# BaratiLab/GAMD

Measured on AMD Instinct MI355X. Metric: atom-steps/sec (force eval + integrate), 10k-atom LJ box, higher is better.
Workload: dtype f32; 1 GPU; C2: 10 000-atom LJ box, rho*=0.5, L=92.29 A, cutoff 3.0 sigma=10.2 A, fp32, 4 conv layers x 128, random-init weights (seed 0), 1 box per GPU; n_atoms=10000, boxes=1, launch=single process

## Files before the change

gamd_amd/csrc/conv_edge.hip:

```cpp
#include "gamd_common.h"
#include "gamd_internal.h"

#include <cstdlib>

namespace {

constexpr int CONV_LDS_FLOATS = 2 * GAMD_WFRAG_FLOATS + 3 * 128;

template <bool F2, typename Post, typename Mid>
__device__ __forceinline__ void gemm128_post(const f32x4* W, int lane, const f32x16 (&X)[4], f32x16 (&acc)[4], Post post, Mid mid) {
#pragma unroll
    for (int tp = 0; tp < 4; ++tp) {
        if (tp == 1) mid();
#pragma unroll
        for (int t = 0; t < 4; ++t) {
#pragma unroll
            for (int q = 0; q < 4; ++q) {
                const f32x4 w = W[((tp * 4 + t) * 4 + q) * 64 + lane];
#pragma unroll
                for (int j = 0; j < 4; ++j) {
                    const float x = X[t][q * 4 + j];
                    acc[tp] = F2 ? mfma32(x, w[j], acc[tp]) : mfma32(w[j], x, acc[tp]);
                }
                if (tp > 0) post(tp - 1, t * 4 + q);
            }
        }
    }
#pragma unroll
    for (int g = 0; g < 16; ++g) post(3, g);
}

template <int N>
__device__ __forceinline__ void phase_barrier() {
    asm volatile("s_waitcnt vmcnt(%0) lgkmcnt(0)" ::"n"(N) : "memory");
    __builtin_amdgcn_s_barrier();
}

__device__ __forceinline__ void load_e_tile(const float* __restrict__ e_frag, int tile, int lane, f32x16 (&X)[4]) {
    const f32x4* ef = (const f32x4*)e_frag + (size_t)tile * 16 * 64;
#pragma unroll
    for (int t = 0; t < 4; ++t)
#pragma unroll
        for (int q = 0; q < 4; ++q) {
            const f32x4 v = gamd_load_stream(&ef[(t * 4 + q) * 64 + lane]);
#pragma unroll
            for (int j = 0; j < 4; ++j) X[t][q * 4 + j] = v[j];
        }
}

template <bool TIME>
__global__ void __launch_bounds__(512, 2) k_conv_edge(ConvEdgeArgs a) {
    if (a.devflags[DEVFLAG_FROZEN]) return;
    extern __shared__ __attribute__((aligned(16))) float lds[];
    float* buf0 = lds;
    float* buf1 = lds + GAMD_WFRAG_FLOATS;
    float* vb1 = buf1 + GAMD_WFRAG_FLOATS;
    float* vb3 = vb1 + 128;
    float* vb4 = vb3 + 128;

    const int tid = threadIdx.x, lane = tid & 63, slot = lane & 31, half = lane >> 5;
    const int wave = __builtin_amdgcn_readfirstlane(tid >> 6);
    const unsigned lane16 = (unsigned)lane * 16u;
    int E = a.counters[CNT_E];
    if ((long long)E > a.e_cap) E = (int)a.e_cap;
    const int n_tiles = (E + GAMD_TILE - 1) / GAMD_TILE;
    const int n_units = (n_tiles + 3) / 4;
    int first, end, step;
    gamd_xcd_range(n_units, blockIdx.x, gridDim.x, first, end, step);
    if (first >= end) return;
    const int n_iter = ((end - first + step - 1) / step + 1) / 2;
    const int wsub = wave & 3, whalf = wave >> 2;
    const bool early = whalf == 0;
    auto tile_of = [&](int it) {
        const int u = first + (2 * it + whalf) * step;
        return (it < n_iter && u < end) ? u * 4 + wsub : n_tiles;
    };
    auto stage = [&](const float* gw, float* buf) { gamd_stage_weight_raw_contig<8>(gw, buf, wave, lane16); };

    long long tacc[16];
#pragma unroll
    for (int i = 0; i < 16; ++i) tacc[i] = 0;
    long long tprev = 0;
#define TMARK(i) do { if (TIME) { const long long tn__ = (long long)__builtin_readcyclecounter(); tacc[i] += tn__ - tprev; tprev = tn__; } } while (0)

    if (tid < 128) { vb1[tid] = a.b1[tid]; vb3[tid] = a.b3[tid]; vb4[tid] = a.b4[tid]; }
    stage(a.w1p, buf0);

    f32x16 RA[4], RB[4], RC[4];
    auto init_b4 = [&]() {
#pragma unroll
        for (int tp = 0; tp < 4; ++tp) {
            const float b = vb4[32 * tp + slot];
#pragma unroll
            for (int r = 0; r < 16; ++r) RC[tp][r] = b;
        }
    };

    int tile = tile_of(0);
    bool active = tile < n_tiles;
    int src = 0, dst = 0;
    {
        const int x = tile * GAMD_TILE + gamd_pi(slot);
        if (active && x < E) { src = GAMD_CHK_RANGE(a.sticky, a.col[x], 0, a.zero_row, GAMD_CHK_CONV_SRC); dst = GAMD_CHK_RANGE(a.sticky, a.erow[x], 0, a.zero_row, GAMD_CHK_CONV_DST); }
        else { src = a.zero_row; dst = a.zero_row; }
        if (active) load_e_tile(a.e_frag, tile, lane, RA);
    }
    asm volatile("" ::"v"(src), "v"(dst));
    asm volatile("s_waitcnt vmcnt(0)" ::: "memory");
    __syncthreads();
    if (TIME) tprev = (long long)__builtin_readcyclecounter();
    unsigned pend_ends = 0;
    int pend_p = 0;

    auto gather_S = [&]() { load_row_chain(a.S + (size_t)src * GAMD_H, half, RA); };
    auto gather_hn = [&]() {
        const unsigned soff = (unsigned)src << 9;
        const unsigned idx0 = 16u * (unsigned)half;
        const unsigned slot16 = 16u * (unsigned)slot;
#pragma unroll
        for (int r4 = 0; r4 < 4; ++r4) {
            unsigned o0, o1, o2, o3;
            asm volatile("ds_bpermute_b32 %0, %4, %5 offset:%6\n\tds_bpermute_b32 %1, %4, %5 offset:%7\n\t"
                         "ds_bpermute_b32 %2, %4, %5 offset:%8\n\tds_bpermute_b32 %3, %4, %5 offset:%9\n\ts_waitcnt lgkmcnt(0)"
                         : "=&v"(o0), "=&v"(o1), "=&v"(o2), "=&v"(o3)
                         : "v"(idx0), "v"(soff), "n"(4 * (0 + 8 * r4)), "n"(4 * (1 + 8 * r4)), "n"(4 * (2 + 8 * r4)), "n"(4 * (3 + 8 * r4)));
            const unsigned o[4] = {o0, o1, o2, o3};
#pragma unroll
            for (int k = 0; k < 4; ++k) {
                const f32x4 hv = *(const f32x4*)((const char*)a.hn + (o[k] + slot16));
#pragma unroll
                for (int tp = 0; tp < 4; ++tp) RA[r4][k * 4 + tp] = hv[tp];
            }
        }
    };

    auto early_barrier = [&](bool gathered) { if (gathered) phase_barrier<16>(); else phase_barrier<0>(); };
    auto piece_stores = [&]() {
        while (__any(pend_ends != 0)) {
            if (pend_ends != 0) {
                const int r = __builtin_ctz(pend_ends);
                pend_ends &= pend_ends - 1;
                f32x4 pv;
#pragma unroll
                for (int tp = 0; tp < 4; ++tp) {
                    float v = RC[tp][0];
#pragma unroll
                    for (int k = 1; k < 16; ++k) v = (r == k) ? RC[tp][k] : v;
                    pv[tp] = v;
                }
                *(f32x4*)(a.partial + (size_t)pend_p * GAMD_H + 4 * slot) = pv;
                ++pend_p;
            }
        }
    };
#define FENCE() __builtin_amdgcn_sched_barrier(0)

    for (int it = 0; it < n_iter; ++it) {
        const int x0 = tile * GAMD_TILE + 16 * half;
        int nvalid = E - x0;
        nvalid = !active ? 0 : (nvalid >= 16 ? 16 : (nvalid <= 0 ? 0 : nvalid));
        const int tile_n = tile_of(it + 1);
        const bool active_n = tile_n < n_tiles;
        int src_n = a.zero_row, dst_n = src_n;

        if (active) {
            load_bias_chain(vb1, half, RB);
            TMARK(0);
            gemm128_post<false>((const f32x4*)buf0, lane, RA, RB,
                                [&](int tp, int g) { RB[tp][g] = gamd_silu_hw(RB[tp][g]); },
                                [&]() {
                                    FENCE();
                                    piece_stores();
                                    load_row_chain(a.D + (size_t)dst * GAMD_H, half, RC);
                                    stage(a.w2p, buf1);
                                    FENCE();
                                });
            TMARK(1);
        } else {
            piece_stores();
            stage(a.w2p, buf1);
        }
        if (!early) phase_barrier<0>();
        TMARK(2);
        if (active) gather_S();
        TMARK(3);
        if (early) early_barrier(active);
        if (active) {
            gemm128_post<false>((const f32x4*)buf1, lane, RB, RC,
                                [&](int tp, int g) { RC[tp][g] = gamd_silu_hw(RC[tp][g] + RA[tp][g]); },
                                [&]() { FENCE(); stage(a.w3p, buf0); FENCE(); });
            TMARK(4);
        } else {
            stage(a.w3p, buf0);
        }
        if (!early) phase_barrier<0>();
        TMARK(5);
        if (active) gather_hn();
        TMARK(6);
        if (early) early_barrier(active);
        unsigned mask = 0;
        int p0 = 0;
        if (active) {
            mask = a.chunk_mask[tile * 2 + half];
            p0 = GAMD_CHK_RANGE(a.sticky, a.chunk_piece[tile * 2 + half], 0, a.piece_cap - 17, GAMD_CHK_PIECE);
        }
        if (active_n) {
            const int xn = tile_n * GAMD_TILE + gamd_pi(slot);
            if (xn < E) { src_n = GAMD_CHK_RANGE(a.sticky, a.col[xn], 0, a.zero_row, GAMD_CHK_CONV_SRC); dst_n = GAMD_CHK_RANGE(a.sticky, a.erow[xn], 0, a.zero_row, GAMD_CHK_CONV_DST); }
        }
        if (active) {
            load_bias_chain(vb3, half, RB);
            TMARK(7);
            gemm128_post<false>((const f32x4*)buf0, lane, RC, RB,
                                [&](int tp, int g) { RB[tp][g] = gamd_silu_hw(RB[tp][g]); },
                                [&]() { FENCE(); stage(a.w4p, buf1); FENCE(); });
            TMARK(8);
        } else {
            stage(a.w4p, buf1);
        }
        phase_barrier<0>();
        asm volatile("" ::"v"(mask), "v"(p0), "v"(src_n), "v"(dst_n));
        TMARK(9);
        if (active) {
            init_b4();
            const unsigned keep_bits = ~(mask << 1);
            gemm128_post<true>((const f32x4*)buf1, lane, RB, RC, [&](int tp, int r) {
                RC[tp][r] = gamd_msg_acc(RA[r >> 2][(r & 3) * 4 + tp], RC[tp][r], (r > 0 && ((keep_bits >> r) & 1u)) ? RC[tp][r - 1] : 0.f);
            }, [&]() { FENCE(); if (it + 1 < n_iter) stage(a.w1p, buf0); FENCE(); });
            pend_ends = mask;
            if (nvalid > 0 && !((mask >> (nvalid - 1)) & 1u)) pend_ends |= 1u << (nvalid - 1);
            pend_p = p0;
            TMARK(10);
        } else {
            if (it + 1 < n_iter) stage(a.w1p, buf0);
        }
        if (!early) phase_barrier<0>();
        TMARK(11);
        if (active_n) load_e_tile(a.e_frag, tile_n, lane, RA);
        TMARK(12);
        if (early) early_barrier(active_n);
        TMARK(13);
        tile = tile_n; active = active_n; src = src_n; dst = dst_n;
    }
#undef FENCE
    piece_stores();
    if (TIME && a.tdbg && lane == 0) {
#pragma unroll
        for (int i = 0; i < 16; ++i) a.tdbg[((size_t)blockIdx.x * 8 + wave) * 16 + i] = tacc[i];
    }
#undef TMARK
}

template <bool TIME>
int launch(const ConvEdgeArgs& a, int n_blocks, hipStream_t st) {
    const size_t lds = sizeof(float) * CONV_LDS_FLOATS;
    static PerDeviceOnce once;
    if (int e = gamd_allow_dynamic_lds(once, (int)lds, k_conv_edge<TIME>)) return e;
    hipLaunchKernelGGL(k_conv_edge<TIME>, dim3(n_blocks), dim3(512), lds, st, a);
    GAMD_CHECK_LAUNCH();
    return 0;
}

}

int launch_conv_edge(const ConvEdgeArgs& a, int n_blocks, hipStream_t st) {
#ifdef GAMD_PROFILING
    static const bool timed = getenv("GAMD_CONV_TIME") != nullptr;
    if (timed) return launch<true>(a, n_blocks, st);
#endif
    return launch<false>(a, n_blocks, st);
}
```

gamd_amd/csrc/conv_edge_small.hip:

```cpp
#include "gamd_common.h"
#include "gamd_internal.h"

namespace {

constexpr int XLD = GAMD_XLD;

template <int EHT, int HT, bool WIDE>
__global__ void __launch_bounds__(256) k_conv_edge_small(ConvEdgeArgs a) {
    if (a.devflags[DEVFLAG_FROZEN]) return;
    constexpr int H = 128 * HT;
    __shared__ __attribute__((aligned(16))) float xbuf[32 * XLD];
    const int lane = threadIdx.x & 63, slot = lane & 31, half = lane >> 5;
    const int quarter = __builtin_amdgcn_readfirstlane(threadIdx.x >> 6);
    int E = a.counters[CNT_E];
    if ((long long)E > a.e_cap) E = (int)a.e_cap;
    const int n_tiles = (E + GAMD_TILE - 1) / GAMD_TILE;

    auto feat4 = [&](int ob) { return WIDE ? 128 * ob + 32 * quarter + slot : 4 * slot + quarter; };
    for (int tile = blockIdx.x; tile < n_tiles; tile += gridDim.x) {
        const int x = tile * GAMD_TILE + gamd_pi(slot);
        const bool valid = x < E;
        const int src = valid ? GAMD_CHK_RANGE(a.sticky, a.col[x], 0, a.zero_row, GAMD_CHK_CONV_SRC) : 0;
        const int dst = valid ? GAMD_CHK_RANGE(a.sticky, a.erow[x], 0, a.zero_row, GAMD_CHK_CONV_DST) : 0;
        f32x16 X[4], XE[EHT][4], acc;
        WQuarter wa, wb;
        const float* wblk = a.w1p;
        load_wquarter(wblk, quarter, lane, wa);
#pragma unroll
        for (int kb = 0; kb < EHT; ++kb) {
            const f32x4* ef = (const f32x4*)a.e_frag + ((size_t)tile * EHT + kb) * 16 * 64;
#pragma unroll
            for (int t = 0; t < 4; ++t)
#pragma unroll
                for (int q = 0; q < 4; ++q) {
                    const f32x4 v = ef[(t * 4 + q) * 64 + lane];
#pragma unroll
                    for (int j = 0; j < 4; ++j) XE[kb][t][q * 4 + j] = v[j];
                }
        }
        const f32x16 s_q = load_slice(a.S + (size_t)src * 128, quarter, half);
        const f32x16 d_q = load_slice(a.D + (size_t)dst * 128, quarter, half);
        f32x16 hn_q[HT];
#pragma unroll
        for (int r = 0; r < 16; ++r) {
            const int rho = (r & 3) + 8 * (r >> 2) + 4 * half;
            const int s = __shfl(src, rho, 64);
#pragma unroll
            for (int ob = 0; ob < HT; ++ob) hn_q[ob][r] = a.hn[(size_t)s * H + feat4(ob)];
        }
        const unsigned mask = a.chunk_mask[tile * 2 + half];
        const int p0 = GAMD_CHK_RANGE(a.sticky, a.chunk_piece[tile * 2 + half], 0, a.piece_cap - 17, GAMD_CHK_PIECE);
        const int x0 = tile * GAMD_TILE + 16 * half;
        int nvalid = E - x0;
        nvalid = nvalid >= 16 ? 16 : (nvalid <= 0 ? 0 : nvalid);

        acc = load_slice(a.b1, quarter, half);
#pragma unroll
        for (int kb = 0; kb < EHT; ++kb) {
            WQuarter& cur = (kb & 1) ? wb : wa;
            WQuarter& nxt = (kb & 1) ? wa : wb;
            load_wquarter(wblk + (size_t)(kb + 1) * GAMD_WFRAG_FLOATS, quarter, lane, nxt);
            gemm_quarter<false>(cur, XE[kb], acc);
        }
#pragma unroll
        for (int r = 0; r < 16; ++r) acc[r] = gamd_silu_hw(acc[r]);
        exchange(xbuf, quarter, slot, half, acc, X);
        constexpr int B2 = EHT;
        WQuarter& w2 = (B2 & 1) ? wb : wa;
        WQuarter& w3 = (B2 & 1) ? wa : wb;
        if (WIDE) acc = s_q + d_q; else acc = d_q;
        load_wquarter(wblk + (size_t)(B2 + 1) * GAMD_WFRAG_FLOATS, quarter, lane, w3);
        gemm_quarter<false>(w2, X, acc);
#pragma unroll
        for (int r = 0; r < 16; ++r) acc[r] = gamd_silu_hw(WIDE ? acc[r] : acc[r] + s_q[r]);
        exchange(xbuf, quarter, slot, half, acc, X);
        acc = load_slice(a.b3, quarter, half);
        load_wquarter(wblk + (size_t)(B2 + 2) * GAMD_WFRAG_FLOATS, quarter, lane, w2);
        gemm_quarter<false>(w3, X, acc);
#pragma unroll
        for (int r = 0; r < 16; ++r) acc[r] = gamd_silu_hw(acc[r]);
        exchange(xbuf, quarter, slot, half, acc, X);
        const unsigned keep_bits = ~(mask << 1);
        unsigned ends0 = mask;
        if (nvalid > 0 && !((mask >> (nvalid - 1)) & 1u)) ends0 |= 1u << (nvalid - 1);
#pragma unroll
        for (int ob = 0; ob < HT; ++ob) {
            WQuarter& cur = (ob & 1) ? w3 : w2;
            WQuarter& nxt = (ob & 1) ? w2 : w3;
            if (ob + 1 < HT) load_wquarter(wblk + (size_t)(B2 + 3 + ob) * GAMD_WFRAG_FLOATS, quarter, lane, nxt);
            const float b = a.b4[128 * ob + 32 * quarter + slot];
#pragma unroll
            for (int r = 0; r < 16; ++r) acc[r] = b;
            gemm_quarter<true>(cur, X, acc);
            if (WIDE && a.emb_out) {
#pragma unroll
                for (int r = 0; r < 16; ++r) a.emb_out[(size_t)(x0 + r) * H + feat4(ob)] = acc[r];
            }
#pragma unroll
            for (int r = 0; r < 16; ++r) {
                acc[r] = gamd_msg_acc((r < nvalid) ? hn_q[ob][r] : 0.f, acc[r], (r > 0 && ((keep_bits >> r) & 1u)) ? acc[r - 1] : 0.f);
            }
            unsigned ends = ends0;
            int p = p0;
            while (__any(ends != 0)) {
                if (ends != 0) {
                    const int r = __builtin_ctz(ends);
                    ends &= ends - 1;
                    float v = acc[0];
#pragma unroll
                    for (int k = 1; k < 16; ++k) v = (r == k) ? acc[k] : v;
                    a.partial[(size_t)p * H + feat4(ob)] = v;
                    ++p;
                }
            }
        }
    }
}

}

int launch_conv_edge_small(const ConvEdgeArgs& a, int n_blocks, hipStream_t st) {
    hipLaunchKernelGGL((k_conv_edge_small<1, 1, false>), dim3(n_blocks), dim3(256), 0, st, a);
    GAMD_CHECK_LAUNCH();
    return 0;
}

int launch_conv_edge_small_wide(const ConvEdgeArgs& a, int eht, int ht, int n_blocks, hipStream_t st) {
    if (eht == 1 && ht == 1) hipLaunchKernelGGL((k_conv_edge_small<1, 1, true>), dim3(n_blocks), dim3(256), 0, st, a);
    else if (eht == 1 && ht == 2) hipLaunchKernelGGL((k_conv_edge_small<1, 2, true>), dim3(n_blocks), dim3(256), 0, st, a);
    else if (eht == 2 && ht == 1) hipLaunchKernelGGL((k_conv_edge_small<2, 1, true>), dim3(n_blocks), dim3(256), 0, st, a);
    else if (eht == 2 && ht == 2) hipLaunchKernelGGL((k_conv_edge_small<2, 2, true>), dim3(n_blocks), dim3(256), 0, st, a);
    else return -22;
    GAMD_CHECK_LAUNCH();
    return 0;
}
```

gamd_amd/csrc/gamd_api.hip:

```cpp
#include "../../include/gamd_hip.h"
#include "gamd_common.h"
#include "gamd_internal.h"

#include <algorithm>
#include <cmath>
#include <cstdarg>
#include <cstddef>
#include <cstdio>
#include <cstdlib>
#include <cstring>
#include <deque>
#include <map>
#include <string>
#include <vector>

namespace {

thread_local char g_err[512] = "";

int fail(int code, const char* fmt, ...) {
    va_list ap;
    va_start(ap, fmt);
    vsnprintf(g_err, sizeof(g_err), fmt, ap);
    va_end(ap);
    return code;
}

#define HIP_TRY(expr)                                                                              \
    do {                                                                                           \
        hipError_t e__ = (expr);                                                                   \
        if (e__ != hipSuccess) return fail(-1000 - (int)e__, "%s: %s", #expr, hipGetErrorString(e__)); \
    } while (0)

struct HostTensor {
    std::vector<int64_t> shape;
    std::vector<float> data;
};

thread_local hipStream_t tl_init_stream = nullptr;
struct InitStream {
    hipStream_t prev;
    explicit InitStream(hipStream_t st) : prev(tl_init_stream) { tl_init_stream = st; }
    ~InitStream() { tl_init_stream = prev; }
    InitStream(const InitStream&) = delete;
    InitStream& operator=(const InitStream&) = delete;
};
hipError_t init_upload(void* dst, const void* src, size_t bytes) {
    hipError_t e = hipMemcpyAsync(dst, src, bytes, hipMemcpyHostToDevice, tl_init_stream);
    return e != hipSuccess ? e : hipStreamSynchronize(tl_init_stream);
}

struct DevBuf {
    void* p = nullptr;
    size_t bytes = 0;
    int ensure(size_t want, bool zero) {
        if (want <= bytes && p) return 0;
        if (p) { hipError_t e = hipFree(p); if (e != hipSuccess) return (int)e; p = nullptr; bytes = 0; }
        hipError_t e = hipMalloc(&p, want);
        if (e != hipSuccess) return (int)e;
        bytes = want;
        if (zero) {
            e = hipMemsetAsync(p, 0, want, tl_init_stream);
            if (e == hipSuccess) e = hipStreamSynchronize(tl_init_stream);
            if (e != hipSuccess) return (int)e;
        }
        return 0;
    }
    void release() { if (p) (void)hipFree(p); p = nullptr; bytes = 0; }
    template <typename T> T* as() const { return reinterpret_cast<T*>(p); }
};

struct LayerDev {
    const float *w1p, *w2p, *w3p, *w4p, *b1, *b3, *b4;
    const float *w16p = nullptr;
    const float *e_ln_g = nullptr, *e_ln_b = nullptr;
    NodeLayerW node;
};

struct DeviceGuard {
    int prev = -1;
    bool changed = false;
    explicit DeviceGuard(int dev) {
        if (hipGetDevice(&prev) == hipSuccess && prev != dev) changed = hipSetDevice(dev) == hipSuccess;
    }
    ~DeviceGuard() { if (changed) (void)hipSetDevice(prev); }
    DeviceGuard(const DeviceGuard&) = delete;
    DeviceGuard& operator=(const DeviceGuard&) = delete;
};

struct MdPending {
    bool active = false;
    int kind = 0;
    MdArgs m{};
    NhcArgs a{};
    unsigned long long first_step = 0;
    long long n_steps = 0;
    float* x = nullptr;
    float* f = nullptr;
    const uint8_t* species = nullptr;
    hipStream_t st = nullptr;
};

}

static_assert(sizeof(gamd_config) == 96 && offsetof(gamd_config, n_boxes) == 88 && offsetof(gamd_config, edge_capacity) == 40,
              "gamd_config layout is part of the C ABI (gamd_amd/_lib.py mirrors it)");

struct gamd_handle {
    gamd_config cfg{};
    int dev = 0;
    int n = 0, L = 0, n_feat = 44, n_cu = 256;
    int n_boxes = 1, n_per_box = 0;
    bool use_small = false;
    DevBuf boxes_dev, box_shift;
    std::vector<float> boxes_host;
    int H = 128, Eh = 128, HT = 1, EHT = 1;
    int H_true = 128, Eh_true = 128, D_true = 128;
    int Dp = 128, DT = 1;
    int norm_bn = 0;
    bool update_edge = false;
    bool node_f16 = false;
    bool wide_enc = false, wide_conv = false;
    long long small_tile_limit = 512;
    std::map<std::string, HostTensor> host_w;
    bool finalized = false;
    double scaler_mean = 0.0, scaler_var = 1.0;

    DevBuf wblob;
    std::vector<LayerDev> layers;
    const float *enc_w1p = nullptr, *enc_w2p = nullptr, *enc_w3p = nullptr, *enc_b1 = nullptr, *enc_b2 = nullptr,
                *enc_b3 = nullptr, *enc_lng = nullptr, *enc_lnb = nullptr, *centers = nullptr;
    const float *node_emb = nullptr, *nenc_w = nullptr, *nenc_b = nullptr;
    const float *dec_w1p = nullptr, *dec_b1 = nullptr, *dec_w2 = nullptr, *dec_b2 = nullptr;
    float length_mean = 0.f, length_std = 1.f;
    RbfGrid rbf{};

    DevBuf pos_w, pos_s, cell_of, perm, inv_perm, deg, row_ptr, na_excl, bond_nbr;
    DevBuf hbuf, hn, S, D, P, f_norm, f_den;
    DevBuf l0_h, l0_hn, l0_S, l0_D, l0_P;
    DevBuf cell_cnt, cell_fill, cell_start;
    int ncell_cap = 0;
    long long e_cap = 0;
    long long piece_cap = 0;
    DevBuf col, erow, chunk_piece, chunk_mask, e_frag, partial, feat_dbg, e_emb, e_frag2;
    DevBuf counters, tdbg, tmp_eid, ke_partial, com_partial;
    DevBuf cnt2;
    int cnt_parity = 0;
    long long skin_calls = 0;
    int* cur_counters = nullptr;
    int* counters_host = nullptr;
    float* host_in = nullptr;
    float* host_out = nullptr;
    DevBuf pos_in;
    int* sticky_host = nullptr;
    int* sticky_dev = nullptr;
    hipStream_t init_stream = nullptr;
    DevBuf devflags;
    const float* feat_dev = nullptr;
    const uint8_t* rigid_checked = nullptr;
    MdPending pending;
    bool has_bonds = false;

    float skin = 0.f;
    DevBuf ref_pos, cand_deg, cand_ptr, cand_col;
    long long cand_cap = 0;
    bool cand_valid = false;

    float box[3] = {0, 0, 0};
    int nc[3] = {1, 1, 1};
    int ncell = 1;

    bool timing = false;
    std::vector<hipEvent_t> tev;
    std::vector<int> tev_kind;
    size_t tev_used = 0;
    std::vector<hipEvent_t> sev;
    std::vector<uint8_t> sev_closes;
    size_t sev_used = 0;
    static constexpr size_t EVENT_POOL_CAP = 1u << 16;
};

namespace {

bool small_path(const gamd_handle* h) { return h->use_small; }

BoxRef box_ref(const gamd_handle* h) {
    BoxRef r{};
    r.n_boxes = h->n_boxes;
    r.n_per_box = h->n_per_box;
    r.inv_npb = 1.0f / (float)h->n_per_box;
    r.boxes = h->n_boxes > 1 ? h->boxes_dev.as<float4>() : nullptr;
    return r;
}

int fill_com(gamd_handle* h, int enabled, MdCom* c) {
    c->enabled = enabled ? 1 : 0;
    c->blocks = std::max(1, std::min(16, (h->n_per_box + 1023) / 1024));
    c->partial = nullptr;
    if (!c->enabled) return 0;
    if (h->com_partial.ensure(sizeof(double) * 4 * (size_t)c->blocks * (size_t)h->n_boxes, true)) return fail(-12, "allocation failed");
    c->partial = h->com_partial.as<double>();
    return 0;
}

int alloc_candidates(gamd_handle* h, long long cap) {
    cap = std::max<long long>(cap, h->n);
    if (h->cand_col.ensure(sizeof(int) * ((size_t)cap + 64), true)) return fail(-12, "candidate buffer allocation failed");
    h->cand_cap = cap;
    h->cand_valid = false;
    return 0;
}

int alloc_edges(gamd_handle* h, long long e_cap) {
    const size_t ec = (size_t)e_cap + 2 * GAMD_TILE;
    int r = 0;
    r |= h->col.ensure(sizeof(int) * ec, true);
    r |= h->erow.ensure(sizeof(int) * ec, true);
    r |= h->chunk_piece.ensure(sizeof(int) * (ec / GAMD_CHUNK + 2), true);
    r |= h->chunk_mask.ensure(sizeof(unsigned) * (ec / GAMD_CHUNK + 2), true);
    r |= h->e_frag.ensure(sizeof(float) * 4096 * (size_t)h->EHT * (ec / GAMD_TILE + 1), false);
    r |= h->partial.ensure(sizeof(float) * (size_t)h->H * (ec / GAMD_CHUNK + (size_t)h->n + 2), false);
    h->piece_cap = (long long)(ec / GAMD_CHUNK + (size_t)h->n + 2);
    if (h->update_edge) {
        r |= h->e_emb.ensure(sizeof(float) * (size_t)h->H * ec, false);
        r |= h->e_frag2.ensure(sizeof(float) * 4096 * (size_t)h->EHT * (ec / GAMD_TILE + 1), false);
    }
    if (h->cfg.keep_stages) r |= h->feat_dbg.ensure(sizeof(float) * 48 * ec, true);
    if (r) return fail(-12, "edge buffer allocation failed for capacity %lld", e_cap);
    h->e_cap = e_cap;
    if (h->skin > 0.f) {
        const double grow = std::pow(((double)h->cfg.cutoff + h->skin) / (double)h->cfg.cutoff, 3.0);
        const long long want = (long long)((double)e_cap * grow * 1.7) + 1024;
        if (want > h->cand_cap) return alloc_candidates(h, want);
    }
    return 0;
}

int set_box(gamd_handle* h, const float* box, hipStream_t st = nullptr) {
    const int nb = h->n_boxes;
    bool changed = h->boxes_host.size() != (size_t)nb * 3;
    for (int b = 0; b < nb; ++b)
        for (int d = 0; d < 3; ++d) {
            const float v = box[3 * b + d];
            if (!(v > 0.f)) return fail(-22, "box[%d][%d] = %g is not positive", b, d, (double)v);
            if (!changed && h->boxes_host[(size_t)3 * b + d] != v) changed = true;
        }
    if (!changed) return 0;
    h->cand_valid = false;
    std::vector<int> grid((size_t)nb * 4);
    long long ncell = 0;
    for (int b = 0; b < nb; ++b) {
        long long nc_b = 1;
        for (int d = 0; d < 3; ++d) {
            const int nc = std::max(1, (int)std::floor((double)box[3 * b + d] / (((double)h->cfg.cutoff + (double)h->skin) * 1.0001)));
            grid[(size_t)4 * b + d] = nc;
            nc_b *= nc;
        }
        if (ncell + nc_b > (1ll << 30)) return fail(-22, "cell grid too large");
        grid[(size_t)4 * b + 3] = (int)ncell;
        ncell += nc_b;
    }
    for (int d = 0; d < 3; ++d) { h->box[d] = box[d]; h->nc[d] = grid[d]; }
    h->ncell = (int)ncell;
    if ((int)ncell > h->ncell_cap) {
        int r = 0;
        r |= h->counters.ensure(sizeof(int) * (CNT_COUNT + 2 * (size_t)ncell), true);
        r |= h->cell_start.ensure(sizeof(int) * ((size_t)ncell + 1), true);
        if (r) return fail(-12, "cell buffer allocation failed");
        h->ncell_cap = (int)ncell;
    }
    h->boxes_host.assign(box, box + (size_t)nb * 3);
    if (nb > 1) {
        HIP_TRY(hipStreamSynchronize(st));
        std::vector<float> img((size_t)nb * 12, 0.f);
        for (int b = 0; b < nb; ++b) {
            for (int d = 0; d < 3; ++d) { img[(size_t)12 * b + d] = box[3 * b + d]; img[(size_t)12 * b + 4 + d] = 0.5f * box[3 * b + d]; }
            memcpy(&img[(size_t)12 * b + 8], &grid[(size_t)4 * b], 4 * sizeof(int));
        }
        HIP_TRY(init_upload(h->boxes_dev.p, img.data(), sizeof(float) * img.size()));
    }
    return 0;
}

NbrArgs nbr_args(gamd_handle* h, const float* pos_dev, const uint8_t* species_dev) {
    NbrArgs a{};
    a.n = h->n;
    a.flavour = h->cfg.nbr_flavour;
    for (int d = 0; d < 3; ++d) {
        a.box[d] = h->box[d];
        a.half[d] = 0.5f * h->box[d];
        a.nc[d] = h->nc[d];
    }
    a.rc = h->cfg.cutoff;
    a.rc2 = (float)((double)h->cfg.cutoff * (double)h->cfg.cutoff);
    a.ncell = h->ncell;
    a.bx = box_ref(h);
    a.box_shift = h->box_shift.as<int>();
    a.e_cap = h->e_cap;
    a.pos = pos_dev;
    a.species = species_dev;
    a.feat = h->feat_dev;
    a.self_loop = h->cfg.self_loop_mode == GAMD_SELF_LOOP_APPEND_ZERO_FEATURE ? 1 : 0;
    a.devflags = h->devflags.as<int>();
    a.pos_w = h->pos_w.as<float4>();
    a.pos_s = h->pos_s.as<float4>();
    a.cell_of = h->cell_of.as<int>();
    a.ncell_cap = h->ncell_cap;
    a.cell_cnt = h->counters.as<int>() + CNT_COUNT;
    a.cell_fill = h->counters.as<int>() + CNT_COUNT + h->ncell_cap;
    a.cell_start = h->cell_start.as<int>();
    a.perm = h->perm.as<int>();
    a.inv_perm = h->inv_perm.as<int>();
    a.deg = h->deg.as<int>();
    a.row_ptr = h->row_ptr.as<int>();
    a.na_excl = h->na_excl.as<int>();
    a.col = h->col.as<int>();
    a.erow = h->erow.as<int>();
    a.chunk_piece = h->chunk_piece.as<int>();
    a.chunk_mask = h->chunk_mask.as<unsigned>();
    a.counters = h->cur_counters ? h->cur_counters : h->counters.as<int>();
    a.sticky = h->sticky_dev;
    if (h->skin > 0.f) {
        a.skin_half2 = 0.25f * h->skin * h->skin;
        a.rc_build = h->cfg.cutoff + h->skin;
        a.rc2_build = (float)((double)a.rc_build * (double)a.rc_build);
        a.cand_deg = h->cand_deg.as<int>();
        a.cand_ptr = h->cand_ptr.as<int>();
        a.cand_col = h->cand_col.as<int>();
        a.cand_cap = h->cand_cap;
        a.use_small = small_path(h) ? 1 : 0;
        a.cand_stride = (int)std::max<long long>(1, std::min<long long>(h->cand_cap / h->n, 1 << 20));
    }
    return a;
}

void pack128(const float* W, float* out, int ld = 128) {
    for (int tp = 0; tp < 4; ++tp)
        for (int t = 0; t < 4; ++t)
            for (int q = 0; q < 4; ++q)
                for (int lane = 0; lane < 64; ++lane)
                    for (int j = 0; j < 4; ++j) {
                        const int n = 32 * tp + (lane & 31), k = 32 * t + 8 * q + 4 * (lane >> 5) + j;
                        out[((((tp * 4 + t) * 4 + q) * 64 + lane) * 4) + j] = W[(size_t)n * ld + k];
                    }
}
void pack16(const float* W, float* out, int ld = 128) {
    for (int ob = 0; ob < 8; ++ob)
        for (int blk = 0; blk < 8; ++blk)
            for (int lane = 0; lane < 64; ++lane)
                for (int r = 0; r < 4; ++r)
                    out[(((ob * 8 + blk) * 64 + lane) * 4) + r] = W[(size_t)(16 * ob + (lane & 15)) * ld + 16 * blk + 4 * (lane >> 4) + r];
}
void split_f16(float w, uint16_t* hi, uint16_t* lo);
void pack16_f16x3(const float* W, uint16_t* out) {
    for (int ob = 0; ob < 8; ++ob)
        for (int m = 0; m < 4; ++m)
            for (int lane = 0; lane < 64; ++lane)
                for (int j = 0; j < 8; ++j) {
                    const int k = 32 * m + 16 * (j >> 2) + 4 * (lane >> 4) + (j & 3);
                    const size_t hi = ((((size_t)(ob * 4 + m) * 2 + 0) * 64 + lane) * 8) + j, lo = ((((size_t)(ob * 4 + m) * 2 + 1) * 64 + lane) * 8) + j;
                    split_f16(W[(size_t)(16 * ob + (lane & 15)) * 128 + k], out + hi, out + lo);
                }
}
void pack_enc1(const float* W, int n_feat, float* out) {
    for (int tp = 0; tp < 4; ++tp)
        for (int g = 0; g < 6; ++g)
            for (int lane = 0; lane < 64; ++lane)
                for (int j = 0; j < 4; ++j) {
                    const int n = 32 * tp + (lane & 31), k = 2 * (4 * g + j) + (lane >> 5);
                    out[(((tp * 6 + g) * 64 + lane) * 4) + j] = k < n_feat ? W[n * n_feat + k] : 0.f;
                }
}

int kfeat16x(int m, int g) { return 32 * (m >> 3) + 8 * ((m >> 1) & 3) + 4 * (g & 1) + (g >> 1) + 2 * (m & 1); }
void pack16x(const float* W, float* out, int ld, bool chained) {
    for (int ob = 0; ob < 8; ++ob)
        for (int m4 = 0; m4 < 8; ++m4)
            for (int lane = 0; lane < 64; ++lane) {
                const int i = lane & 15, g = lane >> 4;
                const int row = chained ? kfeat16x(4 * ob + (i & 3), i >> 2) : 64 * (ob >> 2) + 4 * i + (ob & 3);
                for (int c = 0; c < 4; ++c)
                    out[(((size_t)ob * 8 + m4) * 64 + lane) * 4 + c] = W[(size_t)row * ld + kfeat16x(4 * m4 + c, g)];
            }
}

uint16_t f2bf(float x) {
    uint32_t u; memcpy(&u, &x, 4);
    if ((u & 0x7f800000u) == 0x7f800000u) return (uint16_t)(u >> 16);
    u += 0x7fffu + ((u >> 16) & 1u);
    return (uint16_t)(u >> 16);
}
void pack128_bf16(const float* W, uint16_t* out, int ld = 128) {
    for (int tp = 0; tp < 4; ++tp)
        for (int t = 0; t < 4; ++t)
            for (int u = 0; u < 2; ++u)
                for (int lane = 0; lane < 64; ++lane)
                    for (int j = 0; j < 8; ++j) {
                        const int r = 8 * u + j, half = lane >> 5;
                        const int n = 32 * tp + (lane & 31), k = 32 * t + (r & 3) + 8 * (r >> 2) + 4 * half;
                        out[((((tp * 4 + t) * 2 + u) * 64 + lane) * 8) + j] = f2bf(W[(size_t)n * ld + k]);
                    }
}
void pack_enc1_bf16(const float* W, int n_feat, uint16_t* out) {
    for (int tp = 0; tp < 4; ++tp)
        for (int s = 0; s < 3; ++s)
            for (int lane = 0; lane < 64; ++lane)
                for (int j = 0; j < 8; ++j) {
                    const int n = 32 * tp + (lane & 31), k = 16 * s + 8 * (lane >> 5) + j;
                    out[(((tp * 3 + s) * 64 + lane) * 8) + j] = k < n_feat ? f2bf(W[n * n_feat + k]) : (uint16_t)0;
                }
}

void split_f16(float w, uint16_t* hi, uint16_t* lo) {
    const _Float16 h = (_Float16)w;
    const _Float16 l = (_Float16)(w - (float)h);
    memcpy(hi, &h, 2); memcpy(lo, &l, 2);
}
void pack128_f16x3(const float* W, uint16_t* out, int ld = 128) {
    for (int tp = 0; tp < 4; ++tp)
        for (int t = 0; t < 4; ++t)
            for (int u = 0; u < 2; ++u)
                for (int lane = 0; lane < 64; ++lane)
                    for (int j = 0; j < 8; ++j) {
                        const int r = 8 * u + j, half = lane >> 5;
                        const int n = 32 * tp + (lane & 31), k = 32 * t + (r & 3) + 8 * (r >> 2) + 4 * half;
                        const size_t at = ((((tp * 4 + t) * 2 + u) * 64 + lane) * 8) + j;
                        split_f16(W[(size_t)n * ld + k], out + at, out + 16384 + at);
                    }
}
void pack_enc1_f16x3(const float* W, int n_feat, uint16_t* out) {
    for (int tp = 0; tp < 4; ++tp)
        for (int s = 0; s < 3; ++s)
            for (int lane = 0; lane < 64; ++lane)
                for (int j = 0; j < 8; ++j) {
                    const int n = 32 * tp + (lane & 31), k = 16 * s + 8 * (lane >> 5) + j;
                    const size_t at = (((tp * 3 + s) * 64 + lane) * 8) + j;
                    split_f16(k < n_feat ? W[n * n_feat + k] : 0.f, out + at, out + 6144 + at);
                }
}

struct BlobBuilder {
    std::vector<float> host;
    size_t add(size_t n_floats) {
        const size_t off = host.size();
        host.resize(off + ((n_floats + 63) & ~(size_t)63), 0.f);
        return off;
    }
};

const HostTensor* find_w(gamd_handle* h, const std::string& name, std::initializer_list<int64_t> shape) {
    auto it = h->host_w.find(name);
    if (it == h->host_w.end()) { fail(-2, "missing weight '%s'", name.c_str()); return nullptr; }
    if (it->second.shape != std::vector<int64_t>(shape)) {
        std::string got;
        for (auto d : it->second.shape) got += std::to_string(d) + ",";
        std::string want;
        for (auto d : shape) want += std::to_string(d) + ",";
        fail(-22, "weight '%s' has shape (%s), expected (%s) for this configuration", name.c_str(), got.c_str(),
             want.c_str());
        return nullptr;
    }
    return &it->second;
}

struct EdgeList { const int* centre; const int* neigh; long long n; };

int fill_rigid(const gamd_handle* h, int rigid_water, float mass_o, float mass_h, float r_oh, float r_hh,
               int* use_rigid, RigidWater* g) {
    *use_rigid = 0;
    if (!rigid_water) return 0;
    if (h->n_per_box % 3 != 0) return fail(-22, "rigid_water needs O,H,H triples: n_atoms = %d is not a multiple of 3", h->n_per_box);
    if (!(mass_h > 0.f) || !(mass_o > 0.f)) return fail(-22, "rigid_water needs mass_amu (O) and mass_h_amu (H)");
    if (!(r_oh > 0.f) || !(r_hh > 0.f) || !(r_hh < 2.f * r_oh)) return fail(-22, "rigid_water needs 0 < r_hh < 2 r_oh");
    const double rc = 0.5 * (double)r_hh, t = std::sqrt((double)r_oh * r_oh - rc * rc);
    const double ra = t * 2.0 * mass_h / ((double)mass_o + 2.0 * mass_h);
    g->m_o = mass_o; g->m_h = mass_h;
    g->rc = (float)rc; g->ra = (float)ra; g->rb = (float)(t - ra);
    *use_rigid = 1;
    return 0;
}

int enqueue_forward(gamd_handle* h, const float* pos_dev, const uint8_t* species_dev, float* out_norm_dev,
                    float* out_denorm_dev, hipStream_t st, hipEvent_t* evs, int* n_ev, std::vector<std::string>* labels,
                    const EdgeList* el = nullptr, const MdFuse* fuse = nullptr, bool copy_counters = true, bool l0_reuse = false) {
    auto mark = [&](const char* label) {
        if (evs) { (void)hipEventRecord(evs[*n_ev], st); ++*n_ev; labels->push_back(label); }
    };
    int r;
    mark("begin");
    const bool pingpong = !el && h->skin > 0.f;
    int* counters_next = nullptr;
    if (pingpong) {
        h->cnt_parity ^= 1;
        h->cur_counters = h->cnt2.as<int>() + h->cnt_parity * CNT_COUNT;
        counters_next = h->cnt2.as<int>() + (1 - h->cnt_parity) * CNT_COUNT;
    } else {
        h->cur_counters = h->counters.as<int>();
    }
    NbrArgs na = nbr_args(h, pos_dev, species_dev);
    na.counters_next = counters_next;
    if (el) {
        if ((r = launch_csr_from_edges(na, el->centre, el->neigh, el->n, h->tmp_eid.as<int>(), st)))
            return fail(-1, "edge-list CSR launch failed (%d)", r);
        h->cand_valid = false;
    } else if (h->skin > 0.f) {
        na.ref_pos = h->ref_pos.as<float4>();
        na.force_rebuild = h->cand_valid ? 0 : 1;
        ++h->skin_calls;
        na.cells_one_wg = (h->skin_calls < 32 || 6ll * h->sticky_host[STICKY_REBUILDS] < h->skin_calls) ? 1 : 0;
        if (fuse && !pingpong) return fail(-1, "internal: integrator halves can only be fused into the skin path");
        if ((r = launch_neighbor_skin(na, st, fuse))) return fail(-1, "neighbor (skin) launch failed (%d)", r);
        h->cand_valid = true;
    } else if ((r = launch_neighbor_build(na, st))) return fail(-1, "neighbor build launch failed (%d)", r);
    mark("neighbor_build");

    EncArgs ea{};
    ea.counters = h->cur_counters;
    ea.devflags = h->devflags.as<int>();
    ea.pos_s = h->pos_s.as<float4>();
    ea.col = h->col.as<int>();
    ea.erow = h->erow.as<int>();
    ea.bond_nbr = h->has_bonds ? h->bond_nbr.as<int>() : nullptr;
    ea.perm = h->perm.as<int>();
    ea.row_ptr = h->row_ptr.as<int>();
    ea.self_loop = na.self_loop;
    ea.zero_row = h->n;
    for (int d = 0; d < 3; ++d) { ea.box[d] = h->box[d]; ea.half[d] = 0.5f * h->box[d]; }
    ea.bx = box_ref(h);
    ea.length_mean = h->length_mean;
    ea.length_std = h->length_std;
    ea.gamma = (float)(1.0 / 0.025);
    ea.ln_inv_width = 1.0f / (float)h->Eh_true;
    ea.ln_n_pad = (float)(h->Eh - h->Eh_true);
    ea.n_feat = h->n_feat;
    ea.n_ksteps = (h->n_feat + 1) / 2;
    ea.centers = h->centers;
    ea.rbf = h->rbf;
    ea.w1p = h->enc_w1p; ea.w2p = h->enc_w2p; ea.w3p = h->enc_w3p;
    ea.b1 = h->enc_b1; ea.b2 = h->enc_b2; ea.b3 = h->enc_b3;
    ea.ln_g = h->enc_lng; ea.ln_b = h->enc_lnb;
    ea.e_format = !h->wide_enc ? 0 : h->cfg.edge_dtype == GAMD_EDGE_F16X3 ? 2 : h->cfg.edge_dtype == GAMD_EDGE_BF16 ? 1 : 0;
    ea.e_frag = h->e_frag.as<float>();
    ea.e_cap = h->e_cap;
    ea.sticky = h->sticky_dev;
    ea.feat_dbg = h->cfg.keep_stages ? h->feat_dbg.as<float>() : nullptr;
    int small_tiles = 0;
    if (h->cfg.edge_dtype == GAMD_EDGE_F32) {
        const long long e_est = el ? el->n + (na.self_loop ? h->n : 0)
                                   : (h->counters_host[CNT_E] > 0 ? (long long)h->counters_host[CNT_E] : (long long)((double)h->e_cap / 1.5));
        const long long tiles = (e_est + GAMD_TILE - 1) / GAMD_TILE;
        if (tiles <= h->small_tile_limit) small_tiles = (int)std::max<long long>(1, std::min<long long>(tiles + tiles / 8 + 1, 4096));
    }
    const bool half_quantum = h->wide_conv && h->cfg.edge_dtype == GAMD_EDGE_F32 && (h->cfg.kernel_select & GAMD_KSEL_FORCE_HALF_QUANTUM) != 0;
    bool tev_full = false;
    auto tev_begin = [&](int kind) -> int {
        if (!h->timing) return 0;
        if (h->tev_used + 2 > h->tev.size()) {
            if (h->tev.size() >= 8 * gamd_handle::EVENT_POOL_CAP) { tev_full = true; return 0; }
            for (int k = 0; k < 256; ++k) { hipEvent_t e; HIP_TRY(hipEventCreate(&e)); h->tev.push_back(e); h->tev_kind.push_back(0); }
        }
        h->tev_kind[h->tev_used] = kind;
        HIP_TRY(hipEventRecord(h->tev[h->tev_used], st));
        return 0;
    };
    auto tev_end = [&]() -> int {
        if (!h->timing || tev_full) return 0;
        HIP_TRY(hipEventRecord(h->tev[h->tev_used + 1], st));
        h->tev_used += 2;
        return 0;
    };
    if ((r = tev_begin(100))) return r;
    r = h->DT > 1 ? launch_edge_encode_wide_d(ea, h->EHT, h->DT, h->n_cu, st)
        : h->wide_enc ? launch_edge_encode_wide(ea, h->EHT, h->n_cu, st)
        : h->cfg.edge_dtype == GAMD_EDGE_BF16 ? launch_edge_encode_bf16(ea, h->n_cu, st)
        : h->cfg.edge_dtype == GAMD_EDGE_F16X3 ? launch_edge_encode_f16x3(ea, h->n_cu, st)
        : small_tiles > 0 ? launch_edge_encode_small(ea, small_tiles, st) : launch_edge_encode(ea, h->n_cu, st);
    if (r) return fail(-1, "edge encode launch failed (%d)", r);
    if ((r = tev_end())) return r;
    mark("edge_encode");

    const size_t nh = (size_t)h->n * (size_t)h->H;
    auto node = [&](const NodeArgs& na_) {
        return h->DT > 1 ? launch_node_wide_d(na_, h->HT, h->DT, st) : h->wide_conv ? launch_node_wide(na_, h->HT, st) : launch_node(na_, st);
    };
    auto hptr = [&](int l) { return h->hbuf.as<float>() + (h->cfg.keep_stages ? (size_t)l * nh : (size_t)(l & 1) * nh); };

    NodeArgs no{};
#ifdef GAMD_PROFILING
    { static const bool node_time = getenv("GAMD_NODE_TIME") != nullptr; if (node_time) no.tdbg = h->tdbg.as<long long>(); }
#endif
    no.counters = h->cur_counters;
    no.devflags = h->devflags.as<int>();
    no.sticky = h->sticky_dev;
    no.n = h->n;
    no.pos_s = h->pos_s.as<float4>();
    no.node_emb = h->node_emb; no.enc_w = h->nenc_w; no.enc_b = h->nenc_b;
    no.row_ptr = h->row_ptr.as<int>(); no.na_excl = h->na_excl.as<int>(); no.deg = h->deg.as<int>();
    no.partial = h->partial.as<float>();
    no.piece_cap = h->piece_cap;
    no.P_in = h->P.as<float>();
    no.hn_perm = (!h->wide_conv && h->cfg.edge_dtype == GAMD_EDGE_F16X3) ? 1 : 0;
    no.tab16 = (!h->wide_conv && h->cfg.edge_dtype == GAMD_EDGE_BF16) ? 1 : 0;
    no.hn_out = h->hn.as<float>(); no.S_out = h->S.as<float>(); no.D_out = h->D.as<float>(); no.P_out = h->P.as<float>();
    no.dec_w1p = h->dec_w1p; no.dec_b1 = h->dec_b1; no.dec_w2 = h->dec_w2; no.dec_b2 = h->dec_b2;
    no.ln_inv_width = 1.0f / (float)h->H_true;
    no.ln_n_pad = (float)(h->H - h->H_true);
    no.norm_bn = h->norm_bn;
    no.f16x3 = h->node_f16 ? 1 : 0;
    no.scale = (float)std::sqrt(h->scaler_var);
    no.shift = (float)h->scaler_mean;
    no.perm = h->perm.as<int>();
    no.forces_norm = out_norm_dev ? out_norm_dev : h->f_norm.as<float>();
    no.forces = out_denorm_dev;

    const bool l0 = h->skin > 0.f && !el;
    float* const h0 = (l0 && !h->cfg.keep_stages) ? h->l0_h.as<float>() : hptr(0);
    no.mode = 0;
    no.pre = h->layers[0].node;
    no.h_out = h0;
    if (l0) { no.hn_out = h->l0_hn.as<float>(); no.S_out = h->l0_S.as<float>(); no.D_out = h->l0_D.as<float>(); no.P_out = h->l0_P.as<float>(); }
    no.l0_gate = (l0 && l0_reuse) ? 1 : 0;
    if ((r = node(no))) return fail(-1, "node(0) launch failed (%d)", r);
    no.l0_gate = 0;
    no.hn_out = h->hn.as<float>(); no.S_out = h->S.as<float>(); no.D_out = h->D.as<float>(); no.P_out = h->P.as<float>();
    mark("node_first");


    for (int l = 0; l < h->L; ++l) {
        ConvEdgeArgs ca{};
        ca.counters = h->cur_counters;
        ca.devflags = h->devflags.as<int>();
        ca.col = h->col.as<int>(); ca.erow = h->erow.as<int>();
        ca.chunk_piece = h->chunk_piece.as<int>(); ca.chunk_mask = h->chunk_mask.as<unsigned>();
        ca.e_frag = (h->update_edge && l > 0) ? h->e_frag2.as<float>() : h->e_frag.as<float>();
        ca.emb_out = (h->update_edge && l + 1 < h->L) ? h->e_emb.as<float>() : nullptr;
        ca.hn = h->hn.as<float>(); ca.S = h->S.as<float>(); ca.D = h->D.as<float>();
        if (l0 && l == 0) { ca.hn = h->l0_hn.as<float>(); ca.S = h->l0_S.as<float>(); ca.D = h->l0_D.as<float>(); }
        const LayerDev& ld = h->layers[l];
        ca.w1p = ld.w1p; ca.w2p = ld.w2p; ca.w3p = ld.w3p; ca.w4p = ld.w4p; ca.w16p = ld.w16p;
        ca.b1 = ld.b1; ca.b3 = ld.b3; ca.b4 = ld.b4;
        ca.partial = h->partial.as<float>();
        ca.piece_cap = h->piece_cap;
        ca.sticky = h->sticky_dev;
        ca.e_cap = h->e_cap;
        ca.zero_row = h->n;
#ifdef GAMD_CHECKED
        { static const bool inject = getenv("GAMD_CHK_INJECT") != nullptr; if (inject) ca.zero_row = 0; }
#endif
        ca.tdbg = h->tdbg.as<long long>();
        if ((r = tev_begin(l))) return r;
        r = h->DT > 1 ? launch_conv_edge_wide_d(ca, h->EHT, h->HT, h->DT, h->n_cu, st)
            : h->wide_conv ? (h->cfg.edge_dtype == GAMD_EDGE_F16X3 ? launch_conv_edge_f16x3_wide(ca, h->EHT, h->HT, h->n_cu, st)
                            : h->cfg.edge_dtype == GAMD_EDGE_BF16 ? launch_conv_edge_bf16_wide(ca, h->EHT, h->HT, h->n_cu, st)
                            : (half_quantum && ca.w16p && !ca.emb_out) ? launch_conv_edge_wide16(ca, h->EHT, h->HT, h->n_cu, st)
                            : small_tiles > 0 ? launch_conv_edge_small_wide(ca, h->EHT, h->HT, small_tiles, st)
                                              : launch_conv_edge_wide(ca, h->EHT, h->HT, h->n_cu, st))
            : h->cfg.edge_dtype == GAMD_EDGE_BF16 ? launch_conv_edge_bf16(ca, h->n_cu, st)
            : h->cfg.edge_dtype == GAMD_EDGE_F16X3 ? launch_conv_edge_f16x3(ca, h->n_cu, st)
            : small_tiles > 0 ? launch_conv_edge_small(ca, small_tiles, st) : launch_conv_edge(ca, h->n_cu, st);
        if (r) return fail(-1, "conv edge launch failed (%d)", r);
        if ((r = tev_end())) return r;
        mark("conv_edge");
        if (ca.emb_out) {
            EdgeUpdateArgs ua{};
            ua.counters = h->cur_counters; ua.devflags = h->devflags.as<int>(); ua.e_cap = h->e_cap;
            ua.emb = ca.emb_out; ua.ln_g = ld.e_ln_g; ua.ln_b = ld.e_ln_b;
            ua.ln_inv_width = 1.0f / (float)h->Eh_true;
            ua.ln_n_pad = (float)(h->Eh - h->Eh_true);
            ua.e_frag_out = h->e_frag2.as<float>();
            if ((r = launch_edge_update(ua, h->HT, small_tiles > 0 ? std::max(1, small_tiles / 4) : 2 * h->n_cu, st)))
                return fail(-1, "edge update launch failed (%d)", r);
            mark("edge_update");
        }

        no.mode = (l == h->L - 1) ? 2 : 1;
        no.post = ld.node;
        if (l + 1 < h->L) no.pre = h->layers[l + 1].node;
        no.h_in = l == 0 ? h0 : hptr(l);
        no.P_in = (l0 && l == 0) ? h->l0_P.as<float>() : h->P.as<float>();
        no.h_out = hptr(l + 1);
        if ((r = node(no))) return fail(-1, "node launch failed (%d)", r);
        mark(no.mode == 2 ? "node_last_decode" : "node_mid");
    }
    if (copy_counters)
        HIP_TRY(hipMemcpyAsync(h->counters_host, h->cur_counters, sizeof(int) * CNT_COUNT, hipMemcpyDeviceToHost, st));
    return 0;
}

int check_traps(gamd_handle* h) {
    const int code = h->sticky_host[STICKY_CHECK_CODE];
    if (!code) return 0;
    const int value = h->sticky_host[STICKY_CHECK_VALUE], line = h->sticky_host[STICKY_CHECK_LINE];
    h->sticky_host[STICKY_CHECK_CODE] = 0;
    return fail(-35, "checked build: device-side range check %d failed (value %d, source line %d)", code, value, line);
}

int check_ready(gamd_handle* h) {
    if (!h) return fail(-22, "null handle");
    if (!h->finalized) return fail(-22, "weights not finalized (call gamd_finalize_weights)");
    return 0;
}

int check_model_inputs(gamd_handle* h, const uint8_t* species_dev) {
    if (h->cfg.kind == GAMD_KIND_WATER && !species_dev && !h->feat_dev)
        return fail(-22, "water model needs species (or gamd_set_node_features)");
    if (h->cfg.use_bond && !h->has_bonds) return fail(-22, "use_bond set but no bonds given (gamd_set_bonds)");
    return 0;
}

int check_rigid_layout(gamd_handle* h, const uint8_t* species_dev, hipStream_t st) {
    if (!species_dev) return fail(-22, "rigid_water needs species (O = 1, H = 0, atoms ordered O,H,H)");
    if (h->rigid_checked == species_dev) return 0;
    std::vector<uint8_t> sp((size_t)h->n);
    HIP_TRY(hipMemcpyAsync(sp.data(), species_dev, sp.size(), hipMemcpyDeviceToHost, st));
    HIP_TRY(hipStreamSynchronize(st));
    for (int i = 0; i < h->n; ++i)
        if ((sp[(size_t)i] != 0) != (i % 3 == 0))
            return fail(-22, "rigid_water needs atoms ordered O,H,H per molecule: species[%d] = %d", i, (int)sp[(size_t)i]);
    h->rigid_checked = species_dev;
    return 0;
}

int clear_devflags(gamd_handle* h) {
    const int init[2] = {0, -1};
    HIP_TRY(init_upload(h->devflags.p, init, sizeof(init)));
    return 0;
}

int step_event(gamd_handle* h, hipStream_t st, bool closes = false) {
    if (!h->timing) return 0;
    if (h->sev_used == h->sev.size()) {
        if (h->sev.size() >= gamd_handle::EVENT_POOL_CAP) return 0;
        for (int k = 0; k < 256; ++k) { hipEvent_t e; HIP_TRY(hipEventCreate(&e)); h->sev.push_back(e); h->sev_closes.push_back(0); }
    }
    h->sev_closes[h->sev_used] = closes ? 1 : 0;
    HIP_TRY(hipEventRecord(h->sev[h->sev_used++], st));
    return 0;
}

int enqueue_md_steps(gamd_handle* h, long long s_begin, bool skip_first) {
    MdPending& p = h->pending;
    int r;
    if (p.kind == 0 && h->skin > 0.f) {
        for (long long s = s_begin; s < p.n_steps; ++s) {
            if ((r = step_event(h, p.st))) return r;
            p.m.step = p.first_step + (unsigned long long)s;
            p.m.step_index = (int)s;
            int do_second = s > s_begin ? 1 : 0;
            const int do_first = (skip_first && s == s_begin) ? 0 : 1;
            if (p.m.com.enabled) {
                if (do_second && do_first) {
                    MdArgs prev = p.m;
                    prev.step_index = (int)(s - 1);
                    if ((r = launch_baoab_second_com(prev, p.st))) return fail(-1, "integrator launch failed (%d)", r);
                    do_second = 0;
                } else {
                    if (do_second) {
                        MdArgs prev = p.m;
                        prev.step_index = (int)(s - 1);
                        if ((r = launch_baoab_second(prev, p.st))) return fail(-1, "integrator launch failed (%d)", r);
                        do_second = 0;
                    }
                    if (do_first && (r = launch_com_partial(p.m.com, p.m.v, p.m.species, p.m.inv_mass, p.m.inv_mass_h, p.m.n, p.m.bx,
                                                            p.m.devflags, p.m.use_rigid, p.st)))
                        return fail(-1, "integrator launch failed (%d)", r);
                }
            }
            const MdFuse fuse{&p.m, do_second, do_first};
            if ((r = enqueue_forward(h, p.x, p.species, nullptr, p.f, p.st, nullptr, nullptr, nullptr, nullptr, &fuse,
                                     s + 1 == p.n_steps, s > s_begin)))
                return r;
        }
        if (p.n_steps > s_begin) {
            p.m.step_index = (int)(p.n_steps - 1);
            if ((r = launch_baoab_second(p.m, p.st))) return fail(-1, "integrator launch failed (%d)", r);
        }
        return step_event(h, p.st, true);
    }
    for (long long s = s_begin; s < p.n_steps; ++s) {
        if ((r = step_event(h, p.st))) return r;
        const bool first = !(skip_first && s == s_begin);
        const bool last = s + 1 == p.n_steps;
        if (p.kind == 0) {
            p.m.step = p.first_step + (unsigned long long)s;
            p.m.step_index = (int)s;
            if (first && (r = launch_baoab_first(p.m, p.st))) return fail(-1, "integrator launch failed (%d)", r);
            if ((r = enqueue_forward(h, p.x, p.species, nullptr, p.f, p.st, nullptr, nullptr, nullptr, nullptr, nullptr, last, s > s_begin))) return r;
            if ((r = launch_baoab_second(p.m, p.st))) return fail(-1, "integrator launch failed (%d)", r);
        } else {
            p.a.step_index = (int)s;
            if (first && (r = launch_nhc_first(p.a, p.st))) return fail(-1, "integrator launch failed (%d)", r);
            if ((r = enqueue_forward(h, p.x, p.species, nullptr, p.f, p.st, nullptr, nullptr, nullptr, nullptr, nullptr, last, s > s_begin))) return r;
            if ((r = launch_nhc_second(p.a, p.st))) return fail(-1, "integrator launch failed (%d)", r);
        }
    }
    return step_event(h, p.st, true);
}

}

extern "C" {

#ifdef GAMD_CHECKED
const char* gamd_version(void) { return "gamd_hip 0.1 (gfx950) checked"; }
#else
const char* gamd_version(void) { return "gamd_hip 0.1 (gfx950)"; }
#endif
const char* gamd_last_error(void) { return g_err; }

int32_t gamd_create(const gamd_config* cfg, gamd_handle** out) {
    if (!cfg || !out) return fail(-22, "null argument");
    if (cfg->n_atoms <= 0) return fail(-22, "n_atoms must be positive");
    if (cfg->n_boxes < 0 || cfg->n_boxes > (1 << 20)) return fail(-22, "n_boxes out of range");
    const int n_boxes = cfg->n_boxes > 1 ? cfg->n_boxes : 1;
    if ((long long)cfg->n_atoms * n_boxes >= (1 << 23) - 1)
        return fail(-22, "n_atoms x n_boxes = %lld: at most %d atoms per handle", (long long)cfg->n_atoms * n_boxes, (1 << 23) - 2);
    if (cfg->n_layers <= 0 || cfg->n_layers > 16) return fail(-22, "n_layers out of range");
    if (!(cfg->cutoff > 0.f)) return fail(-22, "cutoff must be positive");
    if (cfg->edge_dtype != GAMD_EDGE_F32 && cfg->edge_dtype != GAMD_EDGE_BF16 && cfg->edge_dtype != GAMD_EDGE_F16X3)
        return fail(-22, "unknown edge_dtype");
    if (!(cfg->neighbor_skin >= 0.f)) return fail(-22, "neighbor_skin must be >= 0");
    if (cfg->self_loop_mode != GAMD_SELF_LOOP_DGL07_NOOP && cfg->self_loop_mode != GAMD_SELF_LOOP_APPEND_ZERO_FEATURE)
        return fail(-22, "unknown self_loop_mode %d", cfg->self_loop_mode);
    if (cfg->self_loop_mode != GAMD_SELF_LOOP_DGL07_NOOP && cfg->edge_dtype != GAMD_EDGE_F32)
        return fail(-22, "self_loop_mode 1 is built for the fp32 edge dtype only");
    if (cfg->kernel_select & ~(GAMD_KSEL_FORCE_GENERIC_WIDTH | GAMD_KSEL_FORCE_HALF_QUANTUM))
        return fail(-22, "unknown kernel_select bits 0x%x", cfg->kernel_select);
    int ndev = 0;
    if (hipGetDeviceCount(&ndev) != hipSuccess || ndev <= 0)
        return fail(-19, "no HIP device available: libgamd_hip has no CPU fallback");
    if (cfg->device < 0 || cfg->device >= ndev) return fail(-22, "device %d out of range (%d visible)", cfg->device, ndev);
    DeviceGuard guard(cfg->device);
    hipDeviceProp_t prop;
    HIP_TRY(hipGetDeviceProperties(&prop, cfg->device));
    const int H_true = cfg->encoding_size ? cfg->encoding_size : 128, Eh_true = cfg->edge_embedding_dim ? cfg->edge_embedding_dim : 128;
    const int D_true = cfg->hidden_dim ? cfg->hidden_dim : 128;
    if (H_true < 1 || H_true > 256 || Eh_true < 1 || Eh_true > 256)
        return fail(-22, "encoding_size and edge_embedding_dim must be in [1, 256] (got %d, %d)", H_true, Eh_true);
    if (D_true < 1 || D_true > 256) return fail(-22, "hidden_dim must be in [1, 256] (got %d)", D_true);
    const int Dp = D_true <= 128 ? 128 : 256;
    if (Dp > 128 && cfg->edge_dtype != GAMD_EDGE_F32)
        return fail(-22, "hidden_dim above 128 is built for edge_dtype f32 only (got hidden_dim %d)", D_true);
    const int H = H_true <= 128 ? 128 : 256, Eh = Eh_true <= 128 ? 128 : 256;
    const bool exact128 = H_true == 128 && Eh_true == 128 && D_true == 128;
    const bool generic = H != 128 || Eh != 128 || cfg->no_expand_edge;
    if (cfg->edge_dtype != GAMD_EDGE_F32 && H == 256 && (long long)cfg->n_atoms * n_boxes > (1ll << 22) - 2)
        return fail(-22, "bf16 / split-fp16 with encoding_size > 128: at most 2^22 - 2 atoms per handle (32-bit byte offsets into hn)");
    gamd_handle* h = new gamd_handle();
    h->cfg = *cfg;
    h->dev = cfg->device;
    if (hipStreamCreateWithFlags(&h->init_stream, hipStreamNonBlocking) != hipSuccess) {
        h->init_stream = nullptr;
        gamd_destroy(h);
        return fail(-12, "stream creation failed");
    }
    InitStream init(h->init_stream);
    h->n_boxes = n_boxes;
    h->n_per_box = cfg->n_atoms;
    h->n = cfg->n_atoms * n_boxes;
    h->L = cfg->n_layers;
    h->H = H; h->Eh = Eh; h->HT = H / 128; h->EHT = Eh / 128;
    h->H_true = H_true; h->Eh_true = Eh_true; h->D_true = D_true;
    h->Dp = Dp; h->DT = Dp / 128;
    h->skin = cfg->neighbor_skin;
    if (cfg->small_tile_limit != 0) h->small_tile_limit = cfg->small_tile_limit < 0 ? -1 : cfg->small_tile_limit;
    const bool forced = (cfg->kernel_select & GAMD_KSEL_FORCE_GENERIC_WIDTH) && cfg->edge_dtype == GAMD_EDGE_F32;
    const bool lp_generic = cfg->edge_dtype != GAMD_EDGE_F32 && (generic || !exact128);
    h->wide_enc = generic || forced || lp_generic || Dp > 128;
    h->wide_conv = H != 128 || Eh != 128 || forced || lp_generic || Dp > 128;
    h->n_feat = (cfg->no_expand_edge ? 4 : 44) + (cfg->use_bond ? 1 : 0);
    h->n_cu = prop.multiProcessorCount > 0 ? prop.multiProcessorCount : 256;
    const size_t n = (size_t)h->n;
    int r = 0;
    r |= h->pos_w.ensure(sizeof(float4) * n, true);
    r |= h->pos_s.ensure(sizeof(float4) * (n + 1), true);
    r |= h->cell_of.ensure(sizeof(int) * n, true);
    r |= h->perm.ensure(sizeof(int) * (n + 1), true);
    if (n_boxes > 1) {
        r |= h->boxes_dev.ensure(sizeof(float) * 12 * (size_t)n_boxes, true);
        r |= h->box_shift.ensure(sizeof(int) * ((size_t)n_boxes + 2), true);
    }
    r |= h->inv_perm.ensure(sizeof(int) * n, true);
    r |= h->deg.ensure(sizeof(int) * n, true);
    r |= h->row_ptr.ensure(sizeof(int) * (n + 1), true);
    r |= h->na_excl.ensure(sizeof(int) * (n + 1), true);
    const size_t nh = n * (size_t)H * sizeof(float), nd = n * (size_t)Dp * sizeof(float), zd = (size_t)Dp * sizeof(float);
    r |= h->hbuf.ensure(nh * (cfg->keep_stages ? (size_t)h->L + 1 : 2), true);
    r |= h->hn.ensure(nh + (size_t)H * sizeof(float), true);
    r |= h->S.ensure(nd + zd, true);
    r |= h->D.ensure(nd + zd, true);
    r |= h->P.ensure(nd, true);
    if (cfg->neighbor_skin > 0.f) {
        r |= h->l0_hn.ensure(nh + (size_t)H * sizeof(float), true);
        r |= h->l0_S.ensure(nd + zd, true);
        r |= h->l0_D.ensure(nd + zd, true);
        r |= h->l0_P.ensure(nd, true);
        if (!cfg->keep_stages) r |= h->l0_h.ensure(nh, true);
    }
    r |= h->f_norm.ensure(sizeof(float) * 3 * n, true);
    r |= h->f_den.ensure(sizeof(float) * 3 * n, true);
    r |= h->tdbg.ensure(sizeof(long long) * 16 * 8 * 1024, true);
    r |= h->devflags.ensure(sizeof(int) * DEVFLAG_COUNT, true);
    r |= h->cnt2.ensure(sizeof(int) * 2 * CNT_COUNT, true);
    if (r) { gamd_destroy(h); return fail(-12, "device allocation failed"); }
    {
        const int no_atom = -2;
        if (init_upload(h->perm.as<int>() + n, &no_atom, sizeof(int)) != hipSuccess) {
            gamd_destroy(h);
            return fail(-1, "device copy failed");
        }
    }
    if ((r = clear_devflags(h))) { gamd_destroy(h); return r; }
    if (hipHostMalloc((void**)&h->counters_host, sizeof(int) * CNT_COUNT) != hipSuccess) {
        gamd_destroy(h);
        return fail(-12, "pinned allocation failed");
    }
    memset(h->counters_host, 0, sizeof(int) * CNT_COUNT);
    if (hipHostMalloc((void**)&h->sticky_host, sizeof(int) * STICKY_COUNT, hipHostMallocMapped) != hipSuccess ||
        hipHostGetDevicePointer((void**)&h->sticky_dev, h->sticky_host, 0) != hipSuccess) {
        gamd_destroy(h);
        return fail(-12, "mapped host allocation failed");
    }
    memset(h->sticky_host, 0, sizeof(int) * STICKY_COUNT);
    if (h->skin > 0.f) {
        int rr = 0;
        rr |= h->ref_pos.ensure(sizeof(float4) * n, true);
        rr |= h->cand_deg.ensure(sizeof(int) * n, true);
        rr |= h->cand_ptr.ensure(sizeof(int) * (n + 1), true);
        if (rr) { gamd_destroy(h); return fail(-12, "device allocation failed"); }
    }
    {
        std::vector<float> all((size_t)n_boxes * 3);
        for (int b = 0; b < n_boxes; ++b)
            for (int d = 0; d < 3; ++d) all[(size_t)3 * b + d] = cfg->box[d];
        if ((r = set_box(h, all.data()))) { gamd_destroy(h); return r; }
    }
    {
        const double per_atom = std::min<double>(h->n, 27.0 * h->n / std::max(1, h->ncell));
        h->use_small = h->n <= 1024 && n_boxes <= 1 && (double)h->n * per_atom <= 3.0e5 && h->ncell <= 4096;
    }
    long long ecap = cfg->edge_capacity;
    if (ecap <= 0) {
        const double vol = (double)cfg->box[0] * cfg->box[1] * cfg->box[2];
        const double per_atom = 4.18879 * std::pow((double)cfg->cutoff, 3) * (double)h->n_per_box / vol + 1.0;
        ecap = (long long)(1.5 * per_atom * (double)h->n) + 1024 + 16ll * n_boxes;
    }
    if (cfg->self_loop_mode) ecap += h->n;
    if ((r = alloc_edges(h, ecap))) { gamd_destroy(h); return r; }
    if (hipStreamSynchronize(h->init_stream) != hipSuccess) { gamd_destroy(h); return fail(-1, "device synchronisation failed"); }
    *out = h;
    return 0;
}

int32_t gamd_destroy(gamd_handle* h) {
    if (!h) return 0;
    DeviceGuard guard(h->dev);
    InitStream init(h->init_stream);
    h->devflags.release();
    h->cnt2.release();
    DevBuf* bufs[] = {&h->boxes_dev, &h->box_shift, &h->wblob, &h->pos_w, &h->pos_s, &h->cell_of, &h->perm, &h->inv_perm, &h->deg, &h->row_ptr,
                      &h->na_excl, &h->bond_nbr, &h->hbuf, &h->hn, &h->S, &h->D, &h->P, &h->l0_h, &h->l0_hn, &h->l0_S, &h->l0_D, &h->l0_P, &h->f_norm, &h->f_den,
                      &h->cell_cnt, &h->cell_fill, &h->cell_start, &h->col, &h->erow, &h->chunk_piece,
                      &h->chunk_mask, &h->e_frag, &h->e_emb, &h->e_frag2, &h->partial, &h->feat_dbg, &h->counters, &h->tdbg, &h->tmp_eid, &h->ke_partial, &h->com_partial,
                      &h->ref_pos, &h->cand_deg, &h->cand_ptr, &h->cand_col};
    for (DevBuf* b : bufs) b->release();
    h->pos_in.release();
    if (h->host_in) (void)hipHostFree(h->host_in);
    if (h->host_out) (void)hipHostFree(h->host_out);
    if (h->counters_host) (void)hipHostFree(h->counters_host);
    if (h->sticky_host) (void)hipHostFree(h->sticky_host);
    for (hipEvent_t e : h->tev) (void)hipEventDestroy(e);
    for (hipEvent_t e : h->sev) (void)hipEventDestroy(e);
    if (h->init_stream) (void)hipStreamDestroy(h->init_stream);
    delete h;
    return 0;
}

int32_t gamd_load_weight(gamd_handle* h, const char* name, const float* data, const int64_t* shape, int32_t ndim) {
    if (!h || !name || !data || !shape || ndim < 1 || ndim > 2) return fail(-22, "bad argument to gamd_load_weight");
    HostTensor t;
    size_t cnt = 1;
    for (int i = 0; i < ndim; ++i) { t.shape.push_back(shape[i]); cnt *= (size_t)shape[i]; }
    t.data.assign(data, data + cnt);
    h->host_w[name] = std::move(t);
    h->finalized = false;
    return 0;
}

int32_t gamd_finalize_weights(gamd_handle* h) {
    if (!h) return fail(-22, "null handle");
    DeviceGuard guard(h->dev);
    InitStream init(h->init_stream);
    const int F = h->n_feat, L = h->L;
    const int64_t H = h->H, Eh = h->Eh, HT = h->HT, EHT = h->EHT;
    const int64_t Ht = h->H_true, Et = h->Eh_true, Dt = h->D_true;
    const int64_t Dp = h->Dp, DT = h->DT;
    const bool expand = !h->cfg.no_expand_edge;
    BlobBuilder bb;
    struct Off { size_t w1p, w2p, w3p, w4p, w16p = 0, b1, b3, b4, elng = 0, elnb = 0, lng, lnb, wsp, wdp, wpdp, bS, bP, wpep, wphip, bphi; };
    std::vector<Off> lo(L);
    std::deque<HostTensor> padded;
    auto get = [&](const std::string& nm, std::initializer_list<int64_t> shp, std::initializer_list<int64_t> pad) -> const HostTensor* {
        const HostTensor* t = find_w(h, nm, shp);
        if (!t) return nullptr;
        const std::vector<int64_t> ps(pad);
        if (t->shape == ps) return t;
        HostTensor o;
        o.shape = ps;
        const int64_t r = ps.size() == 2 ? t->shape[0] : 1, c = ps.size() == 2 ? t->shape[1] : t->shape[0];
        const int64_t cp = ps.size() == 2 ? ps[1] : ps[0], rp = ps.size() == 2 ? ps[0] : 1;
        o.data.assign((size_t)(rp * cp), 0.f);
        for (int64_t i = 0; i < r; ++i) std::copy(t->data.begin() + i * c, t->data.begin() + (i + 1) * c, o.data.begin() + i * cp);
        padded.push_back(std::move(o));
        return &padded.back();
    };
    auto put_vec = [&](const HostTensor* t) { size_t o = bb.add(t->data.size()); std::copy(t->data.begin(), t->data.end(), bb.host.begin() + o); return o; };
    auto put_blocks = [&](const HostTensor* t, int OB, int KB) {
        size_t o = bb.add((size_t)OB * KB * GAMD_WFRAG_FLOATS);
        for (int ob = 0; ob < OB; ++ob)
            for (int kb = 0; kb < KB; ++kb)
                pack128(t->data.data() + (size_t)128 * ob * 128 * KB + 128 * kb,
                        bb.host.data() + o + (size_t)(ob * KB + kb) * GAMD_WFRAG_FLOATS, 128 * KB);
        return o;
    };
    auto put_blocks_f16x3_fn = [&](const HostTensor* t, int OB, int KB) {
        size_t o = bb.add((size_t)OB * KB * GAMD_WFRAG_FLOATS);
        for (int ob = 0; ob < OB; ++ob)
            for (int kb = 0; kb < KB; ++kb)
                pack128_f16x3(t->data.data() + (size_t)128 * ob * 128 * KB + 128 * kb,
                              reinterpret_cast<uint16_t*>(bb.host.data() + o + (size_t)(ob * KB + kb) * GAMD_WFRAG_FLOATS), 128 * KB);
        return o;
    };
    h->node_f16 = h->cfg.edge_dtype != GAMD_EDGE_F32;
    auto put_node = [&](const HostTensor* t, int OB, int KB) {
        if (h->wide_conv) return h->node_f16 ? put_blocks_f16x3_fn(t, OB, KB) : put_blocks(t, OB, KB);
        size_t o = bb.add(GAMD_WFRAG_FLOATS);
        if (h->node_f16) pack16_f16x3(t->data.data(), reinterpret_cast<uint16_t*>(bb.host.data() + o));
        else pack16(t->data.data(), bb.host.data() + o);
        return o;
    };
    const bool bf16_edges = h->cfg.edge_dtype == GAMD_EDGE_BF16 && !h->wide_conv;
    const bool bf16_wide = h->cfg.edge_dtype == GAMD_EDGE_BF16 && h->wide_conv;
    const bool f16x3_edges = h->cfg.edge_dtype == GAMD_EDGE_F16X3 && !h->wide_conv;
    const bool f16x3_wide = h->cfg.edge_dtype == GAMD_EDGE_F16X3 && h->wide_conv;
    auto put_edge_f16x3 = [&](const HostTensor* t) {
        size_t o = bb.add(GAMD_WFRAG_FLOATS);
        pack128_f16x3(t->data.data(), reinterpret_cast<uint16_t*>(bb.host.data() + o));
        return o;
    };
    auto put_blocks_f16x3 = put_blocks_f16x3_fn;
    auto put_edge_bf16 = [&](const HostTensor* t) {
        size_t o = bb.add(GAMD_WFRAG_FLOATS / 2);
        pack128_bf16(t->data.data(), reinterpret_cast<uint16_t*>(bb.host.data() + o));
        return o;
    };

    const bool update_edge = h->host_w.count("graph_conv.conv.0.edge_layer_norm.weight") != 0;
    if (update_edge) {
        if (Ht != Et)
            return fail(-22, "update_edge_emb needs encoding_size == edge_embedding_dim (got %d, %d)", (int)Ht, (int)Et);
        if (h->cfg.edge_dtype != GAMD_EDGE_F32 || h->cfg.self_loop_mode)
            return fail(-22, "update_edge_emb is built for the fp32 edge MLP without appended self loops");
        h->wide_enc = h->wide_conv = true;
    }
    if (update_edge != h->update_edge) {
        h->update_edge = update_edge;
        if (alloc_edges(h, h->e_cap)) return -12;
    }
    const bool norm_bn = h->host_w.count("graph_conv.norm_layers.0.running_mean") != 0;
    h->norm_bn = norm_bn ? 1 : 0;
    for (int l = 0; l < L; ++l) {
        const std::string p = "graph_conv.conv." + std::to_string(l);
        const HostTensor *ea0w = get(p + ".edge_affine.mlp_layer.0.weight", {128, Et}, {128, Eh}), *ea0b = get(p + ".edge_affine.mlp_layer.0.bias", {128}, {128});
        const HostTensor *ea2w = get(p + ".edge_affine.mlp_layer.2.weight", {Dt, 128}, {Dp, 128}), *ea2b = get(p + ".edge_affine.mlp_layer.2.bias", {Dt}, {Dp});
        const HostTensor *sw = get(p + ".src_affine.weight", {Dt, Ht}, {Dp, H}), *sb = get(p + ".src_affine.bias", {Dt}, {Dp});
        const HostTensor *dw = get(p + ".dst_affine.weight", {Dt, Ht}, {Dp, H}), *db = get(p + ".dst_affine.bias", {Dt}, {Dp});
        const HostTensor *t1w = get(p + ".theta_edge.mlp_layer.1.weight", {Dt, Dt}, {Dp, Dp}), *t1b = get(p + ".theta_edge.mlp_layer.1.bias", {Dt}, {Dp});
        const HostTensor *t3w = get(p + ".theta_edge.mlp_layer.3.weight", {Ht, Dt}, {H, Dp}), *t3b = get(p + ".theta_edge.mlp_layer.3.bias", {Ht}, {H});
        const HostTensor *pdw = get(p + ".phi_dst.weight", {Dt, Ht}, {Dp, H}), *pdb = get(p + ".phi_dst.bias", {Dt}, {Dp});
        const HostTensor *pew = get(p + ".phi_edge.weight", {Dt, Ht}, {Dp, H}), *peb = get(p + ".phi_edge.bias", {Dt}, {Dp});
        const HostTensor *phw = get(p + ".phi.mlp_layer.1.weight", {Ht, Dt}, {H, Dp}), *phb = get(p + ".phi.mlp_layer.1.bias", {Ht}, {H});
        const HostTensor *ng = get("graph_conv.norm_layers." + std::to_string(l) + ".weight", {Ht}, {H});
        const HostTensor *nb = get("graph_conv.norm_layers." + std::to_string(l) + ".bias", {Ht}, {H});
        if (!ea0w || !ea0b || !ea2w || !ea2b || !sw || !sb || !dw || !db || !t1w || !t1b || !t3w || !t3b || !pdw ||
            !pdb || !pew || !peb || !phw || !phb || !ng || !nb)
            return -2;
        if (norm_bn) {
            const std::string np_ = "graph_conv.norm_layers." + std::to_string(l);
            const HostTensor *rm = get(np_ + ".running_mean", {Ht}, {H}), *rv = get(np_ + ".running_var", {Ht}, {H});
            if (!rm || !rv) return -2;
            HostTensor al, be;
            al.shape = be.shape = {H};
            al.data.assign((size_t)H, 0.f);
            be.data.assign((size_t)H, 0.f);
            for (int64_t i = 0; i < Ht; ++i) {
                const float invstd = 1.0f / std::sqrt(rv->data[i] + 1e-5f);
                al.data[i] = ng->data[i] * invstd;
                be.data[i] = nb->data[i] - rm->data[i] * al.data[i];
            }
            padded.push_back(std::move(al)); ng = &padded.back();
            padded.push_back(std::move(be)); nb = &padded.back();
        }
        if (bf16_edges) {
            auto scaled = [&](const HostTensor* t, double f) -> const HostTensor* {
                HostTensor o = *t;
                for (float& v : o.data) v = (float)((double)v * f);
                padded.push_back(std::move(o));
                return &padded.back();
            };
            const double LOG2E = 1.4426950408889634, LN2 = 0.6931471805599453;
            ea0w = scaled(ea0w, LOG2E); ea0b = scaled(ea0b, LOG2E); t1b = scaled(t1b, LOG2E); t3w = scaled(t3w, LN2);
            sw = scaled(sw, LOG2E); dw = scaled(dw, LOG2E);
            sb = scaled(sb, LOG2E); db = scaled(db, LOG2E); ea2b = scaled(ea2b, LOG2E);
        }
        Off& o = lo[l];
        HostTensor b4_perm;
        HostTensor w4_perm;
        auto permute_w4 = [&]() {
            w4_perm = *t3w;
            b4_perm = *t3b;
            for (int q = 0; q < 4; ++q)
                for (int s = 0; s < 32; ++s) {
                    std::copy(t3w->data.begin() + (size_t)(4 * s + q) * 128, t3w->data.begin() + (size_t)(4 * s + q + 1) * 128,
                              w4_perm.data.begin() + (size_t)(32 * q + s) * 128);
                    b4_perm.data[32 * q + s] = t3b->data[4 * s + q];
                }
            t3b = &b4_perm;
        };
        if (bf16_edges) {
            permute_w4();
            o.w1p = put_edge_bf16(ea0w); o.w2p = put_edge_bf16(ea2w); o.w3p = put_edge_bf16(t1w); o.w4p = put_edge_bf16(&w4_perm);
        } else if (f16x3_edges) {
            o.w1p = put_edge_f16x3(ea0w); o.w2p = put_edge_f16x3(ea2w); o.w3p = put_edge_f16x3(t1w); o.w4p = put_edge_f16x3(t3w);
        } else if (bf16_wide) {
            auto put_blocks_bf16 = [&](const HostTensor* t, int OB, int KB) {
                size_t o = bb.add((size_t)OB * KB * (GAMD_WFRAG_FLOATS / 2));
                for (int ob = 0; ob < OB; ++ob)
                    for (int kb = 0; kb < KB; ++kb)
                        pack128_bf16(t->data.data() + (size_t)128 * ob * 128 * KB + 128 * kb,
                                     reinterpret_cast<uint16_t*>(bb.host.data() + o + (size_t)(ob * KB + kb) * (GAMD_WFRAG_FLOATS / 2)), 128 * KB);
                return o;
            };
            o.w1p = put_blocks_bf16(ea0w, 1, (int)EHT);
            o.w2p = put_blocks_bf16(ea2w, 1, 1);
            o.w3p = put_blocks_bf16(t1w, 1, 1);
            o.w4p = put_blocks_bf16(t3w, (int)HT, 1);
        } else if (f16x3_wide) {
            o.w1p = put_blocks_f16x3(ea0w, 1, (int)EHT);
            o.w2p = put_blocks_f16x3(ea2w, 1, 1);
            o.w3p = put_blocks_f16x3(t1w, 1, 1);
            o.w4p = put_blocks_f16x3(t3w, (int)HT, 1);
        } else {
            o.w1p = put_blocks(ea0w, 1, (int)EHT);
            o.w2p = put_blocks(ea2w, (int)DT, 1);
            o.w3p = put_blocks(t1w, (int)DT, (int)DT);
            if (DT > 1) {
                o.w4p = put_blocks(t3w, (int)HT, (int)DT);
            } else if (h->wide_conv) {
                o.w4p = put_blocks(t3w, (int)HT, 1);
                o.w16p = bb.add((size_t)(EHT + 2 + HT) * GAMD_WFRAG_FLOATS);
                size_t at = o.w16p;
                for (int kb = 0; kb < (int)EHT; ++kb, at += GAMD_WFRAG_FLOATS) pack16x(ea0w->data.data() + 128 * kb, bb.host.data() + at, 128 * (int)EHT, true);
                pack16x(ea2w->data.data(), bb.host.data() + at, 128, true); at += GAMD_WFRAG_FLOATS;
                pack16x(t1w->data.data(), bb.host.data() + at, 128, true); at += GAMD_WFRAG_FLOATS;
                for (int ob = 0; ob < (int)HT; ++ob, at += GAMD_WFRAG_FLOATS) pack16x(t3w->data.data() + (size_t)128 * ob * 128, bb.host.data() + at, 128, false);
            } else {
                permute_w4();
                o.w4p = put_blocks(&w4_perm, 1, 1);
            }
        }
        o.b1 = put_vec(ea0b); o.b3 = put_vec(t1b); o.b4 = put_vec(t3b);
        o.lng = put_vec(ng); o.lnb = put_vec(nb);
        if (update_edge) {
            const HostTensor *eg = get(p + ".edge_layer_norm.weight", {Et}, {Eh}), *eb = get(p + ".edge_layer_norm.bias", {Et}, {Eh});
            if (!eg || !eb) return -2;
            o.elng = put_vec(eg); o.elnb = put_vec(eb);
        }
        o.wsp = put_node(sw, (int)DT, (int)HT); o.wdp = put_node(dw, (int)DT, (int)HT); o.wpdp = put_node(pdw, (int)DT, (int)HT);
        o.bS = bb.add((size_t)Dp);
        for (int i = 0; i < (int)Dp; ++i) bb.host[o.bS + i] = (sb->data[i] + db->data[i]) + ea2b->data[i];
        o.bP = bb.add((size_t)Dp);
        for (int i = 0; i < (int)Dp; ++i) bb.host[o.bP + i] = pdb->data[i] + peb->data[i];
        o.wpep = put_node(pew, (int)DT, (int)HT); o.wphip = put_node(phw, (int)HT, (int)DT); o.bphi = put_vec(phb);
    }
    const HostTensor *e0w = get("edge_encoder.mlp_layer.0.weight", {Dt, (int64_t)F}, {Dp, (int64_t)F}), *e0b = get("edge_encoder.mlp_layer.0.bias", {Dt}, {Dp});
    const HostTensor *e2w = get("edge_encoder.mlp_layer.2.weight", {Dt, Dt}, {Dp, Dp}), *e2b = get("edge_encoder.mlp_layer.2.bias", {Dt}, {Dp});
    const HostTensor *e4w = get("edge_encoder.mlp_layer.4.weight", {Et, Dt}, {Eh, Dp}), *e4b = get("edge_encoder.mlp_layer.4.bias", {Et}, {Eh});
    const HostTensor *elg = get("edge_layer_norm.weight", {Et}, {Eh}), *elb = get("edge_layer_norm.bias", {Et}, {Eh});
    const HostTensor *cen = expand ? get("edge_expand.centers", {40}, {40}) : nullptr;
    const HostTensor *lm = get("length_mean", {1}, {1}), *ls = get("length_std", {1}, {1});
    const HostTensor *d0w = get("graph_decoder.mlp_layer.0.weight", {Dt, Ht}, {Dp, H}), *d0b = get("graph_decoder.mlp_layer.0.bias", {Dt}, {Dp});
    const HostTensor *d2w = get("graph_decoder.mlp_layer.2.weight", {3, Dt}, {3, Dp}), *d2b = get("graph_decoder.mlp_layer.2.bias", {3}, {3});
    if (!e0w || !e0b || !e2w || !e2b || !e4w || !e4b || !elg || !elb || (expand && !cen) || !lm || !ls || !d0w || !d0b ||
        !d2w || !d2b)
        return -2;
    const size_t o_e1 = bb.add(DT > 1 ? (size_t)GAMD_WFRAG_FLOATS : (size_t)(4 * 6 * 64 * 4));
    if (DT > 1) for (int64_t b = 0; b < DT; ++b) pack_enc1(e0w->data.data() + (size_t)(128 * b * F), F, bb.host.data() + o_e1 + (size_t)b * (4 * 6 * 64 * 4));
    else if (bf16_edges) pack_enc1_bf16(e0w->data.data(), F, reinterpret_cast<uint16_t*>(bb.host.data() + o_e1));
    else if (f16x3_edges) pack_enc1_f16x3(e0w->data.data(), F, reinterpret_cast<uint16_t*>(bb.host.data() + o_e1));
    else pack_enc1(e0w->data.data(), F, bb.host.data() + o_e1);
    const bool enc_wide_f16 = h->wide_enc && h->cfg.edge_dtype != GAMD_EDGE_F32;
    const size_t o_e2 = bf16_edges ? put_edge_bf16(e2w) : f16x3_edges ? put_edge_f16x3(e2w) : enc_wide_f16 ? put_blocks_f16x3(e2w, 1, 1)
                                                                                                              : put_blocks(e2w, (int)DT, (int)DT);
    HostTensor e4w_c = *e4w, e4b_c = *e4b;
    if (!bf16_edges && !f16x3_edges) {
        for (int64_t k = 0; k < Dp; ++k) {
            double m = 0.0;
            for (int64_t o = 0; o < Et; ++o) m += (double)e4w->data[(size_t)(o * Dp + k)];
            m /= (double)Et;
            for (int64_t o = 0; o < Et; ++o) e4w_c.data[(size_t)(o * Dp + k)] = (float)((double)e4w->data[(size_t)(o * Dp + k)] - m);
        }
        double mb = 0.0;
        for (int64_t o = 0; o < Et; ++o) mb += (double)e4b->data[(size_t)o];
        mb /= (double)Et;
        for (int64_t o = 0; o < Et; ++o) e4b_c.data[(size_t)o] = (float)((double)e4b->data[(size_t)o] - mb);
    }
    const size_t o_e3 = bf16_edges ? put_edge_bf16(e4w) : f16x3_edges ? put_edge_f16x3(e4w) : enc_wide_f16 ? put_blocks_f16x3(&e4w_c, (int)EHT, 1)
                                                                                                              : put_blocks(&e4w_c, (int)EHT, (int)DT);
    const size_t o_eb1 = put_vec(e0b), o_eb2 = put_vec(e2b), o_eb3 = put_vec(&e4b_c), o_elg = put_vec(elg), o_elb = put_vec(elb);
    const size_t o_cen = expand ? put_vec(cen) : bb.add(64);
    const size_t o_d1 = put_node(d0w, (int)DT, (int)HT), o_db1 = put_vec(d0b), o_d2 = put_vec(d2w), o_db2 = put_vec(d2b);
    size_t o_emb = 0, o_nw = 0, o_nb = 0;
    if (h->cfg.kind == GAMD_KIND_LJ) {
        const HostTensor* emb = get("node_emb", {1, Ht}, {1, H});
        if (!emb) return -2;
        o_emb = put_vec(emb);
    } else {
        const HostTensor *nw = get("node_encoder.weight", {Ht, 1}, {H, 1}), *nb = get("node_encoder.bias", {Ht}, {H});
        if (!nw || !nb) return -2;
        o_nw = put_vec(nw); o_nb = put_vec(nb);
    }
    h->length_mean = lm->data[0];
    h->length_std = ls->data[0];
    h->rbf = RbfGrid{};
    if (expand) {
        const double c0 = cen->data[0], delta = ((double)cen->data[39] - c0) / 39.0;
        bool uniform = delta > 0.0;
        for (int k = 0; k < 40 && uniform; ++k)
            uniform = std::fabs((double)cen->data[k] - (c0 + k * delta)) <= 2.5e-7 * std::max(1.0, std::fabs(c0 + k * delta));
        if (uniform) {
            const double gexp = -(1.0 / 0.025) * 1.4426950408889634, s = 2.0 * delta;
            h->rbf = RbfGrid{1, (float)c0, (float)delta, (float)(-2.0 * gexp * s), (float)(gexp * s * s),
                             (float)std::exp2(2.0 * gexp * s * s)};
        }
    }

    if (h->wblob.ensure(sizeof(float) * bb.host.size(), false)) return fail(-12, "weight blob allocation failed");
    HIP_TRY(init_upload(h->wblob.p, bb.host.data(), sizeof(float) * bb.host.size()));
    const float* B = h->wblob.as<float>();
    h->layers.assign(L, LayerDev{});
    for (int l = 0; l < L; ++l) {
        const Off& o = lo[l];
        LayerDev& d = h->layers[l];
        d.w1p = B + o.w1p; d.w2p = B + o.w2p; d.w3p = B + o.w3p; d.w4p = B + o.w4p;
        d.w16p = (h->wide_conv && h->cfg.edge_dtype == GAMD_EDGE_F32 && DT == 1) ? B + o.w16p : nullptr;
        d.b1 = B + o.b1; d.b3 = B + o.b3; d.b4 = B + o.b4;
        d.node.ln_g = B + o.lng; d.node.ln_b = B + o.lnb;
        if (update_edge) { d.e_ln_g = B + o.elng; d.e_ln_b = B + o.elnb; }
        d.node.wsp = B + o.wsp; d.node.wdp = B + o.wdp; d.node.wpdp = B + o.wpdp;
        d.node.bS = B + o.bS; d.node.bP = B + o.bP;
        d.node.wpep = B + o.wpep; d.node.wphip = B + o.wphip; d.node.bphi = B + o.bphi;
    }
    h->enc_w1p = B + o_e1; h->enc_w2p = B + o_e2; h->enc_w3p = B + o_e3;
    h->enc_b1 = B + o_eb1; h->enc_b2 = B + o_eb2; h->enc_b3 = B + o_eb3;
    h->enc_lng = B + o_elg; h->enc_lnb = B + o_elb; h->centers = B + o_cen;
    h->dec_w1p = B + o_d1; h->dec_b1 = B + o_db1; h->dec_w2 = B + o_d2; h->dec_b2 = B + o_db2;
    h->node_emb = h->cfg.kind == GAMD_KIND_LJ ? B + o_emb : nullptr;
    h->nenc_w = h->cfg.kind == GAMD_KIND_LJ ? nullptr : B + o_nw;
    h->nenc_b = h->cfg.kind == GAMD_KIND_LJ ? nullptr : B + o_nb;
    h->finalized = true;
    return 0;
}

int32_t gamd_set_scaler(gamd_handle* h, double mean, double var) {
    if (!h) return fail(-22, "null handle");
    if (!(var >= 0.0)) return fail(-22, "scaler variance must be non-negative");
    h->scaler_mean = mean;
    h->scaler_var = var;
    return 0;
}

int32_t gamd_set_bonds(gamd_handle* h, const int32_t* bonds, int64_t n_bonds) {
    if (!h || (!bonds && n_bonds > 0)) return fail(-22, "bad argument to gamd_set_bonds");
    DeviceGuard guard(h->dev);
    InitStream init(h->init_stream);
    std::vector<int> tab((size_t)h->n * 4, -1);
    auto add = [&](int i, int j) -> int {
        for (int k = 0; k < 4; ++k) {
            if (tab[(size_t)i * 4 + k] == j) return 0;
            if (tab[(size_t)i * 4 + k] < 0) { tab[(size_t)i * 4 + k] = j; return 0; }
        }
        return -1;
    };
    for (int box = 0; box < h->n_boxes; ++box)
        for (int64_t b = 0; b < n_bonds; ++b) {
            int i = bonds[2 * b], j = bonds[2 * b + 1];
            if (i < 0 || j < 0 || i >= h->n_per_box || j >= h->n_per_box)
                return fail(-22, "bond %lld references atom out of range", (long long)b);
            i += box * h->n_per_box; j += box * h->n_per_box;
            if (add(i, j) || add(j, i)) return fail(-22, "more than 4 bonded partners for one atom is not supported");
        }
    if (h->bond_nbr.ensure(sizeof(int) * tab.size(), false)) return fail(-12, "bond table allocation failed");
    HIP_TRY(init_upload(h->bond_nbr.p, tab.data(), sizeof(int) * tab.size()));
    h->has_bonds = n_bonds > 0;
    return 0;
}

int32_t gamd_set_node_features(gamd_handle* h, const float* feat_dev) {
    if (!h) return fail(-22, "null handle");
    if (feat_dev && h->cfg.kind != GAMD_KIND_WATER) return fail(-22, "node features belong to the water models (the LJ model has node_emb)");
    h->feat_dev = feat_dev;
    return 0;
}

int32_t gamd_get_device_flags(gamd_handle* h, int32_t flags[4]) {
    if (!h || !flags) return fail(-22, "null argument");
    flags[0] = h->sticky_host[STICKY_NONFINITE] ? 1 : 0;
    flags[1] = flags[2] = flags[3] = 0;
    h->sticky_host[STICKY_NONFINITE] = 0;
    return 0;
}

int32_t gamd_build_neighbors(gamd_handle* h, const float* pos_dev, const uint8_t* species_dev, const float* box, void* stream) {
    int r;
    if ((r = check_ready(h))) return r;
    if (!pos_dev || !box) return fail(-22, "null argument");
    DeviceGuard guard(h->dev);
    InitStream init((hipStream_t)stream);
    hipStream_t st = (hipStream_t)stream;
    for (int attempt = 0; attempt < 4; ++attempt) {
        if ((r = set_box(h, box, st))) return r;
        h->cur_counters = h->counters.as<int>();
        NbrArgs na = nbr_args(h, pos_dev, species_dev);
        h->cand_valid = false;
        if ((r = launch_neighbor_build(na, st))) return fail(-1, "neighbor build launch failed (%d)", r);
        HIP_TRY(hipMemcpyAsync(h->counters_host, h->counters.p, sizeof(int) * CNT_COUNT, hipMemcpyDeviceToHost, st));
        HIP_TRY(hipStreamSynchronize(st));
        h->sticky_host[STICKY_EDGE_OVERFLOW] = 0;
        if (int t = check_traps(h)) return t;
        if (!h->counters_host[CNT_OVERFLOW]) return attempt ? 1 : 0;
        const long long need = (long long)(1.25 * (double)h->counters_host[CNT_E]) + 1024;
        if ((r = alloc_edges(h, need))) return r;
        if ((r = clear_devflags(h))) return r;
    }
    return fail(-34, "neighbor buffers still overflow after regrowing");
}

int32_t gamd_forces_async(gamd_handle* h, const float* pos_dev, const uint8_t* species_dev, const float* box,
                          float* out_norm_dev, float* out_denorm_dev, void* stream) {
    int r;
    if ((r = check_ready(h))) return r;
    if (!pos_dev || !box) return fail(-22, "null argument");
    if ((r = check_model_inputs(h, species_dev))) return r;
    DeviceGuard guard(h->dev);
    InitStream init((hipStream_t)stream);
    if ((r = set_box(h, box, (hipStream_t)stream))) return r;
    h->pending.active = false;
    return enqueue_forward(h, pos_dev, species_dev, out_norm_dev, out_denorm_dev, (hipStream_t)stream, nullptr, nullptr, nullptr);
}

int32_t gamd_sync_status(gamd_handle* h, void* stream) {
    if (!h) return fail(-22, "null handle");
    DeviceGuard guard(h->dev);
    InitStream init((hipStream_t)stream);
    bool resumed = false;
    for (int attempt = 0; attempt < 5; ++attempt) {
        HIP_TRY(hipStreamSynchronize((hipStream_t)stream));
        const bool cand_ovf = h->sticky_host[STICKY_CAND_OVERFLOW] != 0;
        const bool edge_ovf = h->counters_host[CNT_OVERFLOW] || h->sticky_host[STICKY_EDGE_OVERFLOW];
        if (int t = check_traps(h)) { h->pending.active = false; return t; }
        if (!cand_ovf && !edge_ovf) {
            h->pending.active = false;
            if (h->cfg.edge_dtype != GAMD_EDGE_F32 && h->sticky_host[STICKY_NONFINITE])
                return fail(-33, "non-finite forces with a reduced-precision edge dtype: an MFMA operand left the fp16 range "
                                 "(|x| > 65504) or the input positions are not finite");
            return resumed ? 1 : 0;
        }
        int r;
        long long need = 0;
        if (cand_ovf) {
            const long long seen = std::max<long long>(h->sticky_host[STICKY_NCAND], h->cand_cap);
            need = (long long)(1.25 * (double)seen) + 1024;
            if ((r = alloc_candidates(h, need))) return r;
        }
        if (edge_ovf) {
            const long long seen = std::max<long long>(h->counters_host[CNT_E], h->e_cap);
            need = (long long)(1.25 * (double)seen) + 1024;
            if ((r = alloc_edges(h, need))) return r;
            h->cand_valid = false;
        }
        h->sticky_host[STICKY_CAND_OVERFLOW] = 0;
        h->sticky_host[STICKY_EDGE_OVERFLOW] = 0;
        h->counters_host[CNT_OVERFLOW] = 0;
        int flags[DEVFLAG_COUNT] = {0, -1, 0, 0};
        HIP_TRY(hipMemcpyAsync(flags, h->devflags.p, sizeof(flags), hipMemcpyDeviceToHost, (hipStream_t)stream));
        HIP_TRY(hipStreamSynchronize((hipStream_t)stream));
        if ((r = clear_devflags(h))) return r;
        if (!h->pending.active)
            return fail(-34, "%s neighbour buffers overflowed; regrown to %lld, re-issue the call", cand_ovf ? "candidate" : "edge", need);
        const int at = flags[DEVFLAG_FROZEN_AT];
        if (at < 0) {
            h->pending.active = false;
            return fail(-34, "neighbour buffers overflowed inside an MD run but no integrator kernel recorded where it stopped");
        }
        if ((r = enqueue_md_steps(h, at / 2, (at & 1) != 0))) return r;
        resumed = true;
    }
    h->pending.active = false;
    return fail(-34, "neighbour buffers still overflow after regrowing four times");
}

int32_t gamd_forces(gamd_handle* h, const float* pos_dev, const uint8_t* species_dev, const float* box,
                    float* out_norm_dev, float* out_denorm_dev, void* stream) {
    for (int attempt = 0; attempt < 4; ++attempt) {
        int r = gamd_forces_async(h, pos_dev, species_dev, box, out_norm_dev, out_denorm_dev, stream);
        if (r) return r;
        r = gamd_sync_status(h, stream);
        if (r == 0) return attempt ? 1 : 0;
        if (r != -34) return r;
    }
    return fail(-34, "neighbour buffers still overflow after regrowing");
}

int32_t gamd_forces_host(gamd_handle* h, const float* pos_host, const uint8_t* species_dev, const float* box, float* out_host,
                         int32_t denormalize, void* stream) {
    int r;
    if ((r = check_ready(h))) return r;
    if (!pos_host || !out_host || !box) return fail(-22, "null argument");
    DeviceGuard guard(h->dev);
    const size_t bytes = sizeof(float) * 3 * (size_t)h->n;
    if (!h->host_in) {
        InitStream init((hipStream_t)stream);
        if (hipHostMalloc((void**)&h->host_in, bytes) != hipSuccess) { h->host_in = nullptr; return fail(-12, "pinned allocation failed"); }
        if (hipHostMalloc((void**)&h->host_out, bytes) != hipSuccess) {
            (void)hipHostFree(h->host_in);
            h->host_in = h->host_out = nullptr;
            return fail(-12, "pinned allocation failed");
        }
        if (h->pos_in.ensure(bytes, false)) return fail(-12, "device allocation failed");
    }
    std::memcpy(h->host_in, pos_host, bytes);
    for (int attempt = 0; attempt < 4; ++attempt) {
        HIP_TRY(hipMemcpyAsync(h->pos_in.p, h->host_in, bytes, hipMemcpyHostToDevice, (hipStream_t)stream));
        if ((r = gamd_forces_async(h, h->pos_in.as<float>(), species_dev, box, nullptr, denormalize ? h->f_den.as<float>() : nullptr, stream)))
            return r;
        HIP_TRY(hipMemcpyAsync(h->host_out, denormalize ? h->f_den.p : h->f_norm.p, bytes, hipMemcpyDeviceToHost, (hipStream_t)stream));
        r = gamd_sync_status(h, stream);
        if (r == 0) {
            std::memcpy(out_host, h->host_out, bytes);
            return attempt ? 1 : 0;
        }
        if (r != -34) return r;
    }
    return fail(-34, "neighbour buffers still overflow after regrowing");
}

int32_t gamd_forces_edges(gamd_handle* h, const float* pos_dev, const uint8_t* species_dev, const float* box,
                          const int32_t* centre_dev, const int32_t* neigh_dev, int64_t n_edges, float* out_norm_dev,
                          float* out_denorm_dev, void* stream) {
    int r;
    if ((r = check_ready(h))) return r;
    if (!pos_dev || !box || n_edges < 0 || (n_edges > 0 && (!centre_dev || !neigh_dev))) return fail(-22, "bad argument");
    if ((r = check_model_inputs(h, species_dev))) return r;
    if (n_edges > 0x7fff0000ll) return fail(-22, "edge list too long");
    DeviceGuard guard(h->dev);
    InitStream init((hipStream_t)stream);
    if ((r = set_box(h, box, (hipStream_t)stream))) return r;
    h->pending.active = false;
    int status = 0;
    const long long total = n_edges + (h->cfg.self_loop_mode ? h->n : 0) + (h->n_boxes > 1 ? 16ll * h->n_boxes : 0);
    if (total > h->e_cap) {
        if ((r = alloc_edges(h, total + total / 8 + 1024))) return r;
        status = 1;
    }
    if (h->tmp_eid.ensure(sizeof(int) * ((size_t)std::max<long long>(total, 1) + 64), false))
        return fail(-12, "edge scratch allocation failed");
    EdgeList el{centre_dev, neigh_dev, (long long)n_edges};
    if ((r = enqueue_forward(h, pos_dev, species_dev, out_norm_dev, out_denorm_dev, (hipStream_t)stream, nullptr, nullptr,
                             nullptr, &el)))
        return r;
    HIP_TRY(hipStreamSynchronize((hipStream_t)stream));
    h->sticky_host[STICKY_EDGE_OVERFLOW] = 0;
    if (h->counters_host[CNT_OVERFLOW]) {
        const int why = h->counters_host[CNT_OVERFLOW];
        h->counters_host[CNT_OVERFLOW] = 0;
        if ((r = clear_devflags(h))) return r;
        if (why == 2) return fail(-22, "edge list references an atom index outside [0, n_atoms)");
        return fail(-34, "edge buffers overflowed unexpectedly");
    }
    return status;
}

int32_t gamd_get_counts(gamd_handle* h, int64_t* n_edges, int64_t* n_pieces, int64_t* edge_capacity) {
    if (!h) return fail(-22, "null handle");
    if (n_edges) *n_edges = h->counters_host[CNT_E];
    if (n_pieces) *n_pieces = h->counters_host[CNT_PIECES];
    if (edge_capacity) *edge_capacity = h->e_cap;
    return 0;
}

int32_t gamd_get_skin_stats(gamd_handle* h, int64_t* n_rebuilds, int64_t* n_candidates, int64_t* candidate_capacity) {
    if (!h) return fail(-22, "null handle");
    if (n_rebuilds) *n_rebuilds = h->sticky_host[STICKY_REBUILDS];
    if (n_candidates) *n_candidates = h->sticky_host[STICKY_NCAND];
    if (candidate_capacity) *candidate_capacity = h->cand_cap;
    return 0;
}

int32_t gamd_debug_get(gamd_handle* h, int32_t what, void* host_out, size_t bytes) {
    if (!h || !host_out) return fail(-22, "null argument");
    DeviceGuard guard(h->dev);
    InitStream init(h->init_stream);
    HIP_TRY(hipDeviceSynchronize());
    const size_t n = (size_t)h->n;
    const size_t E = (size_t)std::min<long long>(h->counters_host[CNT_E], h->e_cap);
    const void* src = nullptr;
    size_t avail = 0;
    if (what == GAMD_DBG_PERM) { src = h->perm.p; avail = sizeof(int) * n; }
    else if (what == GAMD_DBG_ROWPTR) { src = h->row_ptr.p; avail = sizeof(int) * (n + 1); }
    else if (what == GAMD_DBG_COL) { src = h->col.p; avail = sizeof(int) * E; }
    else if (what == GAMD_DBG_EFRAG) { src = h->e_frag.p; avail = sizeof(float) * 4096 * (size_t)h->EHT * ((E + 31) / 32); }
    else if (what == GAMD_DBG_FEAT) {
        if (!h->cfg.keep_stages) return fail(-22, "FEAT needs keep_stages=1");
        src = h->feat_dbg.p; avail = sizeof(float) * 48 * E;
    } else if (what >= GAMD_DBG_H0 && what <= GAMD_DBG_H0 + h->L) {
        if (!h->cfg.keep_stages) return fail(-22, "H_l needs keep_stages=1");
        src = h->hbuf.as<float>() + (size_t)(what - GAMD_DBG_H0) * n * (size_t)h->H; avail = sizeof(float) * n * (size_t)h->H;
    } else if (what == GAMD_DBG_PARTIAL) {
        src = h->partial.p; avail = sizeof(float) * (size_t)h->H * (size_t)std::max(0, h->counters_host[CNT_PIECES]);
    } else if (what == GAMD_DBG_CYCLES) { src = h->tdbg.p; avail = sizeof(long long) * 16 * 8 * (size_t)h->n_cu;
    } else return fail(-22, "unknown debug tensor %d", what);
    if (bytes < avail) return fail(-22, "host buffer too small: %zu < %zu", bytes, avail);
    HIP_TRY(hipMemcpy(host_out, src, avail, hipMemcpyDeviceToHost));
    return 0;
}

int32_t gamd_md_run(gamd_handle* h, float* x_dev, float* v_dev, float* f_dev, const uint8_t* species_dev,
                    const float* box, const gamd_md_params* p, int64_t n_steps, void* stream) {
    int r;
    if ((r = check_ready(h))) return r;
    if (!x_dev || !v_dev || !f_dev || !box || !p) return fail(-22, "null argument");
    if (n_steps < 0 || n_steps > 0x3fffffff) return fail(-22, "n_steps out of range");
    if ((r = check_model_inputs(h, species_dev))) return r;
    DeviceGuard guard(h->dev);
    InitStream init((hipStream_t)stream);
    if ((r = set_box(h, box, (hipStream_t)stream))) return r;
    hipStream_t st = (hipStream_t)stream;
    MdArgs m{};
    m.n = h->n; m.x = x_dev; m.v = v_dev; m.f = f_dev;
    if (!(p->mass_amu > 0.f)) return fail(-22, "mass_amu must be positive");
    m.species = species_dev;
    m.inv_mass = 1.0f / p->mass_amu;
    m.inv_mass_h = p->mass_h_amu > 0.f ? 1.0f / p->mass_h_amu : 0.f;
    m.len = p->length_per_nm > 0.f ? p->length_per_nm : 10.0f;
    m.dt = p->dt_ps;
    const double kB = 0.00831446261815324;
    const double a = std::exp(-(double)p->gamma_per_ps * p->dt_ps);
    m.a = (float)a;
    m.b_len_kT = (float)(std::sqrt(1.0 - a * a) * (double)m.len * std::sqrt(kB * p->temperature_k));
    if ((r = fill_rigid(h, p->rigid_water, p->mass_amu, p->mass_h_amu, p->r_oh, p->r_hh, &m.use_rigid, &m.rigid)))
        return r;
    if (m.use_rigid && (r = check_rigid_layout(h, species_dev, st))) return r;
    for (int d = 0; d < 3; ++d) m.box[d] = box[d];
    m.bx = box_ref(h);
// ... 168 lines not shown
```

gamd_amd/csrc/gamd_common.h:

```cpp
#pragma once
#include <hip/hip_runtime.h>
#include <stdint.h>

typedef float f32x16 __attribute__((ext_vector_type(16)));
typedef float f32x4 __attribute__((ext_vector_type(4)));

#define GAMD_H 128
#define GAMD_TILE 32
#define GAMD_CHUNK 16
#define GAMD_WFRAG_FLOATS (GAMD_H * GAMD_H)

__device__ __forceinline__ int gamd_pi(int rho) {
    return 16 * ((rho >> 2) & 1) + (rho & 3) + 4 * (rho >> 3);
}

__device__ __forceinline__ f32x16 mfma32(float a, float b, f32x16 c) {
    return __builtin_amdgcn_mfma_f32_32x32x2f32(a, b, c, 0, 0, 0);
}

template <bool F2, typename WPtr>
__device__ __forceinline__ void gemm128_tile(WPtr W, int lane, const f32x16 (&X)[4], f32x16& acc, int tp) {
#pragma unroll
    for (int t = 0; t < 4; ++t) {
#pragma unroll
        for (int q = 0; q < 4; ++q) {
            const f32x4 w = W[((tp * 4 + t) * 4 + q) * 64 + lane];
#pragma unroll
            for (int j = 0; j < 4; ++j) {
                const float x = X[t][q * 4 + j];
                acc = F2 ? mfma32(x, w[j], acc) : mfma32(w[j], x, acc);
            }
        }
    }
}

template <bool F2, typename WPtr>
__device__ __forceinline__ void gemm128(WPtr W, int lane, const f32x16 (&X)[4], f32x16 (&acc)[4]) {
#pragma unroll
    for (int tp = 0; tp < 4; ++tp) gemm128_tile<F2>(W, lane, X, acc[tp], tp);
}

__device__ __forceinline__ float gamd_silu_hw(float x) {
    const float e = __builtin_amdgcn_exp2f(x * -1.4426950408889634f);
    return x * __builtin_amdgcn_rcpf(1.0f + e);
}
typedef float f32x2 __attribute__((ext_vector_type(2)));

#define GAMD_GELU_Q0 -9.999880791e-01f
#define GAMD_GELU_Q1 -1.151242852e+00f
#define GAMD_GELU_Q2 -4.586574435e-01f
#define GAMD_GELU_Q3 -5.355345458e-02f
#define GAMD_GELU_Q4 8.167289197e-03f
#define GAMD_GELU_Q5 -7.945232792e-04f
#define GAMD_GELU_Q6 3.589583139e-05f
__device__ __forceinline__ float gamd_gelu_hw(float x) {
    const float a = __builtin_amdgcn_fmed3f(fabsf(x), 0.0f, 6.0f);
    float q = fmaf(GAMD_GELU_Q6, a, GAMD_GELU_Q5);
    q = fmaf(q, a, GAMD_GELU_Q4);
    q = fmaf(q, a, GAMD_GELU_Q3);
    q = fmaf(q, a, GAMD_GELU_Q2);
    q = fmaf(q, a, GAMD_GELU_Q1);
    q = fmaf(q, a, GAMD_GELU_Q0);
    const float relu = x - __builtin_amdgcn_fmed3f(x, -3.0e38f, 0.0f);
    return fmaf(-a, __builtin_amdgcn_exp2f(q), relu);
}
typedef float gelu_f2 __attribute__((ext_vector_type(2)));
struct GeluCoef { gelu_f2 q[7]; };
__device__ __forceinline__ GeluCoef gelu_coef() {
    GeluCoef k;
    const float c[7] = {GAMD_GELU_Q0, GAMD_GELU_Q1, GAMD_GELU_Q2, GAMD_GELU_Q3, GAMD_GELU_Q4, GAMD_GELU_Q5, GAMD_GELU_Q6};
#pragma unroll
    for (int i = 0; i < 7; ++i) { k.q[i] = gelu_f2{c[i], c[i]}; asm volatile("" : "+v"(k.q[i])); }
    return k;
}
__device__ __forceinline__ gelu_f2 pk_fma(gelu_f2 a, gelu_f2 b, gelu_f2 c) {
    gelu_f2 d;
    asm("v_pk_fma_f32 %0, %1, %2, %3" : "=v"(d) : "v"(a), "v"(b), "v"(c));
    return d;
}
__device__ __forceinline__ gelu_f2 gelu_pair(gelu_f2 x, const GeluCoef& k) {
    const gelu_f2 a = {__builtin_amdgcn_fmed3f(fabsf(x[0]), 0.0f, 6.0f), __builtin_amdgcn_fmed3f(fabsf(x[1]), 0.0f, 6.0f)};
    gelu_f2 q = pk_fma(k.q[6], a, k.q[5]);
    q = pk_fma(q, a, k.q[4]);
    q = pk_fma(q, a, k.q[3]);
    q = pk_fma(q, a, k.q[2]);
    q = pk_fma(q, a, k.q[1]);
    q = pk_fma(q, a, k.q[0]);
    const gelu_f2 e = {__builtin_amdgcn_exp2f(q[0]), __builtin_amdgcn_exp2f(q[1])};
    const gelu_f2 relu = {x[0] - __builtin_amdgcn_fmed3f(x[0], -3.0e38f, 0.0f), x[1] - __builtin_amdgcn_fmed3f(x[1], -3.0e38f, 0.0f)};
    gelu_f2 r = {__builtin_fmaf(-a[0], e[0], relu[0]), __builtin_fmaf(-a[1], e[1], relu[1])};
    return r;
}

struct RbfGrid { int uniform; float c0, delta, A, B, C; };
__device__ __forceinline__ void gamd_rbf_chains(float d, int half, float gexp, const RbfGrid& g, float (&F)[24]) {
#pragma clang fp contract(off)
    const float s = 2.0f * g.delta;
    const float dh = d - (g.c0 + (half ? g.delta : 0.0f));
#pragma unroll
    for (int c = 0; c < 4; ++c) {
        const float u0 = dh - (float)(5 * c) * s;
        float v = __builtin_amdgcn_exp2f(gexp * (u0 * u0));
        float rho = __builtin_amdgcn_exp2f(fmaf(g.A, u0, g.B));
        F[2 + 5 * c] = v;
#pragma unroll
        for (int j = 1; j < 5; ++j) {
            v *= rho;
            F[2 + 5 * c + j] = v;
            if (j < 4) rho *= g.C;
        }
    }
}

__device__ __forceinline__ float gamd_remainder(float a, float b) {
    float m = fmodf(a, b);
    if (m != 0.0f && ((b < 0.0f) != (m < 0.0f))) m += b;
    return m;
}

__device__ __forceinline__ float gamd_min_image_wrapped(float d, float L, float halfL) {
    float t = d + halfL;
    if (t < 0.0f) t += L;
    else if (t >= L) t -= L;
    return t - halfL;
}

__device__ __forceinline__ f32x4 gamd_load_stream(const f32x4* p) { return __builtin_nontemporal_load(p); }

__device__ __forceinline__ float gamd_msg_acc(float hn, float e_emb, float prev) { return __builtin_fmaf(hn, e_emb, prev); }

__host__ __device__ __forceinline__ int gamd_tab16_pos(int f) {
    return 16 * (2 * (f >> 5) + ((f >> 4) & 1)) + 8 * ((f >> 2) & 1) + 4 * ((f >> 3) & 1) + (f & 3);
}

template <typename BPtr>
__device__ __forceinline__ void load_bias_chain(BPtr b, int half, f32x16 (&acc)[4]) {
#pragma unroll
    for (int t = 0; t < 4; ++t)
#pragma unroll
        for (int q = 0; q < 4; ++q) {
            const f32x4 v = *reinterpret_cast<const f32x4*>(&b[32 * t + 8 * q + 4 * half]);
#pragma unroll
            for (int j = 0; j < 4; ++j) acc[t][q * 4 + j] = v[j];
        }
}

__device__ __forceinline__ void load_row_chain(const float* __restrict__ row, int half, f32x16 (&X)[4]) {
#pragma unroll
    for (int t = 0; t < 4; ++t)
#pragma unroll
        for (int q = 0; q < 4; ++q) {
            const f32x4 v = *reinterpret_cast<const f32x4*>(row + 32 * t + 8 * q + 4 * half);
#pragma unroll
            for (int j = 0; j < 4; ++j) X[t][q * 4 + j] = v[j];
        }
}

__device__ __forceinline__ void store_row_chain(float* __restrict__ row, int half, const f32x16 (&X)[4]) {
#pragma unroll
    for (int t = 0; t < 4; ++t)
#pragma unroll
        for (int q = 0; q < 4; ++q) {
            f32x4 v;
#pragma unroll
            for (int j = 0; j < 4; ++j) v[j] = X[t][q * 4 + j];
            *reinterpret_cast<f32x4*>(row + 32 * t + 8 * q + 4 * half) = v;
        }
}

__device__ __forceinline__ float gamd_xhalf_sum(float v) {
    return v + __shfl_xor(v, 32, 64);
}

template <typename GPtr>
__device__ __forceinline__ void layernorm_chain(f32x16 (&X)[4], GPtr gamma, GPtr beta, int half, float eps) {
    float s = 0.f;
#pragma unroll
    for (int t = 0; t < 4; ++t)
#pragma unroll
        for (int r = 0; r < 16; ++r) s += X[t][r];
    const float mean = gamd_xhalf_sum(s) * (1.0f / 128.0f);
    float v = 0.f;
#pragma unroll
    for (int t = 0; t < 4; ++t)
#pragma unroll
        for (int r = 0; r < 16; ++r) {
            const float d = X[t][r] - mean;
            v += d * d;
        }
    const float var = gamd_xhalf_sum(v) * (1.0f / 128.0f);
    const float rstd = 1.0f / sqrtf(var + eps);
#pragma unroll
    for (int t = 0; t < 4; ++t)
#pragma unroll
        for (int q = 0; q < 4; ++q) {
            const f32x4 g = *reinterpret_cast<const f32x4*>(&gamma[32 * t + 8 * q + 4 * half]);
            const f32x4 b = *reinterpret_cast<const f32x4*>(&beta[32 * t + 8 * q + 4 * half]);
#pragma unroll
            for (int j = 0; j < 4; ++j) X[t][q * 4 + j] = (X[t][q * 4 + j] - mean) * rstd * g[j] + b[j];
        }
}

template <int NW = 8>
__device__ __forceinline__ void gamd_stage_weight(const float* __restrict__ gw, float* ldsbuf, int wave, unsigned lane16) {
    asm volatile("" : "+v"(lane16));
#pragma unroll
    for (int k = 0; k < 64 / NW; ++k) {
        const int chunk = k * NW + wave;
        const char* base = reinterpret_cast<const char*>(gw) + chunk * 1024;
        __builtin_amdgcn_global_load_lds(
            (const __attribute__((address_space(1))) void*)(base + lane16),
            (__attribute__((address_space(3))) void*)(ldsbuf + chunk * 256), 16, 0, 0);
    }
}

#pragma clang diagnostic push
#pragma clang diagnostic ignored "-Winline-asm"

template <int NW = 8>
__device__ __forceinline__ void gamd_stage_weight_raw(const float* __restrict__ gw, float* ldsbuf, int wave, unsigned lane16) {
    const unsigned lds0 = (unsigned)(size_t)(__attribute__((address_space(3))) float*)ldsbuf;
#pragma unroll
    for (int k = 0; k < 64 / NW; ++k) {
        const int chunk = k * NW + wave;
        asm volatile("s_mov_b32 m0, %2\n\ts_nop 0\n\tglobal_load_lds_dwordx4 %0, %1"
                     ::"v"(lane16), "s"(reinterpret_cast<const char*>(gw) + chunk * 1024), "s"(lds0 + chunk * 1024u)
                     : "memory", "m0");
    }
}

template <int NW = 8>
__device__ __forceinline__ void gamd_stage_weight_raw_contig(const float* __restrict__ gw, float* ldsbuf, int wave, unsigned lane16) {
    static_assert((64 / NW) % 4 == 0, "whole groups of four KiB-sized copies per wave");
    int woff = wave * (64 / NW) * 1024;
    asm volatile("" : "+s"(woff));
    const char* g0 = reinterpret_cast<const char*>(gw) + woff;
    const unsigned l0 = (unsigned)(size_t)(__attribute__((address_space(3))) float*)ldsbuf + (unsigned)woff;
#pragma unroll
    for (int h = 0; h < 64 / NW / 4; ++h)
        asm volatile("s_mov_b32 m0, %2\n\ts_nop 0\n\t"
                     "global_load_lds_dwordx4 %0, %1\n\t"
                     "global_load_lds_dwordx4 %0, %1 offset:1024\n\t"
                     "global_load_lds_dwordx4 %0, %1 offset:2048\n\t"
                     "global_load_lds_dwordx4 %0, %1 offset:3072"
                     ::"v"(lane16), "s"(g0 + h * 4096), "s"(l0 + h * 4096u)
                     : "memory", "m0");
}

#pragma clang diagnostic pop

struct WQuarter { f32x4 w[16]; };

__device__ __forceinline__ void load_wquarter(const float* __restrict__ Wp, int quarter, int lane, WQuarter& o) {
    const f32x4* W = reinterpret_cast<const f32x4*>(Wp) + (size_t)quarter * 16 * 64 + lane;
#pragma unroll
    for (int i = 0; i < 16; ++i) o.w[i] = W[i * 64];
}

template <bool F2 = false>
__device__ __forceinline__ void gemm_quarter(const WQuarter& wq, const f32x16 (&X)[4], f32x16& acc) {
#pragma unroll
    for (int t = 0; t < 4; ++t)
#pragma unroll
        for (int q = 0; q < 4; ++q)
#pragma unroll
            for (int j = 0; j < 4; ++j)
                acc = F2 ? mfma32(X[t][q * 4 + j], wq.w[t * 4 + q][j], acc) : mfma32(wq.w[t * 4 + q][j], X[t][q * 4 + j], acc);
}

__device__ __forceinline__ f32x16 load_slice(const float* __restrict__ row, int quarter, int half) {
    f32x16 v;
#pragma unroll
    for (int q = 0; q < 4; ++q) {
        const f32x4 x = *reinterpret_cast<const f32x4*>(row + 32 * quarter + 8 * q + 4 * half);
#pragma unroll
        for (int j = 0; j < 4; ++j) v[q * 4 + j] = x[j];
    }
    return v;
}

__device__ __forceinline__ void store_slice(float* __restrict__ row, int quarter, int half, const f32x16& v) {
#pragma unroll
    for (int q = 0; q < 4; ++q) {
        f32x4 x;
#pragma unroll
        for (int j = 0; j < 4; ++j) x[j] = v[q * 4 + j];
        *reinterpret_cast<f32x4*>(row + 32 * quarter + 8 * q + 4 * half) = x;
    }
}

template <int NB, int XLDW>
__device__ __forceinline__ void exchange_blocks(float* xbuf, int quarter, int slot, int half, const f32x16 (&mine)[NB],
                                                f32x16 (&X)[NB][4]) {
    __syncthreads();
#pragma unroll
    for (int b = 0; b < NB; ++b) store_slice(xbuf + slot * XLDW + 128 * b, quarter, half, mine[b]);
    __syncthreads();
#pragma unroll
    for (int b = 0; b < NB; ++b) load_row_chain(xbuf + slot * XLDW + 128 * b, half, X[b]);
}

constexpr int GAMD_XLD = 132;

__device__ __forceinline__ void exchange(float* xbuf, int quarter, int slot, int half, const f32x16& mine, f32x16 (&X)[4]) {
    __syncthreads();
    store_slice(xbuf + slot * GAMD_XLD, quarter, half, mine);
    __syncthreads();
    load_row_chain(xbuf + slot * GAMD_XLD, half, X);
}

template <typename GPtr>
__device__ __forceinline__ void layernorm_chain_centered(f32x16 (&X)[4], GPtr gamma, GPtr beta, int half, float eps,
                                                         float inv_width = 1.0f / 128.0f) {
    float vt[4];
#pragma unroll
    for (int t = 0; t < 4; ++t) {
        vt[t] = 0.f;
#pragma unroll
        for (int r = 0; r < 16; ++r) vt[t] = fmaf(X[t][r], X[t][r], vt[t]);
    }
    const float var = gamd_xhalf_sum((vt[0] + vt[1]) + (vt[2] + vt[3])) * inv_width;
    const float rstd = 1.0f / sqrtf(var + eps);
#pragma unroll
    for (int t = 0; t < 4; ++t)
#pragma unroll
        for (int q = 0; q < 4; ++q) {
            const f32x4 g = *reinterpret_cast<const f32x4*>(&gamma[32 * t + 8 * q + 4 * half]);
            const f32x4 b = *reinterpret_cast<const f32x4*>(&beta[32 * t + 8 * q + 4 * half]);
#pragma unroll
            for (int j = 0; j < 4; ++j) X[t][q * 4 + j] = fmaf(X[t][q * 4 + j] * rstd, g[j], b[j]);
        }
}

__device__ __forceinline__ void gamd_xcd_range(int n_tiles, int block, int n_blocks, int& first, int& end, int& step) {
    const int nx = 8;
    if (n_blocks % nx != 0 || n_blocks < nx) { first = block; end = n_tiles; step = n_blocks; return; }
    const int x = block % nx, w = block / nx, per = n_blocks / nx;
    const int q = n_tiles / nx, rem = n_tiles % nx;
    const int lo = x * q + (x < rem ? x : rem);
    const int cnt = q + (x < rem ? 1 : 0);
    first = lo + w; end = lo + cnt; step = per;
}

#define GAMD_CHECK_LAUNCH() do { hipError_t e__ = hipGetLastError(); if (e__ != hipSuccess) return (int)e__; } while (0)
```

gamd_amd/csrc/gamd_internal.h:

```cpp
#pragma once
#include <hip/hip_runtime.h>
#include <stdint.h>
#include <atomic>
#include "gamd_common.h"

enum { CNT_E = 0, CNT_PIECES = 1, CNT_OVERFLOW = 2, CNT_TILES = 3, CNT_REBUILD = 4, CNT_NCAND = 5,
       CNT_CAND_MAX = 6,
       CNT_COUNT = 8 };
enum { STICKY_EDGE_OVERFLOW = 0, STICKY_CAND_OVERFLOW = 1, STICKY_REBUILDS = 2, STICKY_NCAND = 3,
       STICKY_NONFINITE = 4,
       STICKY_CHECK_CODE = 5, STICKY_CHECK_VALUE = 6, STICKY_CHECK_LINE = 7,
       STICKY_COUNT = 8 };
enum { GAMD_CHK_CELL = 101, GAMD_CHK_CAND = 102, GAMD_CHK_EDGE_POS = 103, GAMD_CHK_PERM = 104, GAMD_CHK_ENC_SRC = 111, GAMD_CHK_ENC_DST = 112,
       GAMD_CHK_CONV_SRC = 121, GAMD_CHK_CONV_DST = 122, GAMD_CHK_PIECE = 123, GAMD_CHK_NODE_PIECES = 131, GAMD_CHK_INJECTED = 199 };
#ifdef GAMD_CHECKED
template <typename T>
__device__ __forceinline__ T gamd_chk_range(int* sticky, T v, long long lo, long long hi, int code, int line) {
    if ((long long)v >= lo && (long long)v <= hi) return v;
    if (sticky && sticky[STICKY_CHECK_CODE] == 0) {
        sticky[STICKY_CHECK_VALUE] = (int)v;
        sticky[STICKY_CHECK_LINE] = line;
        __threadfence_system();
        sticky[STICKY_CHECK_CODE] = code;
    }
    return (T)lo;
}
#define GAMD_CHK_RANGE(sticky, v, lo, hi, code) gamd_chk_range((sticky), (v), (long long)(lo), (long long)(hi), (code), __LINE__)
#else
#define GAMD_CHK_RANGE(sticky, v, lo, hi, code) (v)
#endif
enum { DEVFLAG_FROZEN = 0, DEVFLAG_FROZEN_AT = 1, DEVFLAG_REBUILDS = 2, DEVFLAG_COUNT = 4 };

constexpr int GAMD_MAX_DEVICES = 64;
struct PerDeviceOnce { std::atomic<bool> done[GAMD_MAX_DEVICES] = {}; };
template <typename... Fn>
inline int gamd_allow_dynamic_lds(PerDeviceOnce& once, int bytes, Fn... fns) {
    int dev = 0;
    hipError_t e = hipGetDevice(&dev);
    if (e != hipSuccess) return (int)e;
    if (dev >= 0 && dev < GAMD_MAX_DEVICES && once.done[dev].load(std::memory_order_relaxed)) return 0;
    const void* list[] = {(const void*)fns...};
    for (const void* fn : list) {
        e = hipFuncSetAttribute(fn, hipFuncAttributeMaxDynamicSharedMemorySize, bytes);
        if (e != hipSuccess) return (int)e;
    }
    if (dev >= 0 && dev < GAMD_MAX_DEVICES) once.done[dev].store(true, std::memory_order_relaxed);
    return 0;
}

struct BoxRef {
    int n_boxes, n_per_box;
    float inv_npb;
    const float4* boxes;
};
__device__ __forceinline__ int gamd_box_of(const BoxRef& r, int i) {
    int q = (int)(((float)i + 0.5f) * r.inv_npb);
    const int rem = i - q * r.n_per_box;
    q += rem >= r.n_per_box ? 1 : (rem < 0 ? -1 : 0);
    return q;
}
struct BoxDims { float bx, by, bz, hx, hy, hz; };
__device__ __forceinline__ BoxDims gamd_box_dims(const BoxRef& r, const float (&box)[3], const float (&half)[3], int box_id) {
    if (r.n_boxes <= 1) return BoxDims{box[0], box[1], box[2], half[0], half[1], half[2]};
    const float4 b = r.boxes[3 * box_id], h = r.boxes[3 * box_id + 1];
    return BoxDims{b.x, b.y, b.z, h.x, h.y, h.z};
}

struct NbrArgs {
    int n;
    BoxRef bx;
    int* box_shift;
    int flavour;
    float box[3], half[3];
    float rc, rc2;
    int nc[3], ncell;
    int ncell_cap;
    long long e_cap;
    const float* pos;
    const uint8_t* species;
    const float* feat;
    int self_loop;
    int* devflags;
    float4* pos_w;
    float4* pos_s;
    int* cell_of;
    int* cell_cnt;
    int* cell_fill;
    int* cell_start;
    int* perm;
    int* inv_perm;
    int* deg;
    int* row_ptr;
    int* na_excl;
    int* col;
    int* erow;
    int* chunk_piece;
    unsigned* chunk_mask;
    int* counters;
    int* counters_next;
    int* sticky;
    const int* gate;
    float skin_half2;
    int force_rebuild;
    float4* ref_pos;
    int* cand_deg;
    int* cand_ptr;
    int* cand_col;
    long long cand_cap;
    int cand_stride;
    int use_small;
    int cells_one_wg;
    float rc_build, rc2_build;
};
struct MdArgs;
struct MdFuse { const MdArgs* md; int do_second, do_first; };
int launch_neighbor_build(const NbrArgs& a, hipStream_t st);
int launch_neighbor_skin(const NbrArgs& a, hipStream_t st, const MdFuse* fuse = nullptr);
int launch_csr_from_edges(const NbrArgs& a, const int* centre, const int* neigh, long long n_edges, int* tmp_eid,
                          hipStream_t st);

struct EncArgs {
    const int* counters;
    const int* devflags;
    const float4* pos_s;
    const int* col;
    const int* erow;
    const int* bond_nbr;
    const int* perm;
    const int* row_ptr;
    int self_loop;
    int zero_row;
    float box[3], half[3];
    BoxRef bx;
    float length_mean, length_std, gamma;
    float ln_inv_width, ln_n_pad;
    int n_feat;
    int n_ksteps;
    const float* centers;
    RbfGrid rbf;
    const float* w1p;
    const float* w2p;
    const float* w3p;
    const float* b1; const float* b2; const float* b3;
    const float* ln_g; const float* ln_b;
    float* e_frag;
    long long e_cap;
    float* feat_dbg;
    int* sticky;
    int e_format;
};
__device__ __forceinline__ bool gamd_is_appended_loop(const EncArgs& a, long long x, int src, int dst) {
    if (!a.self_loop || src == a.zero_row) return false;
    const long long row_end = a.row_ptr[dst + 1];
    return x == row_end - 1 || (x + 1 < row_end && a.col[x + 1] == a.zero_row);
}

__device__ __forceinline__ BoxDims gamd_edge_box(const EncArgs& a, int dst) {
    return gamd_box_dims(a.bx, a.box, a.half, a.bx.n_boxes > 1 ? gamd_box_of(a.bx, dst) : 0);
}
int launch_edge_encode(const EncArgs& a, int n_blocks, hipStream_t st);
int launch_edge_encode_small(const EncArgs& a, int n_blocks, hipStream_t st);
int launch_edge_encode_bf16(const EncArgs& a, int n_blocks, hipStream_t st);
int launch_edge_encode_f16x3(const EncArgs& a, int n_blocks, hipStream_t st);
int launch_edge_encode_wide(const EncArgs& a, int eht, int n_blocks, hipStream_t st);
int launch_edge_encode_wide_d(const EncArgs& a, int eht, int dt, int n_blocks, hipStream_t st);

struct ConvEdgeArgs {
    const int* counters;
    const int* devflags;
    const int* col;
    const int* erow;
    const int* chunk_piece;
    const unsigned* chunk_mask;
    const float* e_frag;
    const float* hn;
    const float* S;
    const float* D;
    const float* w1p; const float* w2p; const float* w3p; const float* w4p;
    const float* w16p;
    const float* b1; const float* b3; const float* b4;
    float* partial;
    long long e_cap;
    int zero_row;
    long long* tdbg;
    int* sticky;
    long long piece_cap;
    float* emb_out;
};
int launch_conv_edge(const ConvEdgeArgs& a, int n_blocks, hipStream_t st);
int launch_conv_edge_bf16(const ConvEdgeArgs& a, int n_blocks, hipStream_t st);
int launch_conv_edge_small(const ConvEdgeArgs& a, int n_blocks, hipStream_t st);
int launch_conv_edge_small_wide(const ConvEdgeArgs& a, int eht, int ht, int n_blocks, hipStream_t st);
int launch_conv_edge_f16x3(const ConvEdgeArgs& a, int n_blocks, hipStream_t st);
int launch_conv_edge_wide(const ConvEdgeArgs& a, int eht, int ht, int n_blocks, hipStream_t st);
int launch_conv_edge_wide16(const ConvEdgeArgs& a, int eht, int ht, int n_blocks, hipStream_t st);
int launch_conv_edge_wide_d(const ConvEdgeArgs& a, int eht, int ht, int dt, int n_blocks, hipStream_t st);
int launch_conv_edge_f16x3_wide(const ConvEdgeArgs& a, int eht, int ht, int n_blocks, hipStream_t st);
int launch_conv_edge_bf16_wide(const ConvEdgeArgs& a, int eht, int ht, int n_blocks, hipStream_t st);

struct EdgeUpdateArgs {
    const int* counters;
    const int* devflags;
    long long e_cap;
    const float* emb;
    const float* ln_g; const float* ln_b;
    float ln_inv_width, ln_n_pad;
    float* e_frag_out;
};
int launch_edge_update(const EdgeUpdateArgs& a, int ht, int n_blocks, hipStream_t st);

struct NodeLayerW {
    const float* ln_g; const float* ln_b;
    const float* wsp; const float* wdp; const float* wpdp;
    const float* bS;
    const float* bP;
    const float* wpep;
    const float* wphip;
    const float* bphi;
};
struct NodeArgs {
    const int* counters;
    const int* devflags;
    int* sticky;
    int n;
    int mode;
    int l0_gate;
    const float4* pos_s;
    const float* node_emb;
    const float* enc_w; const float* enc_b;
    const int* row_ptr; const int* na_excl; const int* deg;
    const float* partial;
    long long piece_cap;
    const float* h_in;
    const float* P_in;
    NodeLayerW post;
    NodeLayerW pre;
    const float* dec_w1p; const float* dec_b1; const float* dec_w2; const float* dec_b2;
    float scale, shift;
    float ln_inv_width, ln_n_pad;
    int norm_bn;
    int f16x3;
    const int* perm;
    float* h_out;
    float* hn_out; float* S_out; float* D_out; float* P_out;
    int hn_perm;
    int tab16;
    float* forces_norm;
    float* forces;
    long long* tdbg;
};
int launch_node(const NodeArgs& a, hipStream_t st);
int launch_node_wide(const NodeArgs& a, int ht, hipStream_t st);
int launch_node_wide_d(const NodeArgs& a, int ht, int dt, hipStream_t st);

struct RigidWater { float m_o, m_h, ra, rb, rc; };
struct MdCom {
    int enabled;
    int blocks;
    double* partial;
};
struct MdArgs {
    int n;
    float* x; float* v;
    const float* f;
    const uint8_t* species;
    float inv_mass, inv_mass_h;
    float len;
    float dt;
    float a, b_len_kT;
    float box[3];
    BoxRef bx;
    int use_rigid;
    RigidWater rigid;
    unsigned long long seed; unsigned long long step;
    int* devflags;
    int step_index;
    MdCom com;
};
int launch_baoab_first(const MdArgs& a, hipStream_t st);
int launch_baoab_second(const MdArgs& a, hipStream_t st);
int launch_baoab_second_com(const MdArgs& a, hipStream_t st);

struct NhcArgs {
    int n;
    float* x; float* v;
    const float* f;
    const uint8_t* species;
    float mass, mass_h;
    float len;
    float dt;
    float box[3];
    BoxRef bx;
    int use_rigid;
    RigidWater rigid;
    double kT, freq, ndf;
    int M, n_c, n_ys;
    double w[5];
    double* state;
    double* partial;
    int n_blocks;
    int* devflags;
    int step_index;
    MdCom com;
};
int launch_com_partial(const MdCom& com, const float* v, const uint8_t* species, float inv_mass, float inv_mass_h, int n,
                       const BoxRef& bx, const int* devflags, int by_molecule, hipStream_t st);
int launch_nhc_first(const NhcArgs& a, hipStream_t st);
int launch_nhc_second(const NhcArgs& a, hipStream_t st);
```

gamd_amd/csrc/node.hip:

```cpp
#include "gamd_common.h"
#include "gamd_internal.h"

namespace {

typedef _Float16 nf16x8 __attribute__((ext_vector_type(8)));
typedef _Float16 nf16x2 __attribute__((ext_vector_type(2)));
typedef float nf32x2 __attribute__((ext_vector_type(2)));

constexpr int NT = 16;
constexpr int XLD = 136;

__device__ __forceinline__ f32x4 mfma16(float a, float b, f32x4 c) {
    return __builtin_amdgcn_mfma_f32_16x16x4f32(a, b, c, 0, 0, 0);
}

struct WHalf { f32x4 w[8]; };
__device__ __forceinline__ void load_whalf(const float* __restrict__ Wp, int w, int lane, int half, WHalf& h) {
    const f32x4* W = reinterpret_cast<const f32x4*>(Wp) + (size_t)w * 16 * 64 + lane;
#pragma unroll
    for (int o = 0; o < 2; ++o)
#pragma unroll
        for (int b = 0; b < 4; ++b) h.w[o * 4 + b] = W[(o * 8 + 4 * half + b) * 64];
}

__device__ __forceinline__ void gemm16_half(const WHalf& h, int half, const f32x4 (&XB)[8], f32x4 (&acc)[2]) {
#pragma unroll
    for (int b = 0; b < 4; ++b)
#pragma unroll
        for (int r = 0; r < 4; ++r) {
            acc[0] = mfma16(h.w[b][r], XB[4 * half + b][r], acc[0]);
            acc[1] = mfma16(h.w[4 + b][r], XB[4 * half + b][r], acc[1]);
        }
}

struct XSplit { nf16x8 h[4], l[4]; };
__device__ __forceinline__ void split16(const f32x4 (&XB)[8], XSplit& s) {
#pragma unroll
    for (int m = 0; m < 4; ++m)
#pragma unroll
        for (int j = 0; j < 8; j += 2) {
            const f32x4& q = XB[2 * m + (j >> 2)];
            const nf32x2 x = {q[j & 3], q[(j & 3) + 1]};
            const nf16x2 hi = __builtin_convertvector(x, nf16x2);
            const nf32x2 rem = x - __builtin_convertvector(hi, nf32x2);
            const nf16x2 lo = __builtin_convertvector(rem, nf16x2);
            s.h[m][j] = hi[0]; s.h[m][j + 1] = hi[1];
            s.l[m][j] = lo[0]; s.l[m][j + 1] = lo[1];
        }
}
__device__ __forceinline__ void gemm16_half_f16(const WHalf& h, int half, const XSplit& X, f32x4 (&acc)[2]) {
#pragma unroll
    for (int mm = 0; mm < 2; ++mm) {
        const int m = 2 * half + mm;
#pragma unroll
        for (int o = 0; o < 2; ++o) {
            const nf16x8 wh = __builtin_bit_cast(nf16x8, h.w[o * 4 + mm * 2]), wl = __builtin_bit_cast(nf16x8, h.w[o * 4 + mm * 2 + 1]);
            acc[o] = __builtin_amdgcn_mfma_f32_16x16x32_f16(wh, X.l[m], acc[o], 0, 0, 0);
            acc[o] = __builtin_amdgcn_mfma_f32_16x16x32_f16(wl, X.h[m], acc[o], 0, 0, 0);
            acc[o] = __builtin_amdgcn_mfma_f32_16x16x32_f16(wh, X.h[m], acc[o], 0, 0, 0);
        }
    }
}

template <bool NEXT, bool F16, typename XT>
__device__ __forceinline__ void gemm16(const float* W, const float* next, WHalf& wn, const XT& XB, f32x4 (&acc)[2], int w, int lane) {
    WHalf cur = wn;
    asm volatile("" ::: "memory");
    load_whalf(W, w, lane, 1, wn);
    asm volatile("" ::: "memory");
    if constexpr (F16) gemm16_half_f16(cur, 0, XB, acc); else gemm16_half(cur, 0, XB, acc);
    __builtin_amdgcn_sched_barrier(0);
    cur = wn;
    if (NEXT) {
        asm volatile("" ::: "memory");
        load_whalf(next, w, lane, 0, wn);
        asm volatile("" ::: "memory");
    }
    if constexpr (F16) gemm16_half_f16(cur, 1, XB, acc); else gemm16_half(cur, 1, XB, acc);
    __builtin_amdgcn_sched_barrier(0);
}

__device__ __forceinline__ void load16(const float* __restrict__ row, int w, int g, f32x4 (&v)[2]) {
    v[0] = *reinterpret_cast<const f32x4*>(row + 32 * w + 4 * g);
    v[1] = *reinterpret_cast<const f32x4*>(row + 32 * w + 16 + 4 * g);
}
__device__ __forceinline__ void store16(float* __restrict__ row, int w, int g, const f32x4 (&v)[2]) {
    *reinterpret_cast<f32x4*>(row + 32 * w + 4 * g) = v[0];
    *reinterpret_cast<f32x4*>(row + 32 * w + 16 + 4 * g) = v[1];
}

__device__ __forceinline__ void exchange16(float* xbuf, int w, int a, int g, const f32x4 (&mine)[2], f32x4 (&XB)[8]) {
    __syncthreads();
    store16(xbuf + a * XLD, w, g, mine);
    __syncthreads();
#pragma unroll
    for (int blk = 0; blk < 8; ++blk) XB[blk] = *reinterpret_cast<const f32x4*>(xbuf + a * XLD + 16 * blk + 4 * g);
}

typedef _Float16 nf16x4 __attribute__((ext_vector_type(4)));
__device__ __forceinline__ nf16x4 cvt16x4(const f32x4& v) {
    const nf16x2 lo = __builtin_convertvector(nf32x2{v[0], v[1]}, nf16x2), hi = __builtin_convertvector(nf32x2{v[2], v[3]}, nf16x2);
    return nf16x4{lo[0], lo[1], hi[0], hi[1]};
}
__device__ __forceinline__ void store16_h(_Float16* __restrict__ row, int w, int g, const f32x4 (&v)[2]) {
    *reinterpret_cast<nf16x4*>(row + 32 * w + 4 * g) = cvt16x4(v[0]);
    *reinterpret_cast<nf16x4*>(row + 32 * w + 16 + 4 * g) = cvt16x4(v[1]);
}
__device__ __forceinline__ void store16_tab(_Float16* __restrict__ row, int w, int g, const f32x4 (&v)[2]) {
    *reinterpret_cast<nf16x4*>(row + 32 * w + 8 * (g & 1) + 4 * (g >> 1)) = cvt16x4(v[0]);
    *reinterpret_cast<nf16x4*>(row + 32 * w + 16 + 8 * (g & 1) + 4 * (g >> 1)) = cvt16x4(v[1]);
}

__device__ __forceinline__ float group_sum(float v) {
    v += __shfl_xor(v, 16, 64);
    return v + __shfl_xor(v, 32, 64);
}

template <bool F16>
__global__ void __launch_bounds__(256, 3) k_node(NodeArgs a) {
    __shared__ __attribute__((aligned(16))) float xbuf[NT * XLD];
    __shared__ float obuf[4][NT][3];
    __shared__ float red[2][4][NT];

    if (a.counters[CNT_OVERFLOW] || a.devflags[DEVFLAG_FROZEN]) return;
    if (a.mode == 0 && a.l0_gate && a.counters[CNT_REBUILD] == 0) return;

    const int lane = threadIdx.x & 63, la = lane & 15, g = lane >> 4;
    const int w = __builtin_amdgcn_readfirstlane(threadIdx.x >> 6);
    const int atom_raw = blockIdx.x * NT + la;
    const bool valid = atom_raw < a.n;
    const int atom = valid ? atom_raw : a.n - 1;
    const size_t row = (size_t)atom * GAMD_H;

#ifdef GAMD_PROFILING
    long long tm[16] = {0, 0, 0, 0, 0, 0, 0, 0, 0, 0, 0, 0, 0, 0, 0, 0};
#define NMARK(I) do { if (a.tdbg) tm[I] = (long long)__builtin_readcyclecounter(); } while (0)
#else
#define NMARK(I) do { } while (0)
#endif
    NMARK(0);
    f32x4 XB[8];
    XSplit XS;
#define GEMM16(NEXT, W, NXT) do { if constexpr (F16) gemm16<NEXT, true>(W, NXT, wn, XS, mine, w, lane); \
                                  else gemm16<NEXT, false>(W, NXT, wn, XB, mine, w, lane); } while (0)
#define SPLIT16() do { if constexpr (F16) split16(XB, XS); } while (0)
    f32x4 mine[2];
    WHalf wn;

    if (a.mode == 0) {
        if (a.node_emb) {
            load16(a.node_emb, w, g, mine);
        } else {
            const float f = a.pos_s[atom].w;
            f32x4 ww[2];
            load16(a.enc_w, w, g, ww);
            load16(a.enc_b, w, g, mine);
#pragma unroll
            for (int o = 0; o < 2; ++o)
#pragma unroll
                for (int r = 0; r < 4; ++r) mine[o][r] = f * ww[o][r] + mine[o][r];
        }
        if (valid) store16(a.h_out + row, w, g, mine);
        load_whalf(a.pre.wsp, w, lane, 0, wn);
    } else {
        const int rp0 = a.row_ptr[atom], dg = a.deg[atom];
        const int na_incl = a.na_excl[atom] + ((dg > 0 && (rp0 % GAMD_CHUNK) != 0) ? 1 : 0);
        const int p0 = rp0 / GAMD_CHUNK + na_incl;
        const int np = dg > 0 ? ((rp0 + dg - 1) / GAMD_CHUNK - rp0 / GAMD_CHUNK + 1) : 0;
        (void)GAMD_CHK_RANGE(a.sticky, (long long)p0 + np, 0, a.piece_cap, GAMD_CHK_NODE_PIECES);
        mine[0] = f32x4{0.f, 0.f, 0.f, 0.f};
        mine[1] = mine[0];
        f32x4 p_in[2], h_res[2];
        load16(a.P_in + row, w, g, p_in);
        for (int k0 = 0; __any(k0 < np); k0 += 8) {
            f32x4 pc[8][2];
#pragma unroll
            for (int k = 0; k < 8; ++k) {
                const int kk = (k0 + k < np) ? k0 + k : (np > 0 ? np - 1 : 0);
                load16(a.partial + (size_t)(np > 0 ? p0 + kk : 0) * GAMD_H, w, g, pc[k]);
            }
#pragma unroll
            for (int k = 0; k < 8; ++k)
                if (k0 + k < np) { mine[0] += pc[k][0]; mine[1] += pc[k][1]; }
        }
        NMARK(1);
        asm volatile("" ::: "memory");
        load_whalf(a.post.wpep, w, lane, 0, wn);
        exchange16(xbuf, w, la, g, mine, XB);
        SPLIT16();
        NMARK(2);
        mine[0] = p_in[0]; mine[1] = p_in[1];
        GEMM16(true, a.post.wpep, a.post.wphip);
        NMARK(3);
#pragma unroll
        for (int o = 0; o < 2; ++o)
#pragma unroll
            for (int r = 0; r < 4; ++r) mine[o][r] = gamd_silu_hw(mine[o][r]);
        exchange16(xbuf, w, la, g, mine, XB);
        SPLIT16();
        NMARK(4);
        load16(a.post.bphi, w, g, mine);
        load16(a.h_in + row, w, g, h_res);
        GEMM16(true, a.post.wphip, a.mode != 2 ? a.pre.wsp : a.dec_w1p);
        mine[0] += h_res[0]; mine[1] += h_res[1];
        if (valid) store16(a.h_out + row, w, g, mine);
        NMARK(5);
    }

    if (a.mode != 2) {
        float mean = 0.f, rstd = 1.0f;
        if (!a.norm_bn) {
            float ps = 0.f;
#pragma unroll
            for (int o = 0; o < 2; ++o)
#pragma unroll
                for (int r = 0; r < 4; ++r) ps += mine[o][r];
            ps = group_sum(ps);
            if (g == 0) red[0][w][la] = ps;
            __syncthreads();
            mean = ((red[0][0][la] + red[0][1][la]) + (red[0][2][la] + red[0][3][la])) * a.ln_inv_width;
            float pv = 0.f;
#pragma unroll
            for (int o = 0; o < 2; ++o)
#pragma unroll
                for (int r = 0; r < 4; ++r) { const float d = mine[o][r] - mean; pv += d * d; }
            pv = group_sum(pv);
            if (g == 0) red[1][w][la] = pv;
            __syncthreads();
            const float var = (((red[1][0][la] + red[1][1][la]) + (red[1][2][la] + red[1][3][la])) - a.ln_n_pad * (mean * mean)) * a.ln_inv_width;
            rstd = 1.0f / sqrtf(var + 1e-5f);
        }
        {
            f32x4 gg[2], bb[2];
            load16(a.pre.ln_g, w, g, gg);
            load16(a.pre.ln_b, w, g, bb);
#pragma unroll
            for (int o = 0; o < 2; ++o)
#pragma unroll
                for (int r = 0; r < 4; ++r) mine[o][r] = (mine[o][r] - mean) * rstd * gg[o][r] + bb[o][r];
        }
        if (valid && a.tab16) store16_h(reinterpret_cast<_Float16*>(a.hn_out) + row, w, g, mine);
        else if (valid && !a.hn_perm) store16(a.hn_out + row, w, g, mine);
        exchange16(xbuf, w, la, g, mine, XB);
        SPLIT16();
        NMARK(6);
        if (a.hn_perm) {
#pragma unroll
            for (int k = 0; k < 2; ++k) {
                const int idx = k * 256 + threadIdx.x, at = idx >> 5, c = idx & 31;
                const float* xr = xbuf + at * XLD + c;
                const f32x4 v = {xr[0], xr[32], xr[64], xr[96]};
                const int atom_k = blockIdx.x * NT + at;
                if (atom_k < a.n) *reinterpret_cast<f32x4*>(a.hn_out + (size_t)atom_k * GAMD_H + 4 * c) = v;
            }
        }
        load16(a.pre.bS, w, g, mine);
        GEMM16(true, a.pre.wsp, a.pre.wdp);
        if (valid && a.tab16) store16_tab(reinterpret_cast<_Float16*>(a.S_out) + row, w, g, mine);
        else if (valid) store16(a.S_out + row, w, g, mine);
        NMARK(7);
        mine[0] = f32x4{0.f, 0.f, 0.f, 0.f};
        mine[1] = mine[0];
        GEMM16(true, a.pre.wdp, a.pre.wpdp);
        if (valid && a.tab16) store16_tab(reinterpret_cast<_Float16*>(a.D_out) + row, w, g, mine);
        else if (valid) store16(a.D_out + row, w, g, mine);
        NMARK(8);
        load16(a.pre.bP, w, g, mine);
        GEMM16(false, a.pre.wpdp, nullptr);
        if (valid) store16(a.P_out + row, w, g, mine);
        NMARK(9);
#ifdef GAMD_PROFILING
        if (a.tdbg && a.mode == 1 && lane == 0 && blockIdx.x < 512) {
            long long* o = a.tdbg + ((size_t)blockIdx.x * 4 + w) * 16;
            for (int i = 0; i < 16; ++i) o[i] = tm[i];
        }
#endif
    } else {
        exchange16(xbuf, w, la, g, mine, XB);
        SPLIT16();
        load16(a.dec_b1, w, g, mine);
        GEMM16(false, a.dec_w1p, nullptr);
        float o3[3] = {0.f, 0.f, 0.f};
#pragma unroll
        for (int o = 0; o < 2; ++o) {
            const int f0 = 32 * w + 16 * o + 4 * g;
            f32x4 gl;
#pragma unroll
            for (int r = 0; r < 4; ++r) gl[r] = gamd_gelu_hw(mine[o][r]);
#pragma unroll
            for (int c = 0; c < 3; ++c) {
                const f32x4 ww = *reinterpret_cast<const f32x4*>(a.dec_w2 + c * GAMD_H + f0);
#pragma unroll
                for (int r = 0; r < 4; ++r) o3[c] += ww[r] * gl[r];
            }
        }
#pragma unroll
        for (int c = 0; c < 3; ++c) o3[c] = group_sum(o3[c]);
        if (g == 0) {
#pragma unroll
            for (int c = 0; c < 3; ++c) obuf[w][la][c] = o3[c];
        }
        __syncthreads();
        if (w == 0 && g == 0 && valid) {
            const int orig = a.perm[atom];
#pragma unroll
            for (int c = 0; c < 3; ++c) {
                const float v = ((obuf[0][la][c] + obuf[1][la][c]) + (obuf[2][la][c] + obuf[3][la][c])) + a.dec_b2[c];
                a.forces_norm[3 * (size_t)orig + c] = v;
                if (a.forces) a.forces[3 * (size_t)orig + c] = v * a.scale + a.shift;
                if (!(fabsf(v) <= 3.0e38f)) a.sticky[STICKY_NONFINITE] = 1;
            }
        }
    }
}

#undef NMARK
#undef GEMM16
#undef SPLIT16

}

int launch_node(const NodeArgs& a, hipStream_t st) {
    const int nb = (a.n + NT - 1) / NT;
    if (a.f16x3) hipLaunchKernelGGL((k_node<true>), dim3(nb), dim3(256), 0, st, a);
    else hipLaunchKernelGGL((k_node<false>), dim3(nb), dim3(256), 0, st, a);
    GAMD_CHECK_LAUNCH();
    return 0;
}
```

gamd_amd/engine.py:

```python
from __future__ import annotations

import ctypes as C
from typing import Dict, Optional, Sequence, Tuple, Union

import numpy as np
import torch

from . import _lib
from ._lib import GamdConfig, GamdMdParams, GamdNhcParams, check
from .weights import ModelConfig, infer_config, validate_state_dict

ArrayLike = Union[np.ndarray, torch.Tensor]

KIND = {"lj": 0, "water": 1, "dynbox": 1}
FLAVOUR = {"jaxmd": 0, "torch": 1}
SELF_LOOP = {"dgl07_noop": 0, "append_zero_feature_loops": 1}
KSEL_FORCE_GENERIC_WIDTH = 1


def _box3(box) -> np.ndarray:
    b = np.asarray(box, dtype=np.float64).reshape(-1)
    if b.size == 1:
        b = np.repeat(b, 3)
    if b.size != 3:
        raise ValueError("box must be a scalar or 3 values")
    return b.astype(np.float32)


def _boxes(box, n_boxes: int) -> np.ndarray:
    b = np.asarray(box, dtype=np.float64)
    if b.ndim == 0 or b.size == 1 or (b.ndim == 1 and b.size == 3):
        return np.tile(_box3(b), (n_boxes, 1))
    if b.ndim == 2 and b.shape == (n_boxes, 3):
        return b.astype(np.float32)
    if (b.ndim == 1 and b.size == n_boxes) or (b.ndim == 2 and b.shape == (n_boxes, 1)):
        return np.repeat(b.reshape(-1).astype(np.float32)[:, None], 3, axis=1)
    raise ValueError(f"box must be a scalar, 3 values, [{n_boxes}, 1] or [{n_boxes}, 3] ({n_boxes} boxes)")


class GamdForce:

    def __init__(self, state_dict: Dict[str, torch.Tensor], n_atoms: int, box, cutoff: float,
                 bond: Optional[np.ndarray] = None, scaler: Tuple[float, float] = (0.0, 1.0),
                 nbr_flavour: str = "jaxmd", device: int = 0, keep_stages: bool = False,
                 edge_capacity: int = 0, cfg: Optional[ModelConfig] = None, edge_dtype: str = "f32",
                 neighbor_skin: float = 0.0, self_loop_mode: str = "dgl07_noop", kernel_select: int = 0,
                 small_tile_limit: int = 0, n_boxes: int = 1):
        self._h = C.c_void_p()
        self._lib = _lib.load()
        if not torch.cuda.is_available():
            raise _lib.GamdError("GamdForce needs a HIP device (torch.cuda.is_available() is False); "
                                 "there is no CPU fallback")
        cfg = cfg or infer_config(state_dict)
        if (not 1 <= cfg.encoding_size <= 256 or not 1 <= cfg.edge_embedding_dim <= 256 or not 1 <= cfg.hidden_dim <= 256
                or cfg.n_rbf not in (0, 40)):
            raise ValueError("the gfx950 kernels cover encoding_size / edge_embedding_dim / hidden_dim up to 256 "
                             "and the RBF expansion on (40 centres) or off "
                             f"(got enc={cfg.encoding_size} hidden={cfg.hidden_dim} edge={cfg.edge_embedding_dim} "
                             f"n_rbf={cfg.n_rbf})")
        validate_state_dict(state_dict, cfg)
        self.cfg = cfg
        self.n = int(n_atoms)
        self.n_boxes = max(1, int(n_boxes))
        self.n_total = self.n * self.n_boxes
        self.device = torch.device("cuda", device)
        self.box = _box3(box)
        self.cutoff = float(cutoff)
        c = GamdConfig()
        c.n_boxes = self.n_boxes
        c.n_atoms, c.kind, c.n_layers = self.n, KIND[cfg.kind], cfg.conv_layer
        c.use_bond, c.nbr_flavour, c.device = int(cfg.use_bond), FLAVOUR[nbr_flavour], device
        c.cutoff = self.cutoff
        for d in range(3):
            c.box[d] = float(self.box[d])
        c.edge_capacity, c.keep_stages = int(edge_capacity), int(keep_stages)
        c.edge_dtype = {"f32": 0, "bf16": 1, "f16x3": 2}[edge_dtype]
        c.encoding_size, c.edge_embedding_dim, c.hidden_dim = cfg.encoding_size, cfg.edge_embedding_dim, cfg.hidden_dim
        c.no_expand_edge = int(cfg.n_rbf == 0)
        c.neighbor_skin = float(neighbor_skin)
        if self_loop_mode not in SELF_LOOP:
            raise ValueError(f"self_loop_mode must be one of {sorted(SELF_LOOP)}")
        c.self_loop_mode = SELF_LOOP[self_loop_mode]
        c.kernel_select, c.small_tile_limit = int(kernel_select), int(small_tile_limit)
        self.edge_dtype = edge_dtype
        check(self._lib.gamd_create(C.byref(c), C.byref(self._h)), "gamd_create")
        self.keep_stages = keep_stages
        for name, t in state_dict.items():
            if name.endswith("num_batches_tracked"):
                continue
            a = np.ascontiguousarray(t.detach().cpu().numpy().astype(np.float32))
            shape = (C.c_int64 * a.ndim)(*a.shape)
            check(self._lib.gamd_load_weight(self._h, name.encode(), a.ctypes.data_as(C.c_void_p), shape, a.ndim),
                  f"gamd_load_weight({name})")
        check(self._lib.gamd_finalize_weights(self._h), "gamd_finalize_weights")
        self.set_scaler(*scaler)
        if cfg.use_bond:
            if bond is None:
                raise ValueError("use_bond model needs the bond list")
            b = np.ascontiguousarray(np.asarray(bond, dtype=np.int32))
            check(self._lib.gamd_set_bonds(self._h, b.ctypes.data_as(C.c_void_p), b.shape[0]), "gamd_set_bonds")
        self._feat = None
        self._out = torch.empty((self.n_total, 3), dtype=torch.float32, device=self.device)
        self._out_den = torch.empty((self.n_total, 3), dtype=torch.float32, device=self.device)
        self.last_status = 0

    def close(self):
        if getattr(self, "_h", None) is not None and self._h.value:
            self._lib.gamd_destroy(self._h)
            self._h = C.c_void_p()

    def __del__(self):
        try:
            self.close()
        except Exception:
            pass

    def set_scaler(self, mean, var):
        self.scaler_mean = np.asarray(mean, dtype=np.float64).reshape(-1)[:1]
        self.scaler_var = np.asarray(var, dtype=np.float64).reshape(-1)[:1]
        check(self._lib.gamd_set_scaler(self._h, float(self.scaler_mean[0]), float(self.scaler_var[0])),
              "gamd_set_scaler")

    def _stream(self):
        return C.c_void_p(torch.cuda.current_stream(self.device).cuda_stream)

    def _dev_pos(self, pos: ArrayLike) -> torch.Tensor:
        if isinstance(pos, np.ndarray):
            pos = torch.from_numpy(np.ascontiguousarray(pos, dtype=np.float32))
        pos = pos.to(device=self.device, dtype=torch.float32).contiguous()
        if tuple(pos.shape) == (self.n_boxes, self.n, 3):
            pos = pos.view(self.n_total, 3)
        if tuple(pos.shape) != (self.n_total, 3):
            raise ValueError(f"pos must be [{self.n_total}, 3]" + (f" or [{self.n_boxes}, {self.n}, 3]" if self.n_boxes > 1 else "")
                             + f", got {tuple(pos.shape)}")
        return pos

    def _md_state(self, *ts):
        for t in ts:
            if not (t.is_cuda and t.dtype == torch.float32 and t.is_contiguous()
                    and tuple(t.shape) in ((self.n_total, 3), (self.n_boxes, self.n, 3))):
                raise ValueError(f"x, v, f must be contiguous float32 CUDA tensors of shape [{self.n_total}, 3]")

    def _dev_species(self, species) -> Optional[torch.Tensor]:
        if species is None:
            self._set_features(None)
            return None
        if isinstance(species, np.ndarray):
            species = torch.from_numpy(species)
        key = None
        if not species.is_cuda:
            c = species.detach().reshape(-1).contiguous()
            key = (str(c.dtype), c.numel(), hash(c.view(torch.uint8).numpy().tobytes()), torch.cuda.current_stream(self.device).cuda_stream)
            hit = getattr(self, "_species_cache", None)
            if hit is not None and hit[0] == key:
                self._set_features(hit[2])
                return hit[1]
        s = species.reshape(-1).to(device=self.device)
        if s.numel() == self.n and self.n_boxes > 1:
            s = s.repeat(self.n_boxes)
        if s.numel() != self.n_total:
            raise ValueError("species must have one entry per atom")
        feat = s.to(torch.float32).contiguous() if s.dtype.is_floating_point and self.cfg.kind != "lj" else None
        self._set_features(feat)
        flags = (s != 0).to(torch.uint8).contiguous()
        self._species_prev = getattr(self, "_species_cache", None)
        self._species_cache = (key, flags, feat)
        return flags

    def _set_features(self, feat: Optional[torch.Tensor]) -> None:
        if feat is None and self._feat is None:
            return
        self._feat = feat
        check(self._lib.gamd_set_node_features(self._h, C.c_void_p(feat.data_ptr()) if feat is not None else None),
              "gamd_set_node_features")

    def _box_arg(self, box):
        b = _boxes(self.box if box is None else box, self.n_boxes)
        return (C.c_float * (3 * self.n_boxes))(*[float(x) for x in b.reshape(-1)])

    def forward(self, pos: ArrayLike, box=None, species=None, denormalize: bool = False,
                inplace: bool = False) -> torch.Tensor:
        p = self._dev_pos(pos)
        s = self._dev_species(species)
        st = self._lib.gamd_forces(self._h, C.c_void_p(p.data_ptr()),
                                   C.c_void_p(s.data_ptr()) if s is not None else None,
                                   self._box_arg(box), C.c_void_p(self._out.data_ptr()),
                                   C.c_void_p(self._out_den.data_ptr()), self._stream())
        self.last_status = check(st, "gamd_forces")
        out = self._out_den if denormalize else self._out
        return out if inplace else out.clone()

    __call__ = forward

    def forward_host(self, pos: np.ndarray, box=None, species=None, denormalize: bool = False) -> np.ndarray:
        pos = np.asarray(pos)
        if pos.shape == (self.n_boxes, self.n, 3):
            pos = pos.reshape(self.n_total, 3)
        if pos.shape != (self.n_total, 3):
            raise ValueError(f"pos must be [{self.n_total}, 3], got {tuple(pos.shape)}")
        p32 = np.ascontiguousarray(pos, dtype=np.float32)
        if getattr(self, "_host_out", None) is None:
            self._host_out = np.empty((self.n_total, 3), dtype=np.float32)
        s = self._dev_species(species)
        st = self._lib.gamd_forces_host(self._h, p32.ctypes.data_as(C.c_void_p), C.c_void_p(s.data_ptr()) if s is not None else None,
                                        self._box_arg(box), self._host_out.ctypes.data_as(C.c_void_p), 1 if denormalize else 0,
                                        self._stream())
        self.last_status = check(st, "gamd_forces_host")
        return self._host_out

    def forward_edges(self, pos: ArrayLike, edge_idx, box=None, species=None, denormalize: bool = False,
                      inplace: bool = False) -> torch.Tensor:
        p = self._dev_pos(pos)
        s = self._dev_species(species)
        if isinstance(edge_idx, np.ndarray):
            edge_idx = torch.from_numpy(edge_idx)
        e = edge_idx.to(device=self.device, dtype=torch.int32).contiguous()
        if e.dim() != 2 or e.shape[0] != 2:
            raise ValueError("edge_idx must be [2, E]")
        st = self._lib.gamd_forces_edges(self._h, C.c_void_p(p.data_ptr()),
                                         C.c_void_p(s.data_ptr()) if s is not None else None, self._box_arg(box),
                                         C.c_void_p(e[0].data_ptr()), C.c_void_p(e[1].data_ptr()), int(e.shape[1]),
                                         C.c_void_p(self._out.data_ptr()), C.c_void_p(self._out_den.data_ptr()),
                                         self._stream())
        self.last_status = check(st, "gamd_forces_edges")
        out = self._out_den if denormalize else self._out
        return out if inplace else out.clone()

    def build_neighbors(self, pos: ArrayLike, box=None, species=None) -> int:
        p = self._dev_pos(pos)
        s = self._dev_species(species)
        st = self._lib.gamd_build_neighbors(self._h, C.c_void_p(p.data_ptr()),
                                            C.c_void_p(s.data_ptr()) if s is not None else None,
                                            self._box_arg(box), self._stream())
        return check(st, "gamd_build_neighbors")

    def counts(self) -> Tuple[int, int, int]:
        e, p, c = C.c_int64(), C.c_int64(), C.c_int64()
        check(self._lib.gamd_get_counts(self._h, C.byref(e), C.byref(p), C.byref(c)), "gamd_get_counts")
        return e.value, p.value, c.value

    def skin_stats(self) -> Tuple[int, int, int]:
        r, c, cap = C.c_int64(), C.c_int64(), C.c_int64()
        check(self._lib.gamd_get_skin_stats(self._h, C.byref(r), C.byref(c), C.byref(cap)), "gamd_get_skin_stats")
        return r.value, c.value, cap.value

    def _dbg(self, what: int, shape, dtype) -> np.ndarray:
        out = np.empty(shape, dtype=dtype)
        check(self._lib.gamd_debug_get(self._h, what, out.ctypes.data_as(C.c_void_p), out.nbytes), "gamd_debug_get")
        return out

    def debug_partial(self) -> np.ndarray:
        return self._dbg(6, (self.counts()[1], 128 * ((self.cfg.encoding_size + 127) // 128)), np.float32)

    def debug_perm(self) -> np.ndarray:
        return self._dbg(0, (self.n_total,), np.int32)

    def debug_csr(self) -> Tuple[np.ndarray, np.ndarray]:
        e = self.counts()[0]
        return self._dbg(1, (self.n_total + 1,), np.int32), self._dbg(2, (e,), np.int32)

    def debug_edges(self) -> np.ndarray:
        perm = self.debug_perm().astype(np.int64)
        row_ptr, col = self.debug_csr()
        dst = np.repeat(np.arange(self.n_total), np.diff(row_ptr))
        real = col < self.n_total
        return np.stack([perm[dst[real]], perm[col[real]]])

    def debug_edge_rows(self) -> np.ndarray:
        return self.debug_csr()[1] < self.n_total

    def debug_e(self) -> np.ndarray:
        e = self.counts()[0]
        nt = (e + 31) // 32
        nb = (self.cfg.edge_embedding_dim + 127) // 128
        if self.edge_dtype in ("f16x3", "bf16"):
            raw = self._dbg(3, (nt, nb, 4096), np.float32)
            if self.edge_dtype == "f16x3":
                v = raw.view(np.float16).reshape(nt, nb, 4, 2, 2, 64, 8).astype(np.float32)
                val = v[:, :, :, :, 0] + v[:, :, :, :, 1]
            else:
                u16 = raw.reshape(-1).view(np.uint16)[:nt * nb * 4096].reshape(nt, nb, 4, 2, 64, 8)
                val = (u16.astype(np.uint32) << 16).view(np.float32)
            lane = np.arange(64)
            slot, half = lane & 31, lane >> 5
            pi = 16 * ((slot >> 2) & 1) + (slot & 3) + 4 * (slot >> 3)
            rows = (np.arange(nt)[:, None] * 32 + pi[None, :])
            out = np.zeros((nt * 32, 128 * nb), dtype=np.float32)
            for blk in range(nb):
                for t in range(4):
                    for u in range(2):
                        for j in range(8):
                            r = 8 * u + j
                            feat = 128 * blk + 32 * t + (r & 3) + 8 * (r >> 2) + 4 * half
                            out[rows, feat[None, :]] = val[:, blk, t, u, :, j]
            return out[:e, :self.cfg.edge_embedding_dim]
        frag = self._dbg(3, (nt, nb, 4, 4, 64, 4), np.float32)
        lane = np.arange(64)
        slot, half = lane & 31, lane >> 5
        pi = 16 * ((slot >> 2) & 1) + (slot & 3) + 4 * (slot >> 3)
        out = np.zeros((nt * 32, 128 * nb), dtype=np.float32)
        rows = (np.arange(nt)[:, None] * 32 + pi[None, :])
        for b in range(nb):
            for t in range(4):
                for q in range(4):
                    for j in range(4):
                        feat = 128 * b + 32 * t + 8 * q + 4 * half + j
                        out[rows, feat[None, :]] = frag[:, b, t, q, :, j]
        return out[:e, :self.cfg.edge_embedding_dim]

    def debug_feat(self, n_feat: int) -> np.ndarray:
        e = self.counts()[0]
        return self._dbg(4, (e, 48), np.float32)[:, :n_feat]

    def debug_h(self, layer: int) -> np.ndarray:
        hp = 128 * ((self.cfg.encoding_size + 127) // 128)
        hs = self._dbg(16 + layer, (self.n_total, hp), np.float32)[:, :self.cfg.encoding_size]
        out = np.empty_like(hs)
        out[self.debug_perm()] = hs
        return out

# ... 93 lines not shown
```

include/gamd_hip.h:

```cpp
#ifndef GAMD_HIP_H
#define GAMD_HIP_H

#include <stdint.h>
#include <stddef.h>

#ifdef __cplusplus
extern "C" {
#endif

typedef struct gamd_handle gamd_handle;

enum { GAMD_EDGE_F32 = 0, GAMD_EDGE_BF16 = 1, GAMD_EDGE_F16X3 = 2 };

enum { GAMD_KIND_LJ = 0, GAMD_KIND_WATER = 1 };
enum { GAMD_NBR_JAXMD = 0, GAMD_NBR_TORCH = 1 };

typedef struct gamd_config {
    int32_t n_atoms;
    int32_t kind;
    int32_t n_layers;
    int32_t use_bond;
    int32_t nbr_flavour;
    int32_t device;
    float cutoff;
    float box[3];
    int64_t edge_capacity;
    int32_t keep_stages;
    int32_t edge_dtype;
    int32_t encoding_size;
    int32_t edge_embedding_dim;
    int32_t hidden_dim;
    int32_t no_expand_edge;
    float neighbor_skin;
    int32_t self_loop_mode;
    int32_t kernel_select;
    int32_t small_tile_limit;
    int32_t n_boxes;
} gamd_config;
enum { GAMD_SELF_LOOP_DGL07_NOOP = 0, GAMD_SELF_LOOP_APPEND_ZERO_FEATURE = 1 };
enum { GAMD_KSEL_FORCE_GENERIC_WIDTH = 1, GAMD_KSEL_FORCE_HALF_QUANTUM = 2 };

const char* gamd_version(void);
const char* gamd_last_error(void);

int32_t gamd_create(const gamd_config* cfg, gamd_handle** out);
int32_t gamd_destroy(gamd_handle* h);

int32_t gamd_load_weight(gamd_handle* h, const char* name, const float* data, const int64_t* shape, int32_t ndim);
int32_t gamd_finalize_weights(gamd_handle* h);

int32_t gamd_set_scaler(gamd_handle* h, double mean, double var);

int32_t gamd_set_bonds(gamd_handle* h, const int32_t* bonds, int64_t n_bonds);

int32_t gamd_forces_async(gamd_handle* h, const float* pos_dev, const uint8_t* species_dev, const float* box,
                          float* out_norm_dev, float* out_denorm_dev, void* stream);

int32_t gamd_set_node_features(gamd_handle* h, const float* feat_dev);

int32_t gamd_sync_status(gamd_handle* h, void* stream);

int32_t gamd_get_device_flags(gamd_handle* h, int32_t flags[4]);

int32_t gamd_forces(gamd_handle* h, const float* pos_dev, const uint8_t* species_dev, const float* box,
                    float* out_norm_dev, float* out_denorm_dev, void* stream);

int32_t gamd_forces_host(gamd_handle* h, const float* pos_host, const uint8_t* species_dev, const float* box, float* out_host,
                         int32_t denormalize, void* stream);

int32_t gamd_forces_edges(gamd_handle* h, const float* pos_dev, const uint8_t* species_dev, const float* box,
                          const int32_t* centre_dev, const int32_t* neigh_dev, int64_t n_edges,
                          float* out_norm_dev, float* out_denorm_dev, void* stream);

int32_t gamd_build_neighbors(gamd_handle* h, const float* pos_dev, const uint8_t* species_dev, const float* box,
                             void* stream);

int32_t gamd_get_counts(gamd_handle* h, int64_t* n_edges, int64_t* n_pieces, int64_t* edge_capacity);

int32_t gamd_get_skin_stats(gamd_handle* h, int64_t* n_rebuilds, int64_t* n_candidates, int64_t* candidate_capacity);

enum {
    GAMD_DBG_PERM = 0,
    GAMD_DBG_ROWPTR = 1,
    GAMD_DBG_COL = 2,
    GAMD_DBG_EFRAG = 3,
    GAMD_DBG_FEAT = 4,
    GAMD_DBG_CYCLES = 5,
    GAMD_DBG_PARTIAL = 6,
    GAMD_DBG_H0 = 16
};
int32_t gamd_debug_get(gamd_handle* h, int32_t what, void* host_out, size_t bytes);

typedef struct gamd_md_params {
    float dt_ps;
    float mass_amu;
    float temperature_k;
    float gamma_per_ps;
    uint64_t seed;
    uint64_t first_step;
    float mass_h_amu;
    float length_per_nm;
    int32_t rigid_water;
    float r_oh, r_hh;
    int32_t remove_cm_motion;
} gamd_md_params;
int32_t gamd_md_run(gamd_handle* h, float* x_dev, float* v_dev, float* f_dev, const uint8_t* species_dev,
                    const float* box, const gamd_md_params* p, int64_t n_steps, void* stream);

typedef struct gamd_nhc_params {
    float dt_ps;
    float mass_amu;
    float temperature_k;
    float frequency_per_ps;
    int32_t chain_length;
    int32_t num_mts;
    int32_t num_yoshidasuzuki;
    int32_t reset;
    double ndf;
    float mass_h_amu;
    float length_per_nm;
    int32_t rigid_water;
    float r_oh, r_hh;
    int32_t remove_cm_motion;
} gamd_nhc_params;
int32_t gamd_md_run_nhc(gamd_handle* h, float* x_dev, float* v_dev, float* f_dev, const uint8_t* species_dev,
                        const float* box, const gamd_nhc_params* p, double* chain_state_dev, int64_t n_steps, void* stream);

int32_t gamd_profile(gamd_handle* h, const float* pos_dev, const uint8_t* species_dev, const float* box,
                     float* out_norm_dev, void* stream, char* names, size_t names_bytes, float* ms, int32_t max_ms,
                     int32_t* n_out);

int32_t gamd_timing_enable(gamd_handle* h, int32_t enable);
int32_t gamd_timing_read(gamd_handle* h, void* stream, double* total_ms, int64_t* n_launches);
int32_t gamd_timing_read_stages(gamd_handle* h, void* stream, double total_ms[3], int64_t n_launches[3]);
int32_t gamd_timing_read_steps(gamd_handle* h, void* stream, float* step_ms, int64_t max_steps, int64_t* n_steps);

#ifdef __cplusplus
}
#endif
#endif
```

Before: 3.222 million atom-steps/s.

## Specialise layer-0 conv using constant node embedding to drop per-edge node gathers

For the LJ model, all nodes in layer 0 share one embedding, so its normalised features and the S/D projections are constants. A new L0 conv-edge path uses a constant S+D bias instead of gathering rows per source and destination, skips the hn gather and the fourth GEMM, and swaps in the first edge-MLP weights. The last linear map is folded into a host-precomputed matrix m0, with a per-node bias c0 scaled by the real-neighbour count, applied in the node kernel. This cuts per-edge memory gathers and one 128x128 GEMM per edge in layer 0. In exchange it adds padding/sentinel handling and host-side weight folding that could introduce precision differences.

Result: faster. 3.380 million atom-steps/s (median of 6 runs) (+4.9%).

```diff
diff --git a/gamd_amd/csrc/conv_edge.hip b/gamd_amd/csrc/conv_edge.hip
--- a/gamd_amd/csrc/conv_edge.hip
+++ b/gamd_amd/csrc/conv_edge.hip
@@ -5,7 +5,7 @@
 
 namespace {
 
-constexpr int CONV_LDS_FLOATS = 2 * GAMD_WFRAG_FLOATS + 3 * 128;
+constexpr int conv_lds_floats(bool l0) { return 2 * GAMD_WFRAG_FLOATS + 3 * 128; }
 
 template <bool F2, typename Post, typename Mid>
 __device__ __forceinline__ void gemm128_post(const f32x4* W, int lane, const f32x16 (&X)[4], f32x16 (&acc)[4], Post post, Mid mid) {
@@ -48,15 +48,16 @@
         }
 }
 
-template <bool TIME>
+template <bool TIME, bool L0>
 __global__ void __launch_bounds__(512, 2) k_conv_edge(ConvEdgeArgs a) {
     if (a.devflags[DEVFLAG_FROZEN]) return;
     extern __shared__ __attribute__((aligned(16))) float lds[];
-    float* buf0 = lds;
-    float* buf1 = lds + GAMD_WFRAG_FLOATS;
-    float* vb1 = buf1 + GAMD_WFRAG_FLOATS;
+    float* buf0 = lds + (L0 ? 3 * 128 : 0);
+    float* buf1 = buf0 + GAMD_WFRAG_FLOATS;
+    float* vb1 = L0 ? lds : buf1 + GAMD_WFRAG_FLOATS;
     float* vb3 = vb1 + 128;
     float* vb4 = vb3 + 128;
+    float* vSD0 = vb4;
 
     const int tid = threadIdx.x, lane = tid & 63, slot = lane & 31, half = lane >> 5;
     const int wave = __builtin_amdgcn_readfirstlane(tid >> 6);
@@ -83,7 +84,11 @@
     long long tprev = 0;
 #define TMARK(i) do { if (TIME) { const long long tn__ = (long long)__builtin_readcyclecounter(); tacc[i] += tn__ - tprev; tprev = tn__; } } while (0)
 
-    if (tid < 128) { vb1[tid] = a.b1[tid]; vb3[tid] = a.b3[tid]; vb4[tid] = a.b4[tid]; }
+    if (tid < 128) {
+        vb1[tid] = a.b1[tid]; vb3[tid] = a.b3[tid];
+        if (L0) vSD0[tid] = a.S[tid] + a.D[tid];
+        else vb4[tid] = a.b4[tid];
+    }
     stage(a.w1p, buf0);
 
     f32x16 RA[4], RB[4], RC[4];
@@ -101,8 +106,10 @@
     int src = 0, dst = 0;
     {
         const int x = tile * GAMD_TILE + gamd_pi(slot);
-        if (active && x < E) { src = GAMD_CHK_RANGE(a.sticky, a.col[x], 0, a.zero_row, GAMD_CHK_CONV_SRC); dst = GAMD_CHK_RANGE(a.sticky, a.erow[x], 0, a.zero_row, GAMD_CHK_CONV_DST); }
-        else { src = a.zero_row; dst = a.zero_row; }
+        if (active && x < E) {
+            src = GAMD_CHK_RANGE(a.sticky, a.col[x], 0, a.zero_row, GAMD_CHK_CONV_SRC);
+            if (!L0) dst = GAMD_CHK_RANGE(a.sticky, a.erow[x], 0, a.zero_row, GAMD_CHK_CONV_DST);
+        } else { src = a.zero_row; dst = a.zero_row; }
         if (active) load_e_tile(a.e_frag, tile, lane, RA);
     }
     asm volatile("" ::"v"(src), "v"(dst));
@@ -155,6 +162,82 @@
     };
 #define FENCE() __builtin_amdgcn_sched_barrier(0)
 
+    if constexpr (L0) {
+    for (int it = 0; it < n_iter; ++it) {
+        const int x0 = tile * GAMD_TILE + 16 * half;
+        int nvalid = E - x0;
+        nvalid = !active ? 0 : (nvalid >= 16 ? 16 : (nvalid <= 0 ? 0 : nvalid));
+        const int tile_n = tile_of(it + 1);
+        const bool active_n = tile_n < n_tiles;
+        int src_n = a.zero_row;
+        float* const bx = (it & 1) ? buf1 : buf0;
+        float* const by = (it & 1) ? buf0 : buf1;
+
+        if (active) {
+            load_bias_chain(vb1, half, RB);
+            TMARK(0);
+            gemm128_post<false>((const f32x4*)bx, lane, RA, RB,
+                                [&](int tp, int g) { RB[tp][g] = gamd_silu_hw(RB[tp][g]); },
+                                [&]() { FENCE(); piece_stores(); stage(a.w2p, by); FENCE(); });
+            TMARK(1);
+        } else {
+            piece_stores();
+            stage(a.w2p, by);
+        }
+        phase_barrier<0>();
+        TMARK(2);
+        unsigned mask = 0;
+        int p0 = 0;
+        if (active) { load_bias_chain(vSD0, half, RA); FENCE(); }
+        if (active) {
+            mask = a.chunk_mask[tile * 2 + half];
+            p0 = GAMD_CHK_RANGE(a.sticky, a.chunk_piece[tile * 2 + half], 0, a.piece_cap - 17, GAMD_CHK_PIECE);
+        }
+        if (active_n) {
+            const int xn = tile_n * GAMD_TILE + gamd_pi(slot);
+            if (xn < E) src_n = GAMD_CHK_RANGE(a.sticky, a.col[xn], 0, a.zero_row, GAMD_CHK_CONV_SRC);
+        }
+        if (active) {
+            gemm128_post<false>((const f32x4*)by, lane, RB, RA,
+                                [&](int tp, int g) { RA[tp][g] = gamd_silu_hw(RA[tp][g]); },
+                                [&]() { FENCE(); stage(a.w3p, bx); FENCE(); });
+            TMARK(4);
+        } else {
+            stage(a.w3p, bx);
+        }
+        phase_barrier<0>();
+        asm volatile("" ::"v"(mask), "v"(p0), "v"(src_n));
+        TMARK(5);
+        if (active) {
+            const unsigned bl = (unsigned)__ballot(src != a.zero_row) >> (4 * half);
+            const unsigned real = (bl & 0xFu) | ((bl >> 4) & 0xF0u) | ((bl >> 8) & 0xF00u) | ((bl >> 12) & 0xF000u);
+#pragma unroll
+            for (int tp = 0; tp < 4; ++tp) {
+                const float b = vb3[32 * tp + slot];
+#pragma unroll
+                for (int r = 0; r < 16; ++r) RC[tp][r] = ((real >> r) & 1u) ? b : GAMD_L0_PAD;
+            }
+            TMARK(7);
+            const unsigned keep_bits = ~(mask << 1);
+            gemm128_post<true>((const f32x4*)bx, lane, RA, RC, [&](int tp, int r) {
+                RC[tp][r] = gamd_l0_acc(RC[tp][r], (r > 0 && ((keep_bits >> r) & 1u)) ? RC[tp][r - 1] : 0.f);
+            }, [&]() { FENCE(); if (it + 1 < n_iter) stage(a.w1p, by); FENCE(); });
+            pend_ends = mask;
+            if (nvalid > 0 && !((mask >> (nvalid - 1)) & 1u)) pend_ends |= 1u << (nvalid - 1);
+            pend_p = p0;
+            TMARK(10);
+        } else {
+            if (it + 1 < n_iter) stage(a.w1p, by);
+        }
+        if (!early) phase_barrier<0>();
+        TMARK(11);
+        if (active_n) load_e_tile(a.e_frag, tile_n, lane, RA);
+        TMARK(12);
+        if (early) early_barrier(active_n);
+        TMARK(13);
+        tile = tile_n; active = active_n; src = src_n;
+    }
+    } else {
     for (int it = 0; it < n_iter; ++it) {
         const int x0 = tile * GAMD_TILE + 16 * half;
         int nvalid = E - x0;
@@ -242,6 +325,7 @@
         TMARK(13);
         tile = tile_n; active = active_n; src = src_n; dst = dst_n;
     }
+    }
 #undef FENCE
     piece_stores();
     if (TIME && a.tdbg && lane == 0) {
@@ -251,12 +335,12 @@
 #undef TMARK
 }
 
-template <bool TIME>
+template <bool TIME, bool L0>
 int launch(const ConvEdgeArgs& a, int n_blocks, hipStream_t st) {
-    const size_t lds = sizeof(float) * CONV_LDS_FLOATS;
+    const size_t lds = sizeof(float) * conv_lds_floats(L0);
     static PerDeviceOnce once;
-    if (int e = gamd_allow_dynamic_lds(once, (int)lds, k_conv_edge<TIME>)) return e;
-    hipLaunchKernelGGL(k_conv_edge<TIME>, dim3(n_blocks), dim3(512), lds, st, a);
+    if (int e = gamd_allow_dynamic_lds(once, (int)lds, k_conv_edge<TIME, L0>)) return e;
+    hipLaunchKernelGGL((k_conv_edge<TIME, L0>), dim3(n_blocks), dim3(512), lds, st, a);
     GAMD_CHECK_LAUNCH();
     return 0;
 }
@@ -266,7 +350,15 @@
 int launch_conv_edge(const ConvEdgeArgs& a, int n_blocks, hipStream_t st) {
 #ifdef GAMD_PROFILING
     static const bool timed = getenv("GAMD_CONV_TIME") != nullptr;
-    if (timed) return launch<true>(a, n_blocks, st);
+    if (timed) return launch<true, false>(a, n_blocks, st);
 #endif
-    return launch<false>(a, n_blocks, st);
-}
+    return launch<false, false>(a, n_blocks, st);
+}
+
+int launch_conv_edge_l0(const ConvEdgeArgs& a, int n_blocks, hipStream_t st) {
+#ifdef GAMD_PROFILING
+    static const bool timed = getenv("GAMD_CONV_TIME") != nullptr;
+    if (timed) return launch<true, true>(a, n_blocks, st);
+#endif
+    return launch<false, true>(a, n_blocks, st);
+}
diff --git a/gamd_amd/csrc/conv_edge_small.hip b/gamd_amd/csrc/conv_edge_small.hip
--- a/gamd_amd/csrc/conv_edge_small.hip
+++ b/gamd_amd/csrc/conv_edge_small.hip
@@ -5,7 +5,7 @@
 
 constexpr int XLD = GAMD_XLD;
 
-template <int EHT, int HT, bool WIDE>
+template <int EHT, int HT, bool WIDE, bool L0>
 __global__ void __launch_bounds__(256) k_conv_edge_small(ConvEdgeArgs a) {
     if (a.devflags[DEVFLAG_FROZEN]) return;
     constexpr int H = 128 * HT;
@@ -21,7 +21,7 @@
         const int x = tile * GAMD_TILE + gamd_pi(slot);
         const bool valid = x < E;
         const int src = valid ? GAMD_CHK_RANGE(a.sticky, a.col[x], 0, a.zero_row, GAMD_CHK_CONV_SRC) : 0;
-        const int dst = valid ? GAMD_CHK_RANGE(a.sticky, a.erow[x], 0, a.zero_row, GAMD_CHK_CONV_DST) : 0;
+        const int dst = (valid && !L0) ? GAMD_CHK_RANGE(a.sticky, a.erow[x], 0, a.zero_row, GAMD_CHK_CONV_DST) : 0;
         f32x16 X[4], XE[EHT][4], acc;
         WQuarter wa, wb;
         const float* wblk = a.w1p;
@@ -38,15 +38,17 @@
                     for (int j = 0; j < 4; ++j) XE[kb][t][q * 4 + j] = v[j];
                 }
         }
-        const f32x16 s_q = load_slice(a.S + (size_t)src * 128, quarter, half);
-        const f32x16 d_q = load_slice(a.D + (size_t)dst * 128, quarter, half);
+        const f32x16 s_q = load_slice(a.S + (L0 ? 0 : (size_t)src * 128), quarter, half);
+        const f32x16 d_q = load_slice(a.D + (L0 ? 0 : (size_t)dst * 128), quarter, half);
         f32x16 hn_q[HT];
+        if (!L0) {
 #pragma unroll
-        for (int r = 0; r < 16; ++r) {
-            const int rho = (r & 3) + 8 * (r >> 2) + 4 * half;
-            const int s = __shfl(src, rho, 64);
+            for (int r = 0; r < 16; ++r) {
+                const int rho = (r & 3) + 8 * (r >> 2) + 4 * half;
+                const int s = __shfl(src, rho, 64);
 #pragma unroll
-            for (int ob = 0; ob < HT; ++ob) hn_q[ob][r] = a.hn[(size_t)s * H + feat4(ob)];
+                for (int ob = 0; ob < HT; ++ob) hn_q[ob][r] = a.hn[(size_t)s * H + feat4(ob)];
+            }
         }
         const unsigned mask = a.chunk_mask[tile * 2 + half];
         const int p0 = GAMD_CHK_RANGE(a.sticky, a.chunk_piece[tile * 2 + half], 0, a.piece_cap - 17, GAMD_CHK_PIECE);
@@ -68,12 +70,38 @@
         constexpr int B2 = EHT;
         WQuarter& w2 = (B2 & 1) ? wb : wa;
         WQuarter& w3 = (B2 & 1) ? wa : wb;
-        if (WIDE) acc = s_q + d_q; else acc = d_q;
-        load_wquarter(wblk + (size_t)(B2 + 1) * GAMD_WFRAG_FLOATS, quarter, lane, w3);
+        if (WIDE || L0) acc = s_q + d_q; else acc = d_q;
+        load_wquarter(L0 ? a.w3p : wblk + (size_t)(B2 + 1) * GAMD_WFRAG_FLOATS, quarter, lane, w3);
         gemm_quarter<false>(w2, X, acc);
 #pragma unroll
-        for (int r = 0; r < 16; ++r) acc[r] = gamd_silu_hw(WIDE ? acc[r] : acc[r] + s_q[r]);
+        for (int r = 0; r < 16; ++r) acc[r] = gamd_silu_hw((WIDE || L0) ? acc[r] : acc[r] + s_q[r]);
         exchange(xbuf, quarter, slot, half, acc, X);
+        if constexpr (L0) {
+            const unsigned bl = (unsigned)__ballot(valid && src != a.zero_row) >> (4 * half);
+            const unsigned real = (bl & 0xFu) | ((bl >> 4) & 0xF0u) | ((bl >> 8) & 0xF00u) | ((bl >> 12) & 0xF000u);
+            const float b = a.b3[32 * quarter + slot];
+#pragma unroll
+            for (int r = 0; r < 16; ++r) acc[r] = ((real >> r) & 1u) ? b : GAMD_L0_PAD;
+            gemm_quarter<true>(w3, X, acc);
+            const unsigned keep_bits = ~(mask << 1);
+#pragma unroll
+            for (int r = 0; r < 16; ++r) acc[r] = gamd_l0_acc(acc[r], (r > 0 && ((keep_bits >> r) & 1u)) ? acc[r - 1] : 0.f);
+            unsigned ends = mask;
+            if (nvalid > 0 && !((mask >> (nvalid - 1)) & 1u)) ends |= 1u << (nvalid - 1);
+            int p = p0;
+            while (__any(ends != 0)) {
+                if (ends != 0) {
+                    const int r = __builtin_ctz(ends);
+                    ends &= ends - 1;
+                    float v = acc[0];
+#pragma unroll
+                    for (int k = 1; k < 16; ++k) v = (r == k) ? acc[k] : v;
+                    a.partial[(size_t)p * H + feat4(0)] = v;
+                    ++p;
+                }
+            }
+            continue;
+        }
         acc = load_slice(a.b3, quarter, half);
         load_wquarter(wblk + (size_t)(B2 + 2) * GAMD_WFRAG_FLOATS, quarter, lane, w2);
         gemm_quarter<false>(w3, X, acc);
@@ -120,16 +148,22 @@
 }
 
 int launch_conv_edge_small(const ConvEdgeArgs& a, int n_blocks, hipStream_t st) {
-    hipLaunchKernelGGL((k_conv_edge_small<1, 1, false>), dim3(n_blocks), dim3(256), 0, st, a);
+    hipLaunchKernelGGL((k_conv_edge_small<1, 1, false, false>), dim3(n_blocks), dim3(256), 0, st, a);
+    GAMD_CHECK_LAUNCH();
+    return 0;
+}
+
+int launch_conv_edge_small_l0(const ConvEdgeArgs& a, int n_blocks, hipStream_t st) {
+    hipLaunchKernelGGL((k_conv_edge_small<1, 1, false, true>), dim3(n_blocks), dim3(256), 0, st, a);
     GAMD_CHECK_LAUNCH();
     return 0;
 }
 
 int launch_conv_edge_small_wide(const ConvEdgeArgs& a, int eht, int ht, int n_blocks, hipStream_t st) {
-    if (eht == 1 && ht == 1) hipLaunchKernelGGL((k_conv_edge_small<1, 1, true>), dim3(n_blocks), dim3(256), 0, st, a);
-    else if (eht == 1 && ht == 2) hipLaunchKernelGGL((k_conv_edge_small<1, 2, true>), dim3(n_blocks), dim3(256), 0, st, a);
-    else if (eht == 2 && ht == 1) hipLaunchKernelGGL((k_conv_edge_small<2, 1, true>), dim3(n_blocks), dim3(256), 0, st, a);
-    else if (eht == 2 && ht == 2) hipLaunchKernelGGL((k_conv_edge_small<2, 2, true>), dim3(n_blocks), dim3(256), 0, st, a);
+    if (eht == 1 && ht == 1) hipLaunchKernelGGL((k_conv_edge_small<1, 1, true, false>), dim3(n_blocks), dim3(256), 0, st, a);
+    else if (eht == 1 && ht == 2) hipLaunchKernelGGL((k_conv_edge_small<1, 2, true, false>), dim3(n_blocks), dim3(256), 0, st, a);
+    else if (eht == 2 && ht == 1) hipLaunchKernelGGL((k_conv_edge_small<2, 1, true, false>), dim3(n_blocks), dim3(256), 0, st, a);
+    else if (eht == 2 && ht == 2) hipLaunchKernelGGL((k_conv_edge_small<2, 2, true, false>), dim3(n_blocks), dim3(256), 0, st, a);
     else return -22;
     GAMD_CHECK_LAUNCH();
     return 0;
diff --git a/gamd_amd/csrc/gamd_api.hip b/gamd_amd/csrc/gamd_api.hip
--- a/gamd_amd/csrc/gamd_api.hip
+++ b/gamd_amd/csrc/gamd_api.hip
@@ -74,6 +74,7 @@
     const float *w1p, *w2p, *w3p, *w4p, *b1, *b3, *b4;
     const float *w16p = nullptr;
     const float *e_ln_g = nullptr, *e_ln_b = nullptr;
+    const float *w3p_l0 = nullptr, *b3_l0 = nullptr;
     NodeLayerW node;
 };
 
@@ -121,6 +122,7 @@
     bool update_edge = false;
     bool node_f16 = false;
     bool wide_enc = false, wide_conv = false;
+    bool l0_hoist = false;
     long long small_tile_limit = 512;
     std::map<std::string, HostTensor> host_w;
     bool finalized = false;
@@ -596,6 +598,7 @@
     no.pos_s = h->pos_s.as<float4>();
     no.node_emb = h->node_emb; no.enc_w = h->nenc_w; no.enc_b = h->nenc_b;
     no.row_ptr = h->row_ptr.as<int>(); no.na_excl = h->na_excl.as<int>(); no.deg = h->deg.as<int>();
+    no.col = (h->l0_hoist && h->n_boxes > 1) ? h->col.as<int>() : nullptr;
     no.partial = h->partial.as<float>();
     no.piece_cap = h->piece_cap;
     no.P_in = h->P.as<float>();
@@ -639,6 +642,8 @@
         const LayerDev& ld = h->layers[l];
         ca.w1p = ld.w1p; ca.w2p = ld.w2p; ca.w3p = ld.w3p; ca.w4p = ld.w4p; ca.w16p = ld.w16p;
         ca.b1 = ld.b1; ca.b3 = ld.b3; ca.b4 = ld.b4;
+        const bool hoist = l == 0 && h->l0_hoist;
+        if (hoist) { ca.w3p = ld.w3p_l0; ca.b3 = ld.b3_l0; }
         ca.partial = h->partial.as<float>();
         ca.piece_cap = h->piece_cap;
         ca.sticky = h->sticky_dev;
@@ -657,6 +662,7 @@
                                               : launch_conv_edge_wide(ca, h->EHT, h->HT, h->n_cu, st))
             : h->cfg.edge_dtype == GAMD_EDGE_BF16 ? launch_conv_edge_bf16(ca, h->n_cu, st)
             : h->cfg.edge_dtype == GAMD_EDGE_F16X3 ? launch_conv_edge_f16x3(ca, h->n_cu, st)
+            : hoist ? (small_tiles > 0 ? launch_conv_edge_small_l0(ca, small_tiles, st) : launch_conv_edge_l0(ca, h->n_cu, st))
             : small_tiles > 0 ? launch_conv_edge_small(ca, small_tiles, st) : launch_conv_edge(ca, h->n_cu, st);
         if (r) return fail(-1, "conv edge launch failed (%d)", r);
         if ((r = tev_end())) return r;
@@ -824,7 +830,7 @@
         return fail(-22, "unknown self_loop_mode %d", cfg->self_loop_mode);
     if (cfg->self_loop_mode != GAMD_SELF_LOOP_DGL07_NOOP && cfg->edge_dtype != GAMD_EDGE_F32)
         return fail(-22, "self_loop_mode 1 is built for the fp32 edge dtype only");
-    if (cfg->kernel_select & ~(GAMD_KSEL_FORCE_GENERIC_WIDTH | GAMD_KSEL_FORCE_HALF_QUANTUM))
+    if (cfg->kernel_select & ~(GAMD_KSEL_FORCE_GENERIC_WIDTH | GAMD_KSEL_FORCE_HALF_QUANTUM | GAMD_KSEL_NO_LAYER0_HOIST))
         return fail(-22, "unknown kernel_select bits 0x%x", cfg->kernel_select);
     int ndev = 0;
     if (hipGetDeviceCount(&ndev) != hipSuccess || ndev <= 0)
@@ -997,7 +1003,8 @@
     const int64_t Dp = h->Dp, DT = h->DT;
     const bool expand = !h->cfg.no_expand_edge;
     BlobBuilder bb;
-    struct Off { size_t w1p, w2p, w3p, w4p, w16p = 0, b1, b3, b4, elng = 0, elnb = 0, lng, lnb, wsp, wdp, wpdp, bS, bP, wpep, wphip, bphi; };
+    struct Off { size_t w1p, w2p, w3p, w4p, w16p = 0, b1, b3, b4, elng = 0, elnb = 0, lng, lnb, wsp, wdp, wpdp, bS, bP, wpep, wphip, bphi;
+                 size_t w3p_l0 = 0, b3_l0 = 0, m0 = 0, c0 = 0; };
     std::vector<Off> lo(L);
     std::deque<HostTensor> padded;
     auto get = [&](const std::string& nm, std::initializer_list<int64_t> shp, std::initializer_list<int64_t> pad) -> const HostTensor* {
@@ -1069,6 +1076,20 @@
     }
     const bool norm_bn = h->host_w.count("graph_conv.norm_layers.0.running_mean") != 0;
     h->norm_bn = norm_bn ? 1 : 0;
+    h->l0_hoist = h->cfg.kind == GAMD_KIND_LJ && h->cfg.edge_dtype == GAMD_EDGE_F32 && !h->wide_conv && DT == 1 && !update_edge &&
+                  !(h->cfg.kernel_select & GAMD_KSEL_NO_LAYER0_HOIST);
+    const HostTensor* emb0 = h->l0_hoist ? get("node_emb", {1, Ht}, {1, H}) : nullptr;
+    if (h->l0_hoist && !emb0) return -2;
+    auto permute_f2 = [](const HostTensor& w, const HostTensor& b, HostTensor& wo, HostTensor& bo) {
+        wo = w;
+        bo = b;
+        for (int q = 0; q < 4; ++q)
+            for (int s = 0; s < 32; ++s) {
+                std::copy(w.data.begin() + (size_t)(4 * s + q) * 128, w.data.begin() + (size_t)(4 * s + q + 1) * 128,
+                          wo.data.begin() + (size_t)(32 * q + s) * 128);
+                bo.data[32 * q + s] = b.data[4 * s + q];
+            }
+    };
     for (int l = 0; l < L; ++l) {
         const std::string p = "graph_conv.conv." + std::to_string(l);
         const HostTensor *ea0w = get(p + ".edge_affine.mlp_layer.0.weight", {128, Et}, {128, Eh}), *ea0b = get(p + ".edge_affine.mlp_layer.0.bias", {128}, {128});
@@ -1114,17 +1135,48 @@
             sb = scaled(sb, LOG2E); db = scaled(db, LOG2E); ea2b = scaled(ea2b, LOG2E);
         }
         Off& o = lo[l];
+        if (l == 0 && h->l0_hoist) {
+            std::vector<double> hn0((size_t)H, 0.0);
+            if (norm_bn) {
+                for (int64_t i = 0; i < H; ++i) hn0[i] = (double)emb0->data[i] * ng->data[i] + nb->data[i];
+            } else {
+                double mean = 0.0, var = 0.0;
+                for (int64_t i = 0; i < Ht; ++i) mean += emb0->data[i];
+                mean /= (double)Ht;
+                for (int64_t i = 0; i < Ht; ++i) var += ((double)emb0->data[i] - mean) * ((double)emb0->data[i] - mean);
+                var /= (double)Ht;
+                const double rstd = 1.0 / std::sqrt(var + 1e-5);
+                for (int64_t i = 0; i < Ht; ++i) hn0[i] = ((double)emb0->data[i] - mean) * rstd * ng->data[i] + nb->data[i];
+            }
+            HostTensor m0, c0;
+            m0.shape = {Dp, Dp};
+            m0.data.assign((size_t)(Dp * Dp), 0.f);
+            c0.shape = {Dp};
+            c0.data.assign((size_t)Dp, 0.f);
+            std::vector<double> row((size_t)Dp);
+            for (int64_t r = 0; r < Dp; ++r) {
+                std::fill(row.begin(), row.end(), 0.0);
+                double cr = 0.0;
+                for (int64_t i = 0; i < H; ++i) {
+                    const double a = (double)pew->data[(size_t)(r * H + i)] * hn0[i];
+                    if (a == 0.0) continue;
+                    for (int64_t k = 0; k < Dp; ++k) row[k] += a * t3w->data[(size_t)(i * Dp + k)];
+                    cr += a * t3b->data[i];
+                }
+                for (int64_t k = 0; k < Dp; ++k) m0.data[(size_t)(r * Dp + k)] = (float)row[k];
+                c0.data[r] = (float)cr;
+            }
+            HostTensor w3f, b3f;
+            permute_f2(*t1w, *t1b, w3f, b3f);
+            o.w3p_l0 = put_blocks(&w3f, 1, 1);
+            o.b3_l0 = put_vec(&b3f);
+            o.m0 = put_node(&m0, 1, 1);
+            o.c0 = put_vec(&c0);
+        }
         HostTensor b4_perm;
         HostTensor w4_perm;
         auto permute_w4 = [&]() {
-            w4_perm = *t3w;
-            b4_perm = *t3b;
-            for (int q = 0; q < 4; ++q)
-                for (int s = 0; s < 32; ++s) {
-                    std::copy(t3w->data.begin() + (size_t)(4 * s + q) * 128, t3w->data.begin() + (size_t)(4 * s + q + 1) * 128,
-                              w4_perm.data.begin() + (size_t)(32 * q + s) * 128);
-                    b4_perm.data[32 * q + s] = t3b->data[4 * s + q];
-                }
+            permute_f2(*t3w, *t3b, w4_perm, b4_perm);
             t3b = &b4_perm;
         };
         if (bf16_edges) {
@@ -1260,6 +1312,11 @@
         d.node.wsp = B + o.wsp; d.node.wdp = B + o.wdp; d.node.wpdp = B + o.wpdp;
         d.node.bS = B + o.bS; d.node.bP = B + o.bP;
         d.node.wpep = B + o.wpep; d.node.wphip = B + o.wphip; d.node.bphi = B + o.bphi;
+        d.node.c0 = nullptr;
+        if (l == 0 && h->l0_hoist) {
+            d.w3p_l0 = B + o.w3p_l0; d.b3_l0 = B + o.b3_l0;
+            d.node.wpep = B + o.m0; d.node.c0 = B + o.c0;
+        }
     }
     h->enc_w1p = B + o_e1; h->enc_w2p = B + o_e2; h->enc_w3p = B + o_e3;
     h->enc_b1 = B + o_eb1; h->enc_b2 = B + o_eb2; h->enc_b3 = B + o_eb3;
diff --git a/gamd_amd/csrc/gamd_common.h b/gamd_amd/csrc/gamd_common.h
--- a/gamd_amd/csrc/gamd_common.h
+++ b/gamd_amd/csrc/gamd_common.h
@@ -129,6 +129,12 @@
 
 __device__ __forceinline__ float gamd_msg_acc(float hn, float e_emb, float prev) { return __builtin_fmaf(hn, e_emb, prev); }
 
+#define GAMD_L0_PAD (-0x1p100f)
+__device__ __forceinline__ float gamd_l0_acc(float pre, float prev) {
+    const float e = __builtin_amdgcn_exp2f(pre * -1.4426950408889634f);
+    return __builtin_fmaf(pre, __builtin_amdgcn_rcpf(1.0f + e), prev);
+}
+
 __host__ __device__ __forceinline__ int gamd_tab16_pos(int f) {
     return 16 * (2 * (f >> 5) + ((f >> 4) & 1)) + 8 * ((f >> 2) & 1) + 4 * ((f >> 3) & 1) + (f & 3);
 }
diff --git a/gamd_amd/csrc/gamd_internal.h b/gamd_amd/csrc/gamd_internal.h
--- a/gamd_amd/csrc/gamd_internal.h
+++ b/gamd_amd/csrc/gamd_internal.h
@@ -188,8 +188,10 @@
     float* emb_out;
 };
 int launch_conv_edge(const ConvEdgeArgs& a, int n_blocks, hipStream_t st);
+int launch_conv_edge_l0(const ConvEdgeArgs& a, int n_blocks, hipStream_t st);
 int launch_conv_edge_bf16(const ConvEdgeArgs& a, int n_blocks, hipStream_t st);
 int launch_conv_edge_small(const ConvEdgeArgs& a, int n_blocks, hipStream_t st);
+int launch_conv_edge_small_l0(const ConvEdgeArgs& a, int n_blocks, hipStream_t st);
 int launch_conv_edge_small_wide(const ConvEdgeArgs& a, int eht, int ht, int n_blocks, hipStream_t st);
 int launch_conv_edge_f16x3(const ConvEdgeArgs& a, int n_blocks, hipStream_t st);
 int launch_conv_edge_wide(const ConvEdgeArgs& a, int eht, int ht, int n_blocks, hipStream_t st);
@@ -215,6 +217,7 @@
     const float* bS;
     const float* bP;
     const float* wpep;
+    const float* c0;
     const float* wphip;
     const float* bphi;
 };
@@ -229,6 +232,7 @@
     const float* node_emb;
     const float* enc_w; const float* enc_b;
     const int* row_ptr; const int* na_excl; const int* deg;
+    const int* col;
     const float* partial;
     long long piece_cap;
     const float* h_in;
diff --git a/gamd_amd/csrc/node.hip b/gamd_amd/csrc/node.hip
--- a/gamd_amd/csrc/node.hip
+++ b/gamd_amd/csrc/node.hip
@@ -168,6 +168,19 @@
         const int p0 = rp0 / GAMD_CHUNK + na_incl;
         const int np = dg > 0 ? ((rp0 + dg - 1) / GAMD_CHUNK - rp0 / GAMD_CHUNK + 1) : 0;
         (void)GAMD_CHK_RANGE(a.sticky, (long long)p0 + np, 0, a.piece_cap, GAMD_CHK_NODE_PIECES);
+        float n_real = 0.f;
+        if (a.post.c0) {
+            float n_pad = 0.f;
+            if (a.col) {
+#pragma unroll
+                for (int k = 0; k < 4; ++k) {
+                    const int j = g + 4 * k;
+                    if (j < dg && a.col[rp0 + dg - 1 - j] == a.n) n_pad += 1.f;
+                }
+                n_pad = group_sum(n_pad);
+            }
+            n_real = (float)dg - n_pad;
+        }
         mine[0] = f32x4{0.f, 0.f, 0.f, 0.f};
         mine[1] = mine[0];
         f32x4 p_in[2], h_res[2];
@@ -191,6 +204,14 @@
         NMARK(2);
         mine[0] = p_in[0]; mine[1] = p_in[1];
         GEMM16(true, a.post.wpep, a.post.wphip);
+        if (a.post.c0) {
+            f32x4 c[2];
+            load16(a.post.c0, w, g, c);
+#pragma unroll
+            for (int o = 0; o < 2; ++o)
+#pragma unroll
+                for (int r = 0; r < 4; ++r) mine[o][r] = fmaf(n_real, c[o][r], mine[o][r]);
+        }
         NMARK(3);
 #pragma unroll
         for (int o = 0; o < 2; ++o)
diff --git a/gamd_amd/engine.py b/gamd_amd/engine.py
--- a/gamd_amd/engine.py
+++ b/gamd_amd/engine.py
@@ -16,6 +16,7 @@
 FLAVOUR = {"jaxmd": 0, "torch": 1}
 SELF_LOOP = {"dgl07_noop": 0, "append_zero_feature_loops": 1}
 KSEL_FORCE_GENERIC_WIDTH = 1
+KSEL_NO_LAYER0_HOIST = 4
 
 
 def _box3(box) -> np.ndarray:
diff --git a/include/gamd_hip.h b/include/gamd_hip.h
--- a/include/gamd_hip.h
+++ b/include/gamd_hip.h
@@ -38,7 +38,7 @@
     int32_t n_boxes;
 } gamd_config;
 enum { GAMD_SELF_LOOP_DGL07_NOOP = 0, GAMD_SELF_LOOP_APPEND_ZERO_FEATURE = 1 };
-enum { GAMD_KSEL_FORCE_GENERIC_WIDTH = 1, GAMD_KSEL_FORCE_HALF_QUANTUM = 2 };
+enum { GAMD_KSEL_FORCE_GENERIC_WIDTH = 1, GAMD_KSEL_FORCE_HALF_QUANTUM = 2, GAMD_KSEL_NO_LAYER0_HOIST = 4 };
 
 const char* gamd_version(void);
 const char* gamd_last_error(void);
```
